# zhu-xlab/tomosar2height

Measured on AMD Instinct MI355X. Metric: training tiles/sec (Berlin crop, cloud-only), higher is better.
Workload: dtype f32; 1 GPU; BASELINE.json configs[1]: Berlin cloud-only, fp32 per-point GEMMs, train_step(tile) per tile, 4 tiles coalesced per forward/backward (Trainer default), N=131072 points/tile, R=256, ALTO depth 5, 512x512 target, optimize_every=64; points_per_tile=131072, optimize_every=64, train_batch=1, coalesce_tiles=4, optimizer=t2h FlatAdamW (one kernel over the flat bucket), parallelism=dp1, rccl_ranks=0, channels_last=True, point_distribution=70 % in 160 buildings + 30 % uniform, grid_convs=conv_bx3.hip: fp32 products from 3 fp16 MFMAs (2-way split, block scales), library_fallbacks=0, hip_graph=False

## Files before the change

### include/t2h.h

```cpp
#ifndef T2H_H_
#define T2H_H_

#include <stddef.h>
#include <stdint.h>

#ifdef __cplusplus
extern "C" {
#endif

#define T2H_OK 0
#define T2H_ERR_ARG (-1)
#define T2H_ERR_LAUNCH (-2)
#define T2H_ERR_WORKSPACE (-3)

#define T2H_ABI_VERSION 19
#define T2H_MAX_NBITS 10
#define T2H_MAX_RAGGED_TILES 64

typedef void *t2h_stream_t;

int t2h_abi_version(void);
const char *t2h_last_error_string(void);
const char *t2h_last_kernel_name(void);
void t2h_clear_kernel_name(void);
// ... 9 lines not shown
size_t t2h_tile_ragged_workspace_bytes(int B, int64_t total_rows, int max_rows, int nbits);
int t2h_tile_build_ragged(const float *cloud, int dim, int B, const int32_t *starts, int nbits, float *pts_sorted, int out_dim,
                          int32_t *perm, int32_t *cell, int32_t *off0, int32_t *status, void *workspace,
                          size_t workspace_bytes, t2h_stream_t stream);

int t2h_pool_winner_stride(int C);
int t2h_pool_max_fwd(const float *feat, int ldf, const int32_t *off0, int B, int nbits, int C, float *pooled,
                     int ldp, uint8_t *winner, t2h_stream_t stream);
int t2h_pool_max_bwd(const float *gpooled, int ldg, const uint8_t *winner, const int32_t *off0, int B, int nbits,
                     int C, int accumulate, float *gfeat, int ldo, t2h_stream_t stream);
int t2h_scatter_max_fwd(const float *feat, int ld, const int32_t *perm, const int32_t *off0, int B, int N, int nbits, int C,
                        float *val, int64_t *arg, t2h_stream_t stream);
int t2h_scatter_max_bwd(const float *gval, const int64_t *arg, int B, int C, int N, int64_t cells, float *gsrc,
                        t2h_stream_t stream);
int t2h_pool_mean(const float *feat, int ldf, const int32_t *off0, int B, int nbits, int C, int accumulate, float *out,
                  int ldo, t2h_stream_t stream);
int t2h_pool_rows_fwd(const float *feat, int ldf, const int32_t *cell, const int32_t *off0, int64_t n_rows, int C,
                      float *pooled, int ldp, uint8_t *winner, t2h_stream_t stream);
int t2h_pool_rows_bwd(const float *gpooled, int ldg, const uint8_t *winner, const int32_t *cell, const int32_t *off0,
                      int64_t n_rows, int C, int accumulate, float *gfeat, int ldo, t2h_stream_t stream);

size_t t2h_segmean_workspace_bytes(int B, int N, int nbits, int level, int C);
int t2h_segmean_fwd(const float *feat, const int32_t *off0, int B, int N, int nbits, int level, int C,
                    float *plane_nhwc, void *workspace, size_t workspace_bytes, t2h_stream_t stream);
int t2h_segmean_bwd(const float *gplane_nhwc, const int32_t *cell, const int32_t *off0, int B, int N,
                    int nbits, int level, int C, float *gfeat, t2h_stream_t stream);
int t2h_segsum_fwd(const float *feat, const int32_t *off0, int B, int N, int nbits, int level, int C,
                   float *plane_nhwc, int ld_plane, void *workspace, size_t workspace_bytes, t2h_stream_t stream);
int t2h_plane_sumpool2x2(const float *fine_nhwc, int ld_fine, int B, int r_fine, int C, float *coarse_nhwc, int ld_coarse,
                         t2h_stream_t stream);
int t2h_segsum_bwd_multi(const float *const *gplanes_nhwc, const int *levels, const int *lds, int n_planes, const int32_t *cell,
                         int B, int N, int nbits, int C, const float *mask, const float *addend, float *gfeat,
                         t2h_stream_t stream);
int t2h_cell_counts(const int32_t *off0, int B, int nbits, int level, float *cnt, t2h_stream_t stream);
int t2h_mean_bias_fwd(const float *acc, const float *cnt, const float *cvec, int64_t P, int C, float *out, t2h_stream_t stream);
size_t t2h_mean_bias_bwd_workspace_bytes(int64_t P, int C);
int t2h_mean_bias_bwd(const float *g, const float *cnt, int64_t P, int C, float *dacc, float *dcvec, void *workspace,
                      size_t workspace_bytes, t2h_stream_t stream);
int t2h_sample_relu_cellsums(const float *plane_nhwc, const float *pts, int dim, const int32_t *off0, int B, int N, int nbits,
                             int level, int sum_level, int C, float *sums_nhwc, int ld_sums, void *sign_bits, t2h_stream_t stream);
int t2h_sample_relu_cellsums2(const float *plane_nhwc, const float *pts, int dim, const int32_t *off0, int B, int N, int nbits,
                              int level, int sum_level, int C, float *sums_nhwc, int ld_sums, float *pooled_nhwc, int ld_pooled,
                              void *sign_bits, t2h_stream_t stream);
size_t t2h_cell_order_len(int B, int nbits, int level);
int t2h_cell_order_build(const int32_t *off0, int B, int nbits, int level, int32_t *order, t2h_stream_t stream);
int t2h_cell_order_build_range(const int32_t *off0, int B, int nbits, int level_lo, int level_hi, int32_t *order,
                               t2h_stream_t stream);
int t2h_sample_relu_cellsums_ordered(const float *plane_nhwc, const float *pts, int dim, const int32_t *off0, int B, int N,
                                     int nbits, int level, int sum_level, int C, float *sums_nhwc, int ld_sums, float *pooled_nhwc,
                                     int ld_pooled, void *sign_bits, const int32_t *cell_order, t2h_stream_t stream);
int t2h_sample_bwd_from_sums(const float *const *gplanes_nhwc, const int *levels, const int *lds, int n_planes,
                             const int32_t *cell, const void *mask, int mask_is_bits, const float *pts, int dim, const int32_t *off0, int B, int N,
                             int nbits, int level, int C, float *gplane_nhwc, void *workspace, size_t workspace_bytes,
                             t2h_stream_t stream);
int t2h_sample_bwd_from_sums_ordered(const float *const *gplanes_nhwc, const int *levels, const int *lds, int n_planes,
                                     const int32_t *cell, const void *mask, int mask_is_bits, const float *pts, int dim,
                                     const int32_t *off0, int B, int N, int nbits, int level, int C, float *gplane_nhwc,
                                     void *workspace, size_t workspace_bytes, const int32_t *cell_order, t2h_stream_t stream);
int t2h_segmean_bwd_add(const float *gplane_nhwc, const int32_t *cell, const int32_t *off0, int B, int N, int nbits,
                        int level, int C, const float *addend, float *gfeat, t2h_stream_t stream);

int t2h_sample_fwd(const float *plane_nhwc, const float *pts, int dim, int B, int N, int r, int C, float *out,
                   t2h_stream_t stream);
int t2h_sample_fwd_relu(const float *plane_nhwc, const float *pts, int dim, int B, int N, int r, int C, float *out,
                        void *sign_bits, t2h_stream_t stream);
size_t t2h_sample_bwd_workspace_bytes(int B, int N, int nbits, int level, int C);
// ... 216 lines not shown
```

### tomosar2height_amd/_lib.py

```python
import ctypes
import os

import torch

_HERE = os.path.dirname(os.path.abspath(__file__))
LIB_PATH = os.environ.get("T2H_LIBRARY") or os.path.join(_HERE, "libt2h_hip.so")
ABI_VERSION = 19

_vp, _i, _i64, _sz = ctypes.c_void_p, ctypes.c_int, ctypes.c_int64, ctypes.c_size_t

SIGNATURES = {
    "t2h_abi_version": (_i, []),
    "t2h_last_error_string": (ctypes.c_char_p, []),
    "t2h_last_kernel_name": (ctypes.c_char_p, []),
    "t2h_clear_kernel_name": (None, []),
    "t2h_debug_poison_lds": (_i, [_vp]),
    "t2h_coordinate2index": (_i, [_vp, _i, _i64, _i, _vp, _vp]),
    "t2h_tile_workspace_bytes": (_sz, [_i, _i, _i]),
    "t2h_tile_build": (_i, [_vp, _i, _i, _i, _i, _vp, _vp, _vp, _vp, _vp, _vp, _sz, _vp]),
    "t2h_tile_ragged_workspace_bytes": (_sz, [_i, _i64, _i, _i]),
    "t2h_tile_build_ragged": (_i, [_vp, _i, _i, _vp, _i, _vp, _i, _vp, _vp, _vp, _vp, _vp, _sz, _vp]),
    "t2h_pool_winner_stride": (_i, [_i]),
    "t2h_pool_max_fwd": (_i, [_vp, _i, _vp, _i, _i, _i, _vp, _i, _vp, _vp]),
    "t2h_pool_max_bwd": (_i, [_vp, _i, _vp, _vp, _i, _i, _i, _i, _vp, _i, _vp]),
    "t2h_pool_mean": (_i, [_vp, _i, _vp, _i, _i, _i, _i, _vp, _i, _vp]),
    "t2h_scatter_max_fwd": (_i, [_vp, _i, _vp, _vp, _i, _i, _i, _i, _vp, _vp, _vp]),
    "t2h_scatter_max_bwd": (_i, [_vp, _vp, _i, _i, _i, _i64, _vp, _vp]),
    "t2h_pool_rows_fwd": (_i, [_vp, _i, _vp, _vp, _i64, _i, _vp, _i, _vp, _vp]),
    "t2h_pool_rows_bwd": (_i, [_vp, _i, _vp, _vp, _vp, _i64, _i, _i, _vp, _i, _vp]),
    "t2h_segmean_workspace_bytes": (_sz, [_i, _i, _i, _i, _i]),
    "t2h_segmean_fwd": (_i, [_vp, _vp, _i, _i, _i, _i, _i, _vp, _vp, _sz, _vp]),
    "t2h_segmean_bwd": (_i, [_vp, _vp, _vp, _i, _i, _i, _i, _i, _vp, _vp]),
    "t2h_segmean_bwd_add": (_i, [_vp, _vp, _vp, _i, _i, _i, _i, _i, _vp, _vp, _vp]),
    "t2h_segsum_fwd": (_i, [_vp, _vp, _i, _i, _i, _i, _i, _vp, _i, _vp, _sz, _vp]),
    "t2h_plane_sumpool2x2": (_i, [_vp, _i, _i, _i, _i, _vp, _i, _vp]),
    "t2h_segsum_bwd_multi": (_i, [_vp, _vp, _vp, _i, _vp, _i, _i, _i, _i, _vp, _vp, _vp, _vp]),
    "t2h_cell_counts": (_i, [_vp, _i, _i, _i, _vp, _vp]),
    "t2h_mean_bias_fwd": (_i, [_vp, _vp, _vp, _i64, _i, _vp, _vp]),
    "t2h_mean_bias_bwd_workspace_bytes": (_sz, [_i64, _i]),
    "t2h_mean_bias_bwd": (_i, [_vp, _vp, _i64, _i, _vp, _vp, _vp, _sz, _vp]),
    "t2h_sample_relu_cellsums": (_i, [_vp, _vp, _i, _vp, _i, _i, _i, _i, _i, _i, _vp, _i, _vp, _vp]),
    "t2h_sample_relu_cellsums2": (_i, [_vp, _vp, _i, _vp, _i, _i, _i, _i, _i, _i, _vp, _i, _vp, _i, _vp, _vp]),
    "t2h_cell_order_len": (_sz, [_i, _i, _i]),
    "t2h_cell_order_build": (_i, [_vp, _i, _i, _i, _vp, _vp]),
    "t2h_cell_order_build_range": (_i, [_vp, _i, _i, _i, _i, _vp, _vp]),
    "t2h_sample_relu_cellsums_ordered": (_i, [_vp, _vp, _i, _vp, _i, _i, _i, _i, _i, _i, _vp, _i, _vp, _i, _vp, _vp, _vp]),
    "t2h_sample_bwd_from_sums": (_i, [_vp, _vp, _vp, _i, _vp, _vp, _i, _vp, _i, _vp, _i, _i, _i, _i, _i, _vp, _vp, _sz, _vp]),
    "t2h_sample_bwd_from_sums_ordered": (_i, [_vp, _vp, _vp, _i, _vp, _vp, _i, _vp, _i, _vp, _i, _i, _i, _i, _i, _vp, _vp, _sz, _vp, _vp]),
    "t2h_sample_fwd": (_i, [_vp, _vp, _i, _i, _i, _i, _i, _vp, _vp]),
# ... 288 lines not shown
    if name not in _declared:
        raise T2HLibraryError(f"{name} is not declared: the module that binds its header (`_lib.declare`) has not been imported, "
                              "and an untyped call would truncate 64-bit device pointers")
    return getattr(load(), name)


_POISON_LDS = os.environ.get("T2H_POISON_LDS", "0") == "1"


def call(name: str, *args, nbytes: int = 0, flops: int = 0, tag: str = None):
    fn = _fn_cache.get(name)
    if fn is None:
        fn = _fn_cache[name] = _entry(name)
    if _POISON_LDS:
        load().t2h_debug_poison_lds(stream())
    tl = _timeline
    if tl is None:
        rc = fn(*args)
        if rc != 0:
            check(rc, name)
        return
    else:
        s, e = torch.cuda.Event(enable_timing=True), torch.cuda.Event(enable_timing=True)
        lib = load()
        lib.t2h_clear_kernel_name()
        s.record()
        rc = fn(*args)
        e.record()
        symbol = lib.t2h_last_kernel_name().decode() or name
        tl.records.append((tag or name, nbytes, flops, s, e, symbol))
    check(rc, name)


def ptr(t: torch.Tensor) -> int:
    return t.data_ptr()


_ws_cache = {}


def ws_bytes(name: str, *args) -> int:
    key = (name, args)
    hit = _ws_cache.get(key)
    if hit is None:
        hit = _ws_cache[key] = int(_entry(name)(*args))
    return hit


def workspace(nbytes: int, device) -> torch.Tensor:
    return torch.empty(max(int(nbytes), 1), dtype=torch.uint8, device=device)


_on_stream = None
_set_stream = getattr(torch._C, "_cuda_setStream", None)


class on_stream:

    def __init__(self, st, back):
        self.st, self.back = st, back

    def __enter__(self):
        global _on_stream
        st = self.st
        self.prev, _on_stream = _on_stream, st.cuda_stream
        if _set_stream is not None:
# ... 81 lines not shown
```

### tomosar2height_amd/csrc/conv_bx3.hip

```cpp
#include <stdlib.h>
#include "t2h_common.h"
#include "gemm_args.h"
#include "gemm_tile.h"

namespace t2h {
namespace {

using bf16x8 = __attribute__((ext_vector_type(8))) __bf16;
using f16x8 = __attribute__((ext_vector_type(8))) _Float16;
using f16x2 = __attribute__((ext_vector_type(2))) _Float16;
using bf16x2 = __attribute__((ext_vector_type(2))) __bf16;
using f32x2 = __attribute__((ext_vector_type(2))) float;
using s16x4 = __attribute__((ext_vector_type(4))) short;
using s16x8 = __attribute__((ext_vector_type(8))) short;
typedef __attribute__((address_space(3))) void lds_void;
typedef const __attribute__((address_space(1))) void glb_void;
typedef __attribute__((address_space(3))) s16x4 lds_s16x4;

#ifndef T2H_BX3_BDIRECT
#define T2H_BX3_BDIRECT 1
#endif
constexpr int NT = 256;
constexpr int TW = 32;
constexpr int CC = 32;
// ... 150 lines not shown
__global__ __launch_bounds__(256) void prep_split_batch_kernel(PrepBatch b) {
    const int i = prep_find(b, blockIdx.x);
    const t2h_prep_desc &d = b.d[i];
    const long long t = (long long)(blockIdx.x - b.first[i]) * 256 + threadIdx.x;
    unsigned *wf = static_cast<unsigned *>(d.wf), *trailer = wf + d.trailer_word;
    if (d.h2) {
        if (t == 0) trailer[d.maxslot ^ 3] = 0u;
        if (d.kind == 0) prepare_conv_body<false, true>(d.w, d.a, d.b, wf, trailer, d.maxslot, t);
        else if (d.kind == 1) prepare_conv_body<true, true>(d.w, d.a, d.b, wf, trailer, d.maxslot, t);
        else if (d.kind == 2) prepare_gemm_body<true, true>(d.w, d.a, d.b, d.ldw, wf, trailer, d.maxslot, t);
        else prepare_gemm_body<false, true>(d.w, d.a, d.b, d.ldw, wf, trailer, d.maxslot, t);
    } else {
        if (d.kind == 0) prepare_conv_body<false, false>(d.w, d.a, d.b, wf, nullptr, 0, t);
        else if (d.kind == 1) prepare_conv_body<true, false>(d.w, d.a, d.b, wf, nullptr, 0, t);
        else if (d.kind == 2) prepare_gemm_body<true, false>(d.w, d.a, d.b, d.ldw, wf, nullptr, 0, t);
        else prepare_gemm_body<false, false>(d.w, d.a, d.b, d.ldw, wf, nullptr, 0, t);
    }
}

struct RowsArgs {
    const float *x;
    const unsigned *wf;
    const float *wscale;
    const float *bias;
    const float *mask;
    float *y;
    int B, H, W, Kc, Nc, flags;
    int splits, chunks_per_split;
    int ntn_per_wg;
    int ldx, ldy, ldm;
    const float *addend;
    int up_logW, up_logH, up_cout;
    const float *r1_g, *r1_w;
};

__device__ inline size_t up_pixel(long long m, int tap, int logW, int logH) {
    const long long x = m & ((1LL << logW) - 1), y = (m >> logW) & ((1LL << logH) - 1), b = m >> (logW + logH);
    return (size_t)(((b << (logH + 1)) + 2 * y + (tap >> 1)) << (logW + 1)) + 2 * x + (tap & 1);
}

template <int TH, int BN, int WAVES_M, int WAVES_N, int CCH, int NPL, int NTAP, int UPM = 0, bool PERSIST = false>
__global__ __launch_bounds__(NT, 2) void bx3_rows_kernel(RowsArgs p) {
    static_assert(UPM == 0 || NTAP == 1, "the transposed convolution runs on the 1-tap form");
    static_assert(!PERSIST || (NTAP == 1 && UPM == 0 && T2H_BX3_BDIRECT != 0), "PERSIST: plain 1-tap form with register-fetched weights");
    constexpr int PXB = CCH * 2 + 16;
    constexpr int NQ = CCH / 16, F4 = CCH / 4, NSTEP = NTAP * NQ;
    constexpr int QUNROLL = (NPL == 3 && NTAP == 9) ? 1 : NQ;
    constexpr int TM = TH / WAVES_M, TN = BN / (32 * WAVES_N);
    constexpr int HB = NTAP == 9 ? 1 : 0;
    constexpr int HW = TW + 2 * HB;
    constexpr int HP = (TH + 2 * HB) * HW;
    constexpr int PLANE = HP * PXB;
    constexpr int BSLAB = (BN / 32) * NPL * 1024;
    constexpr int HALO_BYTES = NPL * PLANE;
    constexpr bool BDIRECT = T2H_BX3_BDIRECT != 0;
    constexpr int LDS_WORK = HALO_BYTES + (BDIRECT ? 0 : 2 * BSLAB);
    constexpr int PATCH_BYTES = 4 * 32 * 36 * 4;
    constexpr int LDS_BYTES = PERSIST ? LDS_WORK + PATCH_BYTES : (LDS_WORK >= PATCH_BYTES ? LDS_WORK : PATCH_BYTES);
    constexpr bool H2 = NPL == 2;
    constexpr int WPL = H2 ? 2 : 3;
    static_assert(WAVES_M * WAVES_N == 4 && TM * WAVES_M == TH && TN * WAVES_N * 32 == BN, "wave layout");
    __shared__ __attribute__((aligned(1024))) unsigned char lds[LDS_BYTES + (H2 ? 64 : 0)];
    unsigned char *halo = lds, *bbuf = lds + HALO_BYTES;
    float *slots = reinterpret_cast<float *>(lds + LDS_BYTES);

    const int tid = threadIdx.x, lane = tid & 63, wave = tid >> 6;
    const int wm = wave / WAVES_N, wn = wave % WAVES_N;
    const unsigned nb = gridDim.x, bid = blockIdx.x;
    const unsigned qq = nb / 8, rr = nb % 8, xx = bid % 8, i8 = bid / 8;
    unsigned t = (xx < rr ? xx * (qq + 1) : rr * (qq + 1) + (xx - rr) * qq) + i8;
    const int split = t % p.splits; t /= p.splits;
    const int ntn = p.Nc / BN;
    const int tn_groups = PERSIST ? (ntn + p.ntn_per_wg - 1) / p.ntn_per_wg : ntn;
    const int tng = t % tn_groups; t /= tn_groups;
    const int tn_lo = PERSIST ? tng * p.ntn_per_wg : tng, tn_hi = PERSIST ? min(ntn, tn_lo + p.ntn_per_wg) : tng + 1;
    const int tiles_x = p.W / TW;
    const int tx = t % tiles_x; t /= tiles_x;
    const int tiles_y = p.H / TH;
    const int ty = t % tiles_y, b = t / tiles_y;
    const int x0 = tx * TW, y0 = ty * TH;
    int n0 = tn_lo * BN;
    const int c_beg = split * p.chunks_per_split, c_end = min(p.Kc / CCH, c_beg + p.chunks_per_split);

    constexpr int NF4 = HP * F4, PER = (NF4 + NT - 1) / NT;
    float4 hreg[PER];
    auto halo_load = [&](int c) {
#pragma unroll
        for (int f = 0; f < PER; ++f) {
            const int idx = tid + f * NT;
            const int px = idx / F4, c4 = idx % F4;
            const int hy = px / HW, hx = px - hy * HW;
            const int gy = y0 + hy - HB, gx = x0 + hx - HB;
            float4 v = make_float4(0.f, 0.f, 0.f, 0.f);
            if (UPM == 2) {
                const int k0 = c * CCH, tap = k0 / p.up_cout, co0 = k0 - tap * p.up_cout;
                if (idx < NF4)
                    v = *reinterpret_cast<const float4 *>(p.x + up_pixel(((long long)b * p.H + gy) * p.W + gx, tap, p.up_logW, p.up_logH) *
                                                                    p.ldx + co0 + c4 * 4);
            } else if (idx < NF4 && (unsigned)gy < (unsigned)p.H && (unsigned)gx < (unsigned)p.W)
                v = *reinterpret_cast<const float4 *>(p.x + (((size_t)b * p.H + gy) * p.W + gx) * p.ldx + c * CCH + c4 * 4);
            hreg[f] = v;
        }
    };
    int e_run = E_UNSET, e_cur = 0;
    auto halo_store = [&]() {
#pragma unroll
        for (int f = 0; f < PER; ++f) {
            const int idx = tid + f * NT;
            if (idx < NF4) {
                const int px = idx / F4, c4 = idx % F4;
                unsigned a1, a2, a3, b1, b2, b3;
                unsigned char *d = halo + px * PXB + c4 * 8;
                if (H2) {
                    split2h(hreg[f].x, hreg[f].y, e_cur, a1, a2);
                    split2h(hreg[f].z, hreg[f].w, e_cur, b1, b2);
                    *reinterpret_cast<uint2 *>(d) = make_uint2(a1, b1);
                    *reinterpret_cast<uint2 *>(d + PLANE) = make_uint2(a2, b2);
                    continue;
                }
                split3(hreg[f].x, hreg[f].y, a1, a2, a3);
                split3(hreg[f].z, hreg[f].w, b1, b2, b3);
                *reinterpret_cast<uint2 *>(d) = make_uint2(a1, b1);
                if (NPL == 3) {
                    *reinterpret_cast<uint2 *>(d + PLANE) = make_uint2(a2, b2);
                    *reinterpret_cast<uint2 *>(d + 2 * PLANE) = make_uint2(a3, b3);
                }
            }
        }
    };
    auto publish_block_max = [&](int parity) {
        float m = 0.f;
#pragma unroll
// ... 770 lines not shown
    if (int rc = check_launch("conv3x3_bx3_wgrad")) return rc;
    return launch_reduce_slabs(slab, p.splits, (long long)Cout * Ncols, Cout, Ncols, Ncols, (flags & T2H_ACCUM) ? 1 : 0, dw, colslab, db, s,
                               0, 0, (flags & T2H_DEFER_REDUCE) != 0);
}

T2H_API int t2h_gemm_bx3_supported(int64_t M, int K, int N) {
    return M >= 128 && M % 128 == 0 && M <= (1LL << 30) && K >= 64 && K % 64 == 0 && N >= 32 && N % 32 == 0;
}

T2H_API size_t t2h_gemm_bx3_weights_bytes(int K, int N) {
    if (K < 16 || N < 32 || K % 16 || N % 32) return 0;
    return (size_t)K * N * 6;
}

T2H_API int t2h_gemm_bx3_prepare(const float *w, int ldw, int K, int N, int w_is_kn, void *wf, t2h_stream_t stream) {
    if (!w || !wf) return fail(T2H_ERR_ARG, "gemm_bx3_prepare: null pointer");
    if (K < 16 || N < 32 || K % 16 || N % 32 || !al16(wf) || ldw < (w_is_kn ? N : K))
        return fail(T2H_ERR_ARG, "gemm_bx3_prepare: K=%d must be a multiple of 16, N=%d of 32, ldw=%d at least the row length", K, N, ldw);
    const long long total = (long long)(K / 16) * (N / 32) * 64;
    const unsigned blocks = (unsigned)((total + 255) / 256);
    if (w_is_kn) hipLaunchKernelGGL(bx3_prepare_gemm_kernel<true>, dim3(blocks), dim3(256), 0, as_stream(stream), w, K, N, ldw, static_cast<unsigned *>(wf));
    else hipLaunchKernelGGL(bx3_prepare_gemm_kernel<false>, dim3(blocks), dim3(256), 0, as_stream(stream), w, K, N, ldw, static_cast<unsigned *>(wf));
    return check_launch("gemm_bx3_prepare");
}

T2H_API size_t t2h_gemm_bx3_workspace_bytes(int64_t M, int K, int N) {
    if (!t2h_gemm_bx3_supported(M, K, N)) return 0;
    const RowsPlan r = bx3_rows_plan(1, (int)(M / 32), 32, K, N, 1);
    return r.splits > 1 ? (size_t)r.splits * M * N * sizeof(float) : 0;
}

T2H_API int t2h_gemm_bx3(const float *x, int ldx, const void *wf, const float *bias, const float *mask, int ldm, float *y, int ldy,
                         int64_t M, int K, int N, int flags, void *workspace, size_t workspace_bytes, t2h_stream_t stream) {
    if (!x || !wf || !y) return fail(T2H_ERR_ARG, "gemm_bx3: null pointer");
    if (!t2h_gemm_bx3_supported(M, K, N))
        return fail(T2H_ERR_ARG, "gemm_bx3: needs M %% 128 == 0, K %% 64 == 0, N %% 32 == 0 (M=%lld K=%d N=%d)", (long long)M, K, N);
    if (ldx < K || ldy < N || ldx % 4 || ldy % 4 || (mask && (ldm < N || ldm % 4)) || !al16(x) || !al16(wf) || !al16(y) || (bias && !al16(bias)) ||
        (mask && !al16(mask)))
        return fail(T2H_ERR_ARG, "gemm_bx3: rows must be 16-byte aligned and at least K / N floats long");
    RowsArgs a{};
    a.x = x; a.wf = static_cast<const unsigned *>(wf); a.bias = bias; a.mask = mask; a.y = y;
    a.B = 1; a.H = (int)(M / 32); a.W = 32; a.Kc = K; a.Nc = N; a.ldx = ldx; a.ldy = ldy; a.ldm = ldm;
    a.flags = ((flags & T2H_RELU_OUT) ? F_RELU_OUT : 0) | ((flags & T2H_ACCUM) ? F_ACCUM : 0);
    a.wscale = f16_trailer(wf, (size_t)K * N * 4);
    return launch_rows(a, npl_of(flags), workspace, workspace_bytes, as_stream(stream), "gemm_bx3", 1);
}

static int gemm_wgrad_splits(int64_t M, int N) {
    static const long long target = getenv("T2H_GEMM_BX3_WGRAD_WGS") ? atoll(getenv("T2H_GEMM_BX3_WGRAD_WGS")) : 4096;
    const long long groups = N / 64, units = M / TW;
    long long splits = (target + groups - 1) / groups;
    if (splits > units) splits = units;
    if (splits < 1) splits = 1;
    const long long per = (units + splits - 1) / splits;
    return (int)((units + per - 1) / per);
}

T2H_API int t2h_gemm_bx3_wgrad_supported(int64_t M, int K, int N) {
    return M >= TW && M % TW == 0 && M <= (1LL << 30) && (K == 64 || K == 128 || K == 256) && N >= 64 && N % 64 == 0;
}

T2H_API size_t t2h_gemm_bx3_wgrad_workspace_bytes(int64_t M, int K, int N) {
    if (!t2h_gemm_bx3_wgrad_supported(M, K, N)) return 0;
    return (size_t)gemm_wgrad_splits(M, N) * ((size_t)N * K + N) * sizeof(float);
}

T2H_API int t2h_gemm_bx3_wgrad(const float *dy, int lddy, const float *x, int ldx, int64_t M, int K, int N, float *dw, float *db, int flags,
                               void *workspace, size_t workspace_bytes, t2h_stream_t stream) {
    if (!dy || !x || !dw) return fail(T2H_ERR_ARG, "gemm_bx3_wgrad: null pointer");
    if (!t2h_gemm_bx3_wgrad_supported(M, K, N))
        return fail(T2H_ERR_ARG, "gemm_bx3_wgrad: needs M %% 32 == 0, K in {64, 128, 256}, N %% 64 == 0 (M=%lld K=%d N=%d)", (long long)M, K, N);
    if (lddy < N || ldx < K || lddy % 4 || ldx % 4 || !al16(dy) || !al16(x))
        return fail(T2H_ERR_ARG, "gemm_bx3_wgrad: rows must be 16-byte aligned and at least N / K floats long");
    if (!(flags & T2H_F16X2)) return fail(T2H_ERR_ARG, "gemm_bx3_wgrad: only the fp16 two-way split (T2H_F16X2) is built");
    const size_t need = t2h_gemm_bx3_wgrad_workspace_bytes(M, K, N);
    if (!workspace || workspace_bytes < need || !al16(workspace))
        return fail(T2H_ERR_WORKSPACE, "gemm_bx3_wgrad: workspace %zu < %zu bytes", workspace_bytes, need);
// ... 195 lines not shown
```

### tomosar2height_amd/csrc/deferred.hip

```cpp
#include "t2h_common.h"
#include "gemm_tile.h"

namespace t2h {
namespace {

__global__ __launch_bounds__(256) void cell_counts_kernel(const int32_t *__restrict__ off0, int B, int nbits, int level,
                                                         float *__restrict__ cnt) {
    const int rbits = nbits - level, r = 1 << rbits;
    const int64_t total = (int64_t)B << (2 * rbits);
    const int64_t i = (int64_t)blockIdx.x * 256 + threadIdx.x;
    if (i >= total) return;
    const int x = (int)(i & (r - 1)), y = (int)((i >> rbits) & (r - 1));
    const int64_t b = i >> (2 * rbits);
    const size_t obase = ((size_t)b << (2 * nbits)) + ((size_t)morton2((uint32_t)x, (uint32_t)y) << (2 * level));
    cnt[i] = (float)(off0[obase + ((size_t)1 << (2 * level))] - off0[obase]);
}

__global__ __launch_bounds__(256) void mean_bias_fwd_kernel(const float *__restrict__ acc, const float *__restrict__ cnt,
                                                           const float *__restrict__ cvec, int64_t total4, int C4,
                                                           float *__restrict__ out) {
    const int64_t t = (int64_t)blockIdx.x * 256 + threadIdx.x;
    if (t >= total4) return;
    const int64_t p = t / C4;
    const int c4 = (int)(t % C4);
    const float n = cnt[p];
    const float den = n > 0.f ? n : 1.f, ne = n > 0.f ? 1.f : 0.f;
    const float4 a = reinterpret_cast<const float4 *>(acc)[t];
    const float4 cv = reinterpret_cast<const float4 *>(cvec)[c4];
    float4 o;
    o.x = __fadd_rn(__fdiv_rn(a.x, den), __fmul_rn(ne, cv.x)); o.y = __fadd_rn(__fdiv_rn(a.y, den), __fmul_rn(ne, cv.y));
    o.z = __fadd_rn(__fdiv_rn(a.z, den), __fmul_rn(ne, cv.z)); o.w = __fadd_rn(__fdiv_rn(a.w, den), __fmul_rn(ne, cv.w));
    reinterpret_cast<float4 *>(out)[t] = o;
}

static int mb_rows(int64_t P) {
    int64_t r = (P + 255) / 256;
    r = (r + 63) / 64 * 64;
    return (int)(r < 64 ? 64 : (r > 4096 ? 4096 : r));
}
__global__ __launch_bounds__(256) void mean_bias_bwd_kernel(const float *__restrict__ g, const float *__restrict__ cnt,
                                                           int64_t P, int C, float *__restrict__ dacc,
                                                           float *__restrict__ slab, int kMbRows) {
    __shared__ float4 red[256];
    const int C4 = C / 4;
    const int cols = min(C4, 256), slots = 256 / cols;
    const int col = threadIdx.x % cols, slot = threadIdx.x / cols;
    const int64_t p0 = (int64_t)blockIdx.x * kMbRows;
    const int rows = (int)min((int64_t)kMbRows, P - p0);
    for (int c4base = 0; c4base < C4; c4base += cols) {
        const int c4 = c4base + col;
        float4 s = make_float4(0.f, 0.f, 0.f, 0.f);
        if (slot < slots && c4 < C4) {
            for (int i = slot; i < rows; i += slots) {
                const float n = cnt[p0 + i];
                const float4 v = reinterpret_cast<const float4 *>(g + (size_t)(p0 + i) * C)[c4];
                if (dacc) {
                    const float den = n > 0.f ? n : 1.f;
                    reinterpret_cast<float4 *>(dacc + (size_t)(p0 + i) * C)[c4] =
                        make_float4(__fdiv_rn(v.x, den), __fdiv_rn(v.y, den), __fdiv_rn(v.z, den), __fdiv_rn(v.w, den));
                }
                if (n > 0.f) { s.x += v.x; s.y += v.y; s.z += v.z; s.w += v.w; }
            }
        }
        __syncthreads();
        red[threadIdx.x] = s;
        __syncthreads();
        if (slab && slot == 0 && c4 < C4) {
            float4 t = red[col];
            for (int q = 1; q < slots; ++q) {
                const float4 u = red[q * cols + col];
                t.x += u.x; t.y += u.y; t.z += u.z; t.w += u.w;
            }
            reinterpret_cast<float4 *>(slab + (size_t)blockIdx.x * C)[c4] = t;
        }
    }
}

}
}

using namespace t2h;

T2H_API int t2h_cell_counts(const int32_t *off0, int B, int nbits, int level, float *cnt, t2h_stream_t stream) {
    if (!off0 || !cnt) return fail(T2H_ERR_ARG, "cell_counts: null pointer");
    if (B < 1 || nbits < 1 || nbits > T2H_MAX_NBITS || level < 0 || level > nbits) return fail(T2H_ERR_ARG, "cell_counts: bad level");
    const int64_t total = (int64_t)B << (2 * (nbits - level));
    hipLaunchKernelGGL(cell_counts_kernel, dim3((unsigned)((total + 255) / 256)), dim3(256), 0, as_stream(stream), off0, B, nbits,
                       level, cnt);
    return check_launch("cell_counts");
}

static bool al16(const void *p) { return ((uintptr_t)p & 15) == 0; }

T2H_API int t2h_mean_bias_fwd(const float *acc, const float *cnt, const float *cvec, int64_t P, int C, float *out,
                              t2h_stream_t stream) {
    if (!acc || !cnt || !cvec || !out) return fail(T2H_ERR_ARG, "mean_bias_fwd: null pointer");
    if (P < 0 || C < 4 || C % 4 != 0 || !al16(acc) || !al16(cvec) || !al16(out))
        return fail(T2H_ERR_ARG, "mean_bias_fwd: needs C %% 4 == 0 and 16-byte aligned rows");
    if (P == 0) return T2H_OK;
    const int64_t total4 = P * (C / 4);
    hipLaunchKernelGGL(mean_bias_fwd_kernel, dim3((unsigned)((total4 + 255) / 256)), dim3(256), 0, as_stream(stream), acc, cnt,
                       cvec, total4, C / 4, out);
    return check_launch("mean_bias_fwd");
}

T2H_API size_t t2h_mean_bias_bwd_workspace_bytes(int64_t P, int C) {
    if (P < 1 || C < 1) return 0;
    const int kMbRows = mb_rows(P);
    return (size_t)((P + kMbRows - 1) / kMbRows) * C * sizeof(float);
}

T2H_API int t2h_mean_bias_bwd(const float *g, const float *cnt, int64_t P, int C, float *dacc, float *dcvec, void *workspace,
                              size_t workspace_bytes, t2h_stream_t stream) {
    if (!g || !cnt) return fail(T2H_ERR_ARG, "mean_bias_bwd: null pointer");
    if (P < 1 || C < 4 || C % 4 != 0 || !al16(g) || (dacc && !al16(dacc)) || (dcvec && !al16(dcvec)))
        return fail(T2H_ERR_ARG, "mean_bias_bwd: needs P >= 1, C %% 4 == 0 and 16-byte aligned rows");
    const size_t need = t2h_mean_bias_bwd_workspace_bytes(P, C);
    if (dcvec && (!workspace || workspace_bytes < need || !al16(workspace)))
        return fail(T2H_ERR_WORKSPACE, "mean_bias_bwd: workspace %zu < %zu bytes", workspace_bytes, need);
    if (!dacc && !dcvec) return T2H_OK;
    const int kMbRows = mb_rows(P);
    const int blocks = (int)((P + kMbRows - 1) / kMbRows);
    float *slab = dcvec ? static_cast<float *>(workspace) : nullptr;
    hipLaunchKernelGGL(mean_bias_bwd_kernel, dim3(blocks), dim3(256), 0, as_stream(stream), g, cnt, P, C, dacc, slab, kMbRows);
    if (int rc = check_launch("mean_bias_bwd")) return rc;
    if (!dcvec) return T2H_OK;
    return launch_reduce_slabs(slab, blocks, C, 1, C, C, 0, dcvec, nullptr, nullptr, as_stream(stream));
}
```

### tomosar2height_amd/csrc/gemm.hip

```cpp
#include <stdlib.h>
#include <mutex>
#include <string>
#include <vector>
#include "t2h_common.h"
#include "gemm_args.h"
#include "gemm_tile.h"

namespace t2h {

using bf16x8 = __attribute__((ext_vector_type(8))) __bf16;

template <int BM, int BN, int WAVES_M, int WAVES_N, bool A_KC, bool B_KC, int BK = 16, bool XCD = true, int MINW = 1,
          int MODE = 0>
__global__ __launch_bounds__(64 * WAVES_M * WAVES_N, MINW) void gemm_kernel(GemmArgs p) {
    constexpr int NT = 64 * WAVES_M * WAVES_N;
    constexpr int TM = BM / (32 * WAVES_M), TN = BN / (32 * WAVES_N);
    constexpr int SA = BM + kPad, SB = BN + kPad;
    static_assert(TM >= 1 && TN >= 1, "tile too small for the wave grid");
    constexpr int LDS_MIN = (NT / 64) * 32 * 36 > 4 * NT ? (NT / 64) * 32 * 36 : 4 * NT;
    constexpr int LDS_FLOATS = 2 * BK * (SA + SB) > LDS_MIN ? 2 * BK * (SA + SB) : LDS_MIN;
    __shared__ __attribute__((aligned(16))) float lds[LDS_FLOATS];
    constexpr int BUF = BK * (SA + SB);

    const int tid = threadIdx.x, lane = tid & 63, wave = tid >> 6;
    const int wm = wave / WAVES_N, wn = wave % WAVES_N;
    int tile_m = blockIdx.y, tile_n = blockIdx.x, split = blockIdx.z;
    if (XCD) {
        const unsigned nb = gridDim.x * gridDim.y * gridDim.z;
        const unsigned b = (blockIdx.z * gridDim.y + blockIdx.y) * gridDim.x + blockIdx.x;
        const unsigned q = nb / 8, r = nb % 8, x = b % 8, i = b / 8;
        const unsigned t = (x < r ? x * (q + 1) : r * (q + 1) + (x - r) * q) + i;
        tile_n = t % gridDim.x;
        tile_m = (t / gridDim.x) % gridDim.y;
        split = t / (gridDim.x * gridDim.y);
    }
    const int m0 = tile_m * BM, n0 = tile_n * BN;
    const int kbeg = split * p.k_chunk;
    const int kend = min(p.K, kbeg + p.k_chunk);
    const bool relu_a = p.flags & F_RELU_A, relu_b = p.flags & F_RELU_B;

    TileLoader<BM, NT, A_KC, BK> la;
    TileLoader<BN, NT, B_KC, BK> lb;
    f32x16 acc[TM][TN];
#pragma unroll
    for (int i = 0; i < TM; ++i)
#pragma unroll
        for (int j = 0; j < TN; ++j)
#pragma unroll
            for (int q = 0; q < 16; ++q) acc[i][j][q] = 0.0f;

    float4 csum = make_float4(0.f, 0.f, 0.f, 0.f);
    const bool do_colsum = !A_KC && p.colsum != nullptr && tile_n == 0;

    const int nk = (kend - kbeg + BK - 1) / BK;
    if (nk > 0) {
        la.load(p.A, p.lda, m0, p.M, kbeg, kend, tid, relu_a);
        lb.load(p.B, p.ldb, n0, p.N, kbeg, kend, tid, relu_b);
        la.store(lds, tid);
        lb.store(lds + BK * SA, tid);
    }
    __syncthreads();
    for (int kt = 0; kt < nk; ++kt) {
        const int cur = kt & 1;
        if (do_colsum) {
#pragma unroll
            for (int f = 0; f < TileLoader<BM, NT, A_KC, BK>::PER; ++f) {
                csum.x += la.r[f].x; csum.y += la.r[f].y; csum.z += la.r[f].z; csum.w += la.r[f].w;
            }
        }
        if (kt + 1 < nk) {
            la.load(p.A, p.lda, m0, p.M, kbeg + (kt + 1) * BK, kend, tid, relu_a);
// ... 564 lines not shown
}

namespace {
struct WgradPlan { bool smallk; int bm, bn, tiles, splits, k_chunk; };
WgradPlan wgrad_plan(int M, int K, int N) {
    WgradPlan p{};
    p.smallk = (K % 4 != 0);
    if (p.smallk) { p.splits = (M + kSmallKRows - 1) / kSmallKRows; return p; }
    p.bm = N > 64 ? 128 : (N > 32 ? 64 : 32);
    p.bn = K > 64 ? 128 : (K > 32 ? 64 : 32);
    p.tiles = ((N + p.bm - 1) / p.bm) * ((K + p.bn - 1) / p.bn);
    const int target = p.tiles <= 2 ? 512 : 1024;
    int want = target / p.tiles;
    if (want > 512) want = 512;
    int max_splits = (M + 16 * kMinBK - 1) / (16 * kMinBK);
    int splits = want < 1 ? 1 : (want > max_splits ? max_splits : want);
    if (splits < 1) splits = 1;
    int chunk = (M + splits - 1) / splits;
    chunk = (chunk + 31) / 32 * 32;
    p.k_chunk = chunk;
    p.splits = (M + chunk - 1) / chunk;
    return p;
}
}

T2H_API size_t t2h_linear_wgrad_workspace_bytes(int M, int K, int N) {
    if (M < 1 || K < 1 || N < 1) return 0;
    WgradPlan p = wgrad_plan(M, K, N);
    return (size_t)p.splits * ((size_t)N * K + N) * sizeof(float);
}

T2H_API int t2h_linear_wgrad(const float *dy, int lddy, const float *x, int ldx, int M, int K, int N, int flags,
                             float *dw, float *db, void *workspace, size_t workspace_bytes, t2h_stream_t stream) {
    if (!dy || !x || !dw) return fail(T2H_ERR_ARG, "linear_wgrad: null pointer");
    if (M < 1 || K < 1 || N < 1 || lddy < N || ldx < K) return fail(T2H_ERR_ARG, "linear_wgrad: bad shape");
    size_t need = t2h_linear_wgrad_workspace_bytes(M, K, N);
    if (!workspace || workspace_bytes < need)
        return fail(T2H_ERR_WORKSPACE, "linear_wgrad: workspace %zu < %zu bytes", workspace_bytes, need);
    hipStream_t s = as_stream(stream);
    WgradPlan p = wgrad_plan(M, K, N);
    float *slab = static_cast<float *>(workspace);
    float *colslab = slab + (size_t)p.splits * N * K;
    int accumulate = (flags & T2H_ACCUM) ? 1 : 0;
    const bool direct = !p.smallk && p.splits == 1 && !accumulate && !db && aligned4(dw, K);
    if (direct) slab = dw;
    if (p.smallk) {
        if (K > kSmallKMax) return fail(T2H_ERR_ARG, "linear_wgrad: K=%d must be a multiple of 4 (or <= %d)", K, kSmallKMax);
        hipLaunchKernelGGL(wgrad_smallk_kernel, dim3(p.splits), dim3(256), 0, s, dy, lddy, x, ldx, M, K, N,
                           (flags & T2H_RELU_IN) ? 1 : 0, slab, db ? colslab : nullptr);
    } else {
        if (N % 4 != 0 || !aligned4(dy, lddy) || !aligned4(x, ldx))
            return fail(T2H_ERR_ARG, "linear_wgrad: N=%d must be a multiple of 4 (16-byte rows)", N);
        GemmArgs a{};
        a.A = dy; a.lda = lddy; a.B = x; a.ldb = ldx; a.C = slab; a.ldc = K; a.colsum = db ? colslab : nullptr;
        a.M = N; a.N = K; a.K = M; a.flags = (flags & T2H_RELU_IN) ? F_RELU_B : 0;
        a.k_chunk = p.k_chunk; a.slab_stride = (long long)N * K;
        int rc;
        const int mode = mode_of(flags);
        static const int kwaves_wgrad_max_rows = [] { const char *e = getenv("T2H_KWAVES_WGRAD_MAX_ROWS"); return e ? atoi(e) : 1024; }();
        if (mode == 0 && !db && M <= kwaves_wgrad_max_rows && aligned4(dw, K) && kwaves_applicable(N, K, M)) {
            a.C = dw; a.colsum = nullptr; a.k_chunk = M; a.slab_stride = 0;
            if (accumulate) a.flags |= F_ACCUM;
            return launch_gemm_kwaves<false, false>(a, s, "linear_wgrad");
        }
#define T2H_WG(BM_, BN_, WM_, WN_, MW_)                                                                                \
    (mode == 2 ? launch_gemm<BM_, BN_, WM_, WN_, false, false, 16, true, (MW_ > 2 ? 2 : MW_), 2>(a, p.splits, s, "linear_wgrad") \
     : mode == 1 ? launch_gemm<BM_, BN_, WM_, WN_, false, false, 16, true, (MW_ > 3 ? 3 : MW_), 1>(a, p.splits, s, "linear_wgrad") \
                 : launch_gemm<BM_, BN_, WM_, WN_, false, false, 16, true, MW_, 0>(a, p.splits, s, "linear_wgrad"))
        static const bool tn_dma = !(getenv("T2H_GEMM_DMA") && getenv("T2H_GEMM_DMA")[0] == '0');
        if (p.bm == 128 && p.bn == 128 && mode == 0 && tn_dma && gemm_dma_tn_applicable(a))
            rc = launch_gemm_dma_tn(a, p.splits, s, "linear_wgrad");
        else if (p.bm == 128 && p.bn == 128)
            rc = mode != 0 ? launch_gemm_split(mode, false, false, a, p.splits, s, "linear_wgrad") : T2H_WG(128, 128, 2, 2, 4);
        else if (p.bm == 128 && p.bn == 64) rc = T2H_WG(128, 64, 2, 2, 1);
        else if (p.bm == 128 && p.bn == 32) rc = T2H_WG(128, 32, 4, 1, 1);
        else if (p.bm == 64 && p.bn == 128) rc = T2H_WG(64, 128, 2, 2, 1);
        else if (p.bm == 64 && p.bn == 64) rc = T2H_WG(64, 64, 2, 2, 1);
        else if (p.bm == 64 && p.bn == 32) rc = T2H_WG(64, 32, 2, 1, 1);
        else if (p.bm == 32 && p.bn == 128) rc = T2H_WG(32, 128, 1, 4, 1);
        else if (p.bm == 32 && p.bn == 64) rc = T2H_WG(32, 64, 1, 2, 1);
        else rc = T2H_WG(32, 32, 1, 1, 1);
#undef T2H_WG
        if (rc) return rc;
    }
    if (direct) return T2H_OK;
    return launch_reduce_slabs(slab, p.splits, (long long)N * K, N, K, K, accumulate, dw, colslab, db, s, 0, 0,
                               (flags & T2H_DEFER_REDUCE) != 0);
}
```

### tomosar2height_amd/csrc/gemm_args.h

```cpp
#pragma once
#include <hip/hip_runtime.h>

namespace t2h {

enum : int { F_RELU_A = 1, F_RELU_B = 2, F_RELU_OUT = 4, F_ACCUM = 8 };

struct GemmArgs {
    const float *A, *B;
    float *C;
    const float *bias;
    const float *mask;
    const float *addend;
    int ldadd;
    float *colsum;
    int M, N, K;
    int lda, ldb, ldc, ldm;
    int flags;
    int k_chunk;
    long long slab_stride;
};

int launch_gemm_split(int mode, bool a_kc, bool b_kc, const GemmArgs &a, int splits, hipStream_t s, const char *what);

bool gemm_dma_applicable(bool b_kc, const GemmArgs &a);
int launch_gemm_dma(bool b_kc, const GemmArgs &a, hipStream_t s, const char *what);
bool gemm_dma_tn_applicable(const GemmArgs &a);
int launch_gemm_dma_tn(const GemmArgs &a, int splits, hipStream_t s, const char *what);

}
```

### tomosar2height_amd/csrc/point_grid.hip

```cpp
#include <float.h>
#include <stdlib.h>

#include "t2h_common.h"

namespace t2h {

constexpr int kThreads = 256;

struct GroupCfg {
    int lg;
    int span;
};

template <int VEC>
static GroupCfg group_cfg(int C) {
    GroupCfg g;
    g.lg = group_log2(C, VEC);
    g.span = (1 << g.lg) * VEC;
    return g;
}

static inline unsigned grid_for(int64_t groups, int lg) {
    int64_t threads = groups << lg;
    return (unsigned)((threads + kThreads - 1) / kThreads);
// ... 292 lines not shown
            for (int g = 1; g < NG; ++g) { const float4 v = pval[g * G + lane]; t.x += v.x; t.y += v.y; t.z += v.z; t.w += v.w; }
            oval[side * G + lane] = t;
        }
        __syncthreads();
    }
#pragma unroll
    for (int p = 0; p < PASSES; ++p) {
        const int row = r0 + p * NG + grp;
        if (row >= r1 || row != max(segs[p], r0)) continue;
        float4 acc = segs[p] < r0 ? oval[lane] : make_float4(0.f, 0.f, 0.f, 0.f);
        const int end = min(sege[p], r1);
        for (int n = row; n < end; ++n) { const float4 v = val[(n - r0) * G + lane]; acc.x += v.x; acc.y += v.y; acc.z += v.z; acc.w += v.w; }
        if (sege[p] > r1) { const float4 v = oval[G + lane]; acc.x += v.x; acc.y += v.y; acc.z += v.z; acc.w += v.w; }
        val[(row - r0) * G + lane] = acc;
    }
    __syncthreads();
#pragma unroll
    for (int p = 0; p < PASSES; ++p) {
        const int row = r0 + p * NG + grp;
        if (row >= r1 || !cv) continue;
        const float4 sum = val[(max(segs[p], r0) - r0) * G + lane];
        const uint8_t bits = winner[(size_t)row * wstride + lane];
        float4 o = make_float4((bits & 1) ? sum.x : 0.f, (bits & 2) ? sum.y : 0.f, (bits & 4) ? sum.z : 0.f, (bits & 8) ? sum.w : 0.f);
        float4 *dst = reinterpret_cast<float4 *>(gfeat + (size_t)row * ldo + lane * 4);
        if (accumulate) { const float4 old = *dst; o.x += old.x; o.y += old.y; o.z += old.z; o.w += old.w; }
        *dst = o;
    }
}

template <int VEC, bool MEAN = true>
__global__ __launch_bounds__(kThreads) void segmean_fwd_kernel(const float *__restrict__ feat,
                                                               const int32_t *__restrict__ off0, int B, int nbits,
                                                               int level, int C, int lg, float *__restrict__ plane,
                                                               int ld_out) {
    int64_t t = (int64_t)blockIdx.x * kThreads + threadIdx.x;
    int64_t gid = t >> lg;
    const int rbits = nbits - level;
    const int64_t cells_per_tile = (int64_t)1 << (2 * rbits);
    if (gid >= (int64_t)B * cells_per_tile) return;
    int b = (int)(gid >> (2 * rbits));
    uint32_t mk = (uint32_t)(gid & (cells_per_tile - 1));
    size_t obase = ((size_t)b << (2 * nbits)) + ((size_t)mk << (2 * level));
    int s = off0[obase], e = off0[obase + ((size_t)1 << (2 * level))];
    int cx = (int)compact1by1(mk), cy = (int)compact1by1(mk >> 1);
    int r = 1 << rbits;
    float *orow = plane + (((size_t)b * r + cy) * r + cx) * ld_out;
    float inv_den = (float)(e - s > 0 ? e - s : 1);
    int span = VEC << lg;
    for (int c = ((int)t & ((1 << lg) - 1)) * VEC; c < C; c += span) {
        float sum[VEC];
#pragma unroll
        for (int j = 0; j < VEC; ++j) sum[j] = 0.0f;
        int n = s;
        for (; n + 4 <= e; n += 4) {
            Vec<VEC> a0 = Vec<VEC>::load(feat + (size_t)(n + 0) * C + c);
            Vec<VEC> a1 = Vec<VEC>::load(feat + (size_t)(n + 1) * C + c);
            Vec<VEC> a2 = Vec<VEC>::load(feat + (size_t)(n + 2) * C + c);
            Vec<VEC> a3 = Vec<VEC>::load(feat + (size_t)(n + 3) * C + c);
#pragma unroll
            for (int j = 0; j < VEC; ++j) sum[j] = (((sum[j] + a0.v[j]) + a1.v[j]) + a2.v[j]) + a3.v[j];
        }
        for (; n < e; ++n) {
            Vec<VEC> a = Vec<VEC>::load(feat + (size_t)n * C + c);
#pragma unroll
            for (int j = 0; j < VEC; ++j) sum[j] += a.v[j];
        }
        Vec<VEC> o;
#pragma unroll
        for (int j = 0; j < VEC; ++j) o.v[j] = MEAN ? __fdiv_rn(sum[j], inv_den) : sum[j];
        o.store(orow + c);
    }
}

constexpr int kMaxMultiPlanes = 8;
struct MultiPlanes { const float *g[kMaxMultiPlanes]; int level[kMaxMultiPlanes]; int ld[kMaxMultiPlanes]; int n; };
template <int VEC>
__global__ __launch_bounds__(kThreads) void segsum_bwd_multi_kernel(MultiPlanes mp, const int32_t *__restrict__ cell,
                                                                    int64_t npts, int nbits, int C, int lg,
                                                                    const float *__restrict__ mask,
                                                                    const float *__restrict__ addend,
                                                                    float *__restrict__ gfeat) {
    int64_t t = (int64_t)blockIdx.x * kThreads + threadIdx.x;
    int64_t n = t >> lg;
    if (n >= npts) return;
    const uint32_t code = (uint32_t)cell[n];
    const uint32_t b = code >> (2 * nbits), m = code & ((1u << (2 * nbits)) - 1u);
    const uint32_t x0 = compact1by1(m), y0 = compact1by1(m >> 1);
    const float *rows[kMaxMultiPlanes];
#pragma unroll
    for (int q = 0; q < kMaxMultiPlanes; ++q) {
        rows[q] = nullptr;
        if (q < mp.n) {
            const int l = mp.level[q], r = 1 << (nbits - l);
            rows[q] = mp.g[q] + (((size_t)b * r + (y0 >> l)) * r + (x0 >> l)) * mp.ld[q];
        }
    }
    const int span = VEC << lg;
    for (int c = ((int)t & ((1 << lg) - 1)) * VEC; c < C; c += span) {
        Vec<VEC> acc = Vec<VEC>::load(rows[0] + c);
#pragma unroll
        for (int q = 1; q < kMaxMultiPlanes; ++q)
            if (q < mp.n) {
                Vec<VEC> g = Vec<VEC>::load(rows[q] + c);
#pragma unroll
                for (int j = 0; j < VEC; ++j) acc.v[j] = __fadd_rn(acc.v[j], g.v[j]);
            }
        if (mask) {
            Vec<VEC> h = Vec<VEC>::load(mask + (size_t)n * C + c);
#pragma unroll
            for (int j = 0; j < VEC; ++j) acc.v[j] = h.v[j] > 0.0f ? acc.v[j] : 0.0f;
        }
        if (addend) {
            Vec<VEC> o = Vec<VEC>::load(addend + (size_t)n * C + c);
#pragma unroll
            for (int j = 0; j < VEC; ++j) acc.v[j] = __fadd_rn(o.v[j], acc.v[j]);
        }
        acc.store(gfeat + (size_t)n * C + c);
    }
}

__global__ __launch_bounds__(kThreads) void plane_sumpool2x2_kernel(const float *__restrict__ fine, int64_t total4, int rc,
                                                                   int C4, int ld_in, int ld_out, float *__restrict__ coarse) {
    int64_t t = (int64_t)blockIdx.x * kThreads + threadIdx.x;
    if (t >= total4) return;
    const int c4 = (int)(t % C4);
    const int64_t pix = t / C4;
    const int x = (int)(pix % rc), y = (int)((pix / rc) % rc);
    const int64_t b = pix / ((int64_t)rc * rc);
    const int rf = 2 * rc;
    const float *f = fine + ((b * rf + 2 * y) * rf + 2 * x) * (int64_t)ld_in + 4 * c4;
    const float4 a = *reinterpret_cast<const float4 *>(f), bq = *reinterpret_cast<const float4 *>(f + ld_in);
    const float4 cq = *reinterpret_cast<const float4 *>(f + (int64_t)rf * ld_in);
    const float4 d = *reinterpret_cast<const float4 *>(f + (int64_t)rf * ld_in + ld_in);
    float4 o;
    o.x = (a.x + bq.x) + (cq.x + d.x); o.y = (a.y + bq.y) + (cq.y + d.y);
    o.z = (a.z + bq.z) + (cq.z + d.z); o.w = (a.w + bq.w) + (cq.w + d.w);
    *reinterpret_cast<float4 *>(coarse + pix * (int64_t)ld_out + 4 * c4) = o;
}

template <int VEC>
__global__ __launch_bounds__(kThreads) void segmean_bwd_kernel(const float *__restrict__ gplane,
                                                               const int32_t *__restrict__ cell,
                                                               const int32_t *__restrict__ off0, int64_t npts, int nbits,
                                                               int level, int C, int lg, const float *__restrict__ addend,
                                                               float *__restrict__ gfeat) {
    int64_t t = (int64_t)blockIdx.x * kThreads + threadIdx.x;
    int64_t n = t >> lg;
    if (n >= npts) return;
    uint32_t code = (uint32_t)cell[n];
    uint32_t b = code >> (2 * nbits);
    uint32_t m = code & ((1u << (2 * nbits)) - 1u);
    uint32_t mk = m >> (2 * level);
    size_t obase = ((size_t)b << (2 * nbits)) + ((size_t)mk << (2 * level));
    int cnt = off0[obase + ((size_t)1 << (2 * level))] - off0[obase];
    int rbits = nbits - level, r = 1 << rbits;
    int cx = (int)compact1by1(mk), cy = (int)compact1by1(mk >> 1);
    const float *grow = gplane + (((size_t)b * r + cy) * r + cx) * C;
    float den = (float)(cnt > 0 ? cnt : 1);
    int span = VEC << lg;
    for (int c = ((int)t & ((1 << lg) - 1)) * VEC; c < C; c += span) {
        Vec<VEC> g = Vec<VEC>::load(grow + c);
#pragma unroll
        for (int j = 0; j < VEC; ++j) g.v[j] = __fdiv_rn(g.v[j], den);
        if (addend) {
            Vec<VEC> o = Vec<VEC>::load(addend + (size_t)n * C + c);
#pragma unroll
// ... 74 lines not shown
}

__device__ inline float keep_if(unsigned long long lanes, float v) {
    float o;
    asm("v_cndmask_b32_e64 %0, 0, %1, %2" : "=v"(o) : "v"(v), "s"(lanes));
    return o;
}
__device__ inline float readlane_f(float v, int i) { return __int_as_float(__builtin_amdgcn_readlane(__float_as_int(v), i)); }
__device__ inline unsigned long long readlane_u64(unsigned long long v, int i) {
    const unsigned lo = (unsigned)__builtin_amdgcn_readlane((int)(unsigned)v, i);
    const unsigned hi = (unsigned)__builtin_amdgcn_readlane((int)(unsigned)(v >> 32), i);
    return ((unsigned long long)hi << 32) | lo;
}

typedef float f32x2 __attribute__((ext_vector_type(2)));
__device__ inline void park8(unsigned (&acc)[8], unsigned long long w0, unsigned long long w1, unsigned long long w2,
                             unsigned long long w3, int i) {
    asm("s_mov_b32 m0, %8\n\t"
        "v_writelane_b32 %0, %9, m0\n\tv_writelane_b32 %1, %10, m0\n\tv_writelane_b32 %2, %11, m0\n\tv_writelane_b32 %3, %12, m0\n\t"
        "v_writelane_b32 %4, %13, m0\n\tv_writelane_b32 %5, %14, m0\n\tv_writelane_b32 %6, %15, m0\n\tv_writelane_b32 %7, %16, m0"
        : "+v"(acc[0]), "+v"(acc[1]), "+v"(acc[2]), "+v"(acc[3]), "+v"(acc[4]), "+v"(acc[5]), "+v"(acc[6]), "+v"(acc[7])
        : "s"(__builtin_amdgcn_readfirstlane(i)), "s"((unsigned)w0), "s"((unsigned)(w0 >> 32)), "s"((unsigned)w1),
          "s"((unsigned)(w1 >> 32)), "s"((unsigned)w2), "s"((unsigned)(w2 >> 32)), "s"((unsigned)w3), "s"((unsigned)(w3 >> 32))
        : "m0");
}

template <int K, bool POOL>
__global__ __launch_bounds__(256, 2) void sample_relu_cellsums_v2_kernel(const float *__restrict__ plane,
                                                                        const float *__restrict__ pts, int dim,
                                                                        const int32_t *__restrict__ off0, int nbits, int level,
                                                                        int sum_level, int C, float *__restrict__ sums,
                                                                        int ld_sums, unsigned long long *__restrict__ bits,
                                                                        int npts_m1, float *__restrict__ sums2, int ld_sums2,
                                                                        const int32_t *__restrict__ order, int gz) {
    constexpr int SIDE = 3 + K, NS = SIDE * SIDE;
    __shared__ float4 T[NS][64];
    const int tid = threadIdx.x, lane = tid & 63, wave = tid >> 6;
    const int chunks = C >> 8;
    const int chunk = (int)(blockIdx.x % (unsigned)chunks), c0 = chunk * 256 + lane * 4;
    const int zpart = (int)((blockIdx.x / (unsigned)chunks) % (unsigned)gz);
    const unsigned rank = blockIdx.x / (unsigned)(chunks * gz);
    const int rbits = nbits - level, r = 1 << rbits, sbits = rbits - K;
    const int64_t wg = order ? (int64_t)order[rank] : (int64_t)rank;
    const int b = (int)(wg >> (2 * sbits));
    const uint32_t smk = (uint32_t)(wg & (((int64_t)1 << (2 * sbits)) - 1));
    const int d = level - sum_level, nchild = 1 << (2 * d), rs = 1 << (nbits - sum_level);
    const uint32_t mk = K == 0 ? smk : ((smk << 2) | (uint32_t)wave);
    const int cx = (int)compact1by1(mk), cy = (int)compact1by1(mk >> 1);
    const int per_wave = K == 0 ? nchild / (gz * 4) : nchild;
    const int child_lo = K == 0 ? (zpart * 4 + wave) * per_wave : 0, child_hi = child_lo + per_wave;
    const size_t obase = ((size_t)b << (2 * nbits)) + ((size_t)mk << (2 * level));
    int bnd_lo, bnd_hi;
    {
        const int ci = child_lo + lane;
        bnd_lo = ci <= child_hi ? off0[obase + ((size_t)ci << (2 * sum_level))] : 0;
        bnd_hi = ci + 1 <= child_hi ? off0[obase + ((size_t)(ci + 1) << (2 * sum_level))] : 0;
    }
    const int wx0 = K == 0 ? cx - 1 : 2 * (int)compact1by1(smk) - 1, wy0 = K == 0 ? cy - 1 : 2 * (int)compact1by1(smk >> 1) - 1;
    for (int e = tid; e < NS * 64; e += 256) {
        const int sl = e >> 6, py = wy0 + sl / SIDE, px = wx0 + sl % SIDE;
        float4 v = make_float4(0.f, 0.f, 0.f, 0.f);
        if ((unsigned)py < (unsigned)r && (unsigned)px < (unsigned)r)
            v = *reinterpret_cast<const float4 *>(plane + (((size_t)b * r + py) * r + px) * C + chunk * 256 + (e & 63) * 4);
        T[sl][e & 63] = v;
    }
    const int row_first = __builtin_amdgcn_readfirstlane(bnd_lo);
    const int row_end = off0[obase + ((size_t)child_hi << (2 * sum_level))];
// ... 37 lines not shown
                    sw_l = y1ok ? __fmul_rn(tp.wx0, tp.wy1) : 0.f;
                    se_l = (x1ok && y1ok) ? __fmul_rn(tp.wx1, tp.wy1) : 0.f;
#else
                    const float fx1 = (float)min(max(r - 1 - tp.x0, 0), 1), fy1 = (float)min(max(r - 1 - tp.y0, 0), 1);
                    nw_l = __fmul_rn(tp.wx0, tp.wy0);
                    ne_l = __fmul_rn(__fmul_rn(tp.wx1, tp.wy0), fx1);
                    sw_l = __fmul_rn(__fmul_rn(tp.wx0, tp.wy1), fy1);
                    se_l = __fmul_rn(__fmul_rn(tp.wx1, tp.wy1), __fmul_rn(fx1, fy1));
#endif
                    slot_l = (min(max(tp.y0 - cy + 1, 0), 1) + (K ? (wave >> 1) : 0)) * SIDE +
                             min(max(tp.x0 - cx + 1, 0), 1) + (K ? (wave & 1) : 0);
                }
                const int i0 = n - nb0, cnt = min(e - n, 64 - i0);
                auto row = [&](int i) {
                    const float nw = readlane_f(nw_l, i), ne = readlane_f(ne_l, i), sw = readlane_f(sw_l, i), se = readlane_f(se_l, i);
                    const float4 *t00 = Tl + __builtin_amdgcn_readlane(slot_l, i) * 64;
                    const float4 v00 = t00[0], v01 = t00[64], v10 = t00[SIDE * 64], v11 = t00[(SIDE + 1) * 64];
                    f32x2 a01 = f32x2{v00.x, v00.y} * nw, a23 = f32x2{v00.z, v00.w} * nw;
                    a01 = a01 + f32x2{v01.x, v01.y} * ne; a23 = a23 + f32x2{v01.z, v01.w} * ne;
                    a01 = a01 + f32x2{v10.x, v10.y} * sw; a23 = a23 + f32x2{v10.z, v10.w} * sw;
                    a01 = a01 + f32x2{v11.x, v11.y} * se; a23 = a23 + f32x2{v11.z, v11.w} * se;
                    a01.x = fmaxf(a01.x, 0.f); a01.y = fmaxf(a01.y, 0.f); a23.x = fmaxf(a23.x, 0.f); a23.y = fmaxf(a23.y, 0.f);
                    const unsigned long long w0 = __ballot(a01.x > 0.f), w1 = __ballot(a01.y > 0.f);
                    const unsigned long long w2 = __ballot(a23.x > 0.f), w3 = __ballot(a23.y > 0.f);
                    park8(bl, w0, w1, w2, w3, i);
                    sum01 = sum01 + a01; sum23 = sum23 + a23;
                };
                for (int j = 0; j < cnt; ++j) row(i0 + j);
                n += cnt;
            }
            const float4 sum = make_float4(sum01.x, sum01.y, sum23.x, sum23.y);
            const uint32_t cm = (uint32_t)(cb + c);
            const int fx = (cx << d) + (int)compact1by1(cm), fy = (cy << d) + (int)compact1by1(cm >> 1);
            *reinterpret_cast<float4 *>(sums + (((size_t)b * rs + fy) * rs + fx) * ld_sums + c0) = sum;
            if (POOL) {
                const unsigned k4 = cm & 3u;
                if (k4 == 0u) pe = sum;
                else if (k4 == 1u) p01 = make_float4(pe.x + sum.x, pe.y + sum.y, pe.z + sum.z, pe.w + sum.w);
                else if (k4 == 2u) pe = sum;
                else {
                    const float4 o = make_float4(p01.x + (pe.x + sum.x), p01.y + (pe.y + sum.y), p01.z + (pe.z + sum.z),
                                                 p01.w + (pe.w + sum.w));
                    const int rs2 = rs >> 1;
                    *reinterpret_cast<float4 *>(sums2 + (((size_t)b * rs2 + (fy >> 1)) * rs2 + (fx >> 1)) * ld_sums2 + c0) = o;
                }
            }
        }
    }
    flush_bits();
}

template <int VEC>
__global__ __launch_bounds__(kThreads) void sample_bwd_kernel(const float *__restrict__ gout,
                                                              const float *__restrict__ pts, int dim,
                                                              const int32_t *__restrict__ off0, int B, int nbits,
                                                              int level, int C, int lg, const float *__restrict__ addend,
                                                              float *__restrict__ gplane) {
    int64_t t = (int64_t)blockIdx.x * kThreads + threadIdx.x;
    int64_t gid = t >> lg;
    const int rbits = nbits - level, r = 1 << rbits;
    if (gid >= (int64_t)B * r * r) return;
    int b = (int)(gid >> (2 * rbits));
    const uint32_t pm = (uint32_t)(gid & (((int64_t)1 << (2 * rbits)) - 1));
    int py = (int)compact1by1(pm >> 1), px = (int)compact1by1(pm);
    int span = VEC << lg;
    int c0 = ((int)t & ((1 << lg) - 1)) * VEC;
    int segs[9], sege[9];
// ... 224 lines not shown
    int s = off0[obase], e = off0[obase + ((size_t)1 << (2 * level))];
    int lo, hi;
    split_range(s, e, sp, S, lo, hi);
    int c = chunk * cell_chunk_channels(C) + lane_c * 4;
    float4 acc = make_float4(0.f, 0.f, 0.f, 0.f);
    if (c < C) {
        int n = lo + slot;
        for (; n + P < hi; n += 2 * P) {
            float4 a0 = *reinterpret_cast<const float4 *>(feat + (size_t)n * C + c);
            float4 a1 = *reinterpret_cast<const float4 *>(feat + (size_t)(n + P) * C + c);
            acc.x = (acc.x + a0.x) + a1.x; acc.y = (acc.y + a0.y) + a1.y;
            acc.z = (acc.z + a0.z) + a1.z; acc.w = (acc.w + a0.w) + a1.w;
        }
        for (; n < hi; n += P) {
            float4 a0 = *reinterpret_cast<const float4 *>(feat + (size_t)n * C + c);
            acc.x += a0.x; acc.y += a0.y; acc.z += a0.z; acc.w += a0.w;
        }
    }
    red[slot * G + lane_c] = acc;
    __syncthreads();
    if (slot == 0 && c < C) {
        float4 t = red[lane_c];
        for (int q = 1; q < P; ++q) {
            float4 u = red[q * G + lane_c];
            t.x += u.x; t.y += u.y; t.z += u.z; t.w += u.w;
        }
        *reinterpret_cast<float4 *>(partial + ((size_t)cellrow * S + sp) * C + c) = t;
    }
}

__global__ __launch_bounds__(kThreads) void segmean_finalize_kernel(const float *__restrict__ partial,
                                                                   const int32_t *__restrict__ off0, int B, int nbits,
                                                                   int level, int C, int lg, int S,
                                                                   float *__restrict__ plane, int mean = 1, int ld_out = 0) {
    int64_t t = (int64_t)blockIdx.x * kThreads + threadIdx.x;
    int64_t gid = t >> lg;
    const int rbits = nbits - level;
    const int64_t cells_per_tile = (int64_t)1 << (2 * rbits);
    if (gid >= (int64_t)B * cells_per_tile) return;
    int b = (int)(gid >> (2 * rbits));
    uint32_t mk = (uint32_t)(gid & (cells_per_tile - 1));
    size_t obase = ((size_t)b << (2 * nbits)) + ((size_t)mk << (2 * level));
    int cnt = off0[obase + ((size_t)1 << (2 * level))] - off0[obase];
    float den = (float)(cnt > 0 ? cnt : 1);
    int cx = (int)compact1by1(mk), cy = (int)compact1by1(mk >> 1), r = 1 << rbits;
    float *orow = plane + (((size_t)b * r + cy) * r + cx) * (ld_out > 0 ? ld_out : C);
    for (int c = ((int)t & ((1 << lg) - 1)) * 4; c < C; c += 4 << lg) {
        float4 acc = make_float4(0.f, 0.f, 0.f, 0.f);
        for (int sp = 0; sp < S; ++sp) {
            float4 u = *reinterpret_cast<const float4 *>(partial + ((size_t)gid * S + sp) * C + c);
            acc.x += u.x; acc.y += u.y; acc.z += u.z; acc.w += u.w;
        }
        if (mean) {
            acc.x = __fdiv_rn(acc.x, den); acc.y = __fdiv_rn(acc.y, den);
            acc.z = __fdiv_rn(acc.z, den); acc.w = __fdiv_rn(acc.w, den);
        }
        *reinterpret_cast<float4 *>(orow + c) = acc;
    }
}

template <bool FUSED>
__global__ __launch_bounds__(kCellThreads) void sample_bwd_cells_kernel(const float *__restrict__ gout,
                                                                        const float *__restrict__ pts, int dim,
                                                                        const int32_t *__restrict__ off0, int nbits,
                                                                        int level, int C, int lgG, int S,
                                                                        float *__restrict__ partial, MultiPlanes mp,
                                                                        const int32_t *__restrict__ cell,
                                                                        const float *__restrict__ mask) {
    extern __shared__ float4 red[];
    const int G = 1 << lgG, P = kCellThreads >> lgG;
    int lane_c = threadIdx.x & (G - 1), slot = threadIdx.x >> lgG;
    int64_t cellrow = blockIdx.x;
    int sp = blockIdx.y % S, chunk = blockIdx.y / S;
    const int rbits = nbits - level, r = 1 << rbits;
    int b = (int)(cellrow >> (2 * rbits));
    uint32_t mk = (uint32_t)(cellrow & (((int64_t)1 << (2 * rbits)) - 1));
    int cx = (int)compact1by1(mk), cy = (int)compact1by1(mk >> 1);
    size_t obase = ((size_t)b << (2 * nbits)) + ((size_t)mk << (2 * level));
    int s = off0[obase], e = off0[obase + ((size_t)1 << (2 * level))];
    int lo, hi;
    split_range(s, e, sp, S, lo, hi);
    int c = chunk * cell_chunk_channels(C) + lane_c * 4;
    float4 acc[9];
#pragma unroll
    for (int q = 0; q < 9; ++q) acc[q] = make_float4(0.f, 0.f, 0.f, 0.f);
    if (c < C) {
        auto fetch = [&](int n, Taps &tp, float4 &g) {
            tp = make_taps(pts[(size_t)n * dim + 0], pts[(size_t)n * dim + 1], r);
            if (FUSED) {
                const uint32_t code = (uint32_t)cell[n];
                const uint32_t fb = code >> (2 * nbits), fm = code & ((1u << (2 * nbits)) - 1u);
                const uint32_t fx = compact1by1(fm), fy = compact1by1(fm >> 1);
                const float4 hm = *reinterpret_cast<const float4 *>(mask + (size_t)n * C + c);
                g = make_float4(0.f, 0.f, 0.f, 0.f);
#pragma unroll
                for (int q = 0; q < kMaxMultiPlanes; ++q)
                    if (q < mp.n) {
                        const int l = mp.level[q], rq = 1 << (nbits - l);
                        const float4 u = *reinterpret_cast<const float4 *>(mp.g[q] + (((size_t)fb * rq + (fy >> l)) * rq + (fx >> l)) * mp.ld[q] + c);
                        if (q == 0) g = u;
                        else { g.x = __fadd_rn(g.x, u.x); g.y = __fadd_rn(g.y, u.y); g.z = __fadd_rn(g.z, u.z); g.w = __fadd_rn(g.w, u.w); }
                    }
                g.x = hm.x > 0.f ? g.x : 0.f; g.y = hm.y > 0.f ? g.y : 0.f;
                g.z = hm.z > 0.f ? g.z : 0.f; g.w = hm.w > 0.f ? g.w : 0.f;
            } else {
                g = *reinterpret_cast<const float4 *>(gout + (size_t)n * C + c);
            }
        };
        auto accumulate = [&](const Taps &tp, const float4 &g) {
            const int dx = tp.x0 - cx + 1, dy = tp.y0 - cy + 1;
#pragma unroll
            for (int sy = 0; sy < 3; ++sy) {
                float wy = (sy == dy) ? tp.wy0 : ((sy == dy + 1) ? tp.wy1 : 0.0f);
#pragma unroll
                for (int sx = 0; sx < 3; ++sx) {
                    float wx = (sx == dx) ? tp.wx0 : ((sx == dx + 1) ? tp.wx1 : 0.0f);
                    float w = __fmul_rn(wx, wy);
                    float4 &a = acc[sy * 3 + sx];
                    a.x = __fmaf_rn(w, g.x, a.x); a.y = __fmaf_rn(w, g.y, a.y);
                    a.z = __fmaf_rn(w, g.z, a.z); a.w = __fmaf_rn(w, g.w, a.w);
                }
            }
        };
        int n = lo + slot;
        for (; n + P < hi; n += 2 * P) {
            Taps t0, t1;
            float4 g0, g1;
            fetch(n, t0, g0);
            fetch(n + P, t1, g1);
            accumulate(t0, g0);
            accumulate(t1, g1);
        }
// ... 32 lines not shown
                                                                             const int32_t *__restrict__ cell,
                                                                             const float *__restrict__ mask, int tlevel,
                                                                             size_t npts) {
    __shared__ float Wl[kMfmaRows][16];
    __shared__ int Po[kMfmaRows][kMaxMultiPlanes];
    __shared__ float4 Tl[FUSED ? 16 : 1][FUSED ? 65 : 1];
    __shared__ int Ti[kMfmaRows];
    const int tid = threadIdx.x, lane = tid & 63, wave = tid >> 6;
    const int64_t cellrow = blockIdx.x;
    const int sp = blockIdx.y % S, chunk = blockIdx.y / S;
    const int rbits = nbits - level, r = 1 << rbits;
    const int b = (int)(cellrow >> (2 * rbits));
    const uint32_t mk = (uint32_t)(cellrow & (((int64_t)1 << (2 * rbits)) - 1));
    const int cx = (int)compact1by1(mk), cy = (int)compact1by1(mk >> 1);
    const size_t obase = ((size_t)b << (2 * nbits)) + ((size_t)mk << (2 * level));
    const int s = off0[obase], e = off0[obase + ((size_t)1 << (2 * level))];
    int lo, hi;
    split_range(s, e, sp, S, lo, hi);
    const int ch = chunk * cell_chunk_channels(C) + wave * 64 + 4 * (lane & 15);
    const bool active = ch < C;
    const int kq = lane >> 4;
    if (FUSED && tlevel >= 0 && lo < hi) {
        const int tb = 2 * (level - tlevel), nT = 1 << tb;
        for (int e = tid; e < nT * 64; e += kCellThreads) {
            const int t = e >> 6, c4 = e & 63, che = chunk * cell_chunk_channels(C) + c4 * 4;
            if (che < C) {
                const uint32_t mt = (mk << tb) | (uint32_t)t;
                const uint32_t tx = compact1by1(mt), ty = compact1by1(mt >> 1);
                float4 v = make_float4(0.f, 0.f, 0.f, 0.f);
#pragma unroll
                for (int q = 0; q < kMaxMultiPlanes; ++q)
                    if (q < mp.n && mp.level[q] >= tlevel) {
                        const int l = mp.level[q], rq = 1 << (nbits - l), sh = l - tlevel;
                        const float4 w = *reinterpret_cast<const float4 *>(
                            mp.g[q] + (((size_t)b * rq + (ty >> sh)) * rq + (tx >> sh)) * mp.ld[q] + che);
                        v.x = __fadd_rn(v.x, w.x); v.y = __fadd_rn(v.y, w.y); v.z = __fadd_rn(v.z, w.z); v.w = __fadd_rn(v.w, w.w);
                    }
                Tl[t][c4] = v;
            }
        }
    }
    f32x4_t acc[4];
#pragma unroll
    for (int t = 0; t < 4; ++t) acc[t] = f32x4_t{0.f, 0.f, 0.f, 0.f};
    for (int blk = lo; blk < hi; blk += kMfmaRows) {
        __syncthreads();
        if (tid < kMfmaRows) {
            const int n = blk + tid;
            float w[9];
#pragma unroll
            for (int q = 0; q < 9; ++q) w[q] = 0.0f;
            const int nn = min(n, hi - 1);
            if (n < hi) {
                const Taps tp = make_taps(pts[(size_t)n * dim + 0], pts[(size_t)n * dim + 1], r);
                const int dx = tp.x0 - cx + 1, dy = tp.y0 - cy + 1;
#pragma unroll
                for (int sy = 0; sy < 3; ++sy) {
                    const float wy = (sy == dy) ? tp.wy0 : ((sy == dy + 1) ? tp.wy1 : 0.0f);
#pragma unroll
                    for (int sx = 0; sx < 3; ++sx) {
                        const float wx = (sx == dx) ? tp.wx0 : ((sx == dx + 1) ? tp.wx1 : 0.0f);
                        w[sy * 3 + sx] = __fmul_rn(wx, wy);
                    }
                }
            }
            float4 *wr = reinterpret_cast<float4 *>(&Wl[tid][0]);
            wr[0] = make_float4(w[0], w[1], w[2], w[3]);
            wr[1] = make_float4(w[4], w[5], w[6], w[7]);
            wr[2] = make_float4(w[8], 0.f, 0.f, 0.f);
            wr[3] = make_float4(0.f, 0.f, 0.f, 0.f);
            if (FUSED) {
                const uint32_t code = (uint32_t)cell[nn];
                const uint32_t fb = code >> (2 * nbits), fm = code & ((1u << (2 * nbits)) - 1u);
                const uint32_t fx = compact1by1(fm), fy = compact1by1(fm >> 1);
#pragma unroll
                for (int q = 0; q < kMaxMultiPlanes; ++q)
                    if (q < mp.n) {
                        const int l = mp.level[q], rq = 1 << (nbits - l);
                        Po[tid][q] = (int)((fb * rq + (fy >> l)) * rq + (fx >> l));
                    }
                if (tlevel >= 0) Ti[tid] = (int)((fm >> (2 * tlevel)) & ((1u << (2 * (level - tlevel))) - 1u));
            }
        }
        __syncthreads();
        if (active) {
            const int steps = (min(kMfmaRows, hi - blk) + 3) >> 2;
            for (int st0 = 0; st0 < steps; st0 += 2) {
                float a[2];
                float4 g[2];
#pragma unroll
                for (int u = 0; u < 2; ++u) {
                    const int rr = 4 * (st0 + u) + kq;
                    const int n = min(blk + rr, hi - 1);
                    a[u] = Wl[rr][lane & 15];
                    if (FUSED) {
                        float4 hm;
                        if (BITS) {
                            const uint4 *bw = reinterpret_cast<const uint4 *>(
                                reinterpret_cast<const unsigned long long *>(mask) + ((size_t)(ch >> 8) * npts + n) * 4);
                            const uint4 b01 = bw[0], b23 = bw[1];
                            const int li = (ch & 255) >> 2;
                            const unsigned int s0 = li < 32 ? b01.x : b01.y, s1 = li < 32 ? b01.z : b01.w;
                            const unsigned int s2 = li < 32 ? b23.x : b23.y, s3 = li < 32 ? b23.z : b23.w;
                            const int sh = li & 31;
                            hm = make_float4((float)((s0 >> sh) & 1u), (float)((s1 >> sh) & 1u), (float)((s2 >> sh) & 1u),
                                             (float)((s3 >> sh) & 1u));
                        } else {
                            hm = *reinterpret_cast<const float4 *>(mask + (size_t)n * C + ch);
                        }
                        float4 v;
                        if (tlevel >= 0) {
                            v = Tl[Ti[rr]][wave * 16 + (lane & 15)];
// ... 51 lines not shown
                                                            const unsigned long long *__restrict__ bits, int npts_m1,
                                                            const int32_t *__restrict__ order) {
    constexpr int SIDE = 3 + K, NS = SIDE * SIDE;
    __shared__ float4 NB[4 * 9][64];
    const int tid = threadIdx.x, lane = tid & 63, wave = tid >> 6;
    const int cpc = C >> 8;
    const int chunk = (int)(blockIdx.x % (unsigned)cpc), c0 = chunk * 256 + lane * 4;
    const unsigned rank = blockIdx.x / (unsigned)cpc;
    const int rbits = nbits - level, r = 1 << rbits, sbits = rbits - K;
    const int64_t wg = order ? (int64_t)order[rank] : (int64_t)rank;
    const int b = (int)(wg >> (2 * sbits));
    const uint32_t smk = (uint32_t)(wg & (((int64_t)1 << (2 * sbits)) - 1));
    const int d = level - wl, nchild = 1 << (2 * d);
    const uint32_t mk = K == 0 ? smk : ((smk << 2) | (uint32_t)wave);
    const int child_lo = K == 0 ? wave * (nchild >> 2) : 0, child_hi = K == 0 ? child_lo + (nchild >> 2) : nchild;
    const int cx = (int)compact1by1(mk), cy = (int)compact1by1(mk >> 1);
    const size_t obase = ((size_t)b << (2 * nbits)) + ((size_t)mk << (2 * level));
    f32x2 acc[9][2];
#pragma unroll
    for (int q = 0; q < 9; ++q) { acc[q][0] = f32x2{0.f, 0.f}; acc[q][1] = f32x2{0.f, 0.f}; }
    float4 raw[kWalkPlanes];
    int held[kWalkPlanes];
    int prow_l[kWalkPlanes];
#pragma unroll
    for (int q = 0; q < kWalkPlanes; ++q) { held[q] = -1; prow_l[q] = 0; raw[q] = make_float4(0.f, 0.f, 0.f, 0.f); }
    auto plane_rows = [&](int child) {
        const uint32_t cm = (uint32_t)child;
        const int fx = (cx << d) + (int)compact1by1(cm), fy = (cy << d) + (int)compact1by1(cm >> 1);
#pragma unroll
        for (int q = 0; q < kWalkPlanes; ++q)
            if (q < mp.n) {
                const int sh = mp.level[q] - wl, rq = 1 << (nbits - mp.level[q]);
                prow_l[q] = (b * rq + (fy >> sh)) * rq + (fx >> sh);
            }
    };
    auto request = [&](int c) {
#pragma unroll
        for (int q = 0; q < kWalkPlanes; ++q)
            if (q < mp.n) {
                const int row = __builtin_amdgcn_readlane(prow_l[q], c);
                if (row != held[q]) {
                    held[q] = row;
                    raw[q] = *reinterpret_cast<const float4 *>(mp.g[q] + (size_t)row * mp.ld[q] + c0);
                }
            }
    };
    int nb0 = 0;
    float nw_l = 0.f, ne_l = 0.f, sw_l = 0.f, se_l = 0.f;
    unsigned long long cm0 = 0, cm1 = 0, cm2 = 0, cm3 = 0;
    unsigned long long w0_l = 0, w1_l = 0, w2_l = 0, w3_l = 0;
    bool have = false;
    for (int cb = child_lo; cb < child_hi; cb += 64) {
        const int ci = cb + lane;
        const int bnd_lo = ci < child_hi ? off0[obase + ((size_t)ci << (2 * wl))] : 0;
        const int bnd_hi = ci < child_hi ? off0[obase + ((size_t)(ci + 1) << (2 * wl))] : 0;
        unsigned long long todo = __ballot(bnd_hi > bnd_lo);
        plane_rows(ci);
        if (todo) request((int)__builtin_ctzll(todo));
        while (todo) {
            const int c = (int)__builtin_ctzll(todo);
            todo &= todo - 1;
            const int s = __builtin_amdgcn_readlane(bnd_lo, c), e = __builtin_amdgcn_readlane(bnd_hi, c);
            float4 G = raw[0];
#pragma unroll
            for (int q = 1; q < kWalkPlanes; ++q)
                if (q < mp.n) { G.x = __fadd_rn(G.x, raw[q].x); G.y = __fadd_rn(G.y, raw[q].y); G.z = __fadd_rn(G.z, raw[q].z); G.w = __fadd_rn(G.w, raw[q].w); }
// ... 312 lines not shown
    if (n_rows == 0) return T2H_OK;
    const int ws = t2h_pool_winner_stride(C);
    const int lg = group_log2(C, 4);
    const int rows_per_wg = (256 >> lg) > kPoolRows ? (256 >> lg) : kPoolRows;
    const unsigned blocks = (unsigned)((n_rows + rows_per_wg - 1) / rows_per_wg);
#define T2H_POOL_FWD(LG) hipLaunchKernelGGL(pool_rows_fwd_kernel<LG>, dim3(blocks), dim3(256), 0, as_stream(stream), feat, ldf, \
                                            cell, off0, (int)n_rows, C, pooled, ldp, winner, ws)
    if (lg <= 0) T2H_POOL_FWD(0); else if (lg == 1) T2H_POOL_FWD(1); else if (lg == 2) T2H_POOL_FWD(2);
    else if (lg == 3) T2H_POOL_FWD(3); else T2H_POOL_FWD(4);
#undef T2H_POOL_FWD
    return check_launch("pool_rows_fwd");
}

T2H_API int t2h_pool_rows_bwd(const float *gpooled, int ldg, const uint8_t *winner, const int32_t *cell, const int32_t *off0,
                              int64_t n_rows, int C, int accumulate, float *gfeat, int ldo, t2h_stream_t stream) {
    if (!gpooled || !winner || !cell || !off0 || !gfeat) return fail(T2H_ERR_ARG, "pool_rows_bwd: null pointer");
    if (n_rows < 0 || n_rows > (1LL << 30) || C < 4 || C % 4 || C > 64 || ldg < C || ldo < C || ldg % 4 || ldo % 4 ||
        (uintptr_t)gpooled % 16 || (uintptr_t)gfeat % 16)
        return fail(T2H_ERR_ARG, "pool_rows_bwd: needs C in {4, 8, .., 64} and 16-byte aligned rows");
    if (n_rows == 0) return T2H_OK;
    const int ws = t2h_pool_winner_stride(C);
    const int lg = group_log2(C, 4);
    const int rows_per_wg = (256 >> lg) > kPoolRows ? (256 >> lg) : kPoolRows;
    const unsigned blocks = (unsigned)((n_rows + rows_per_wg - 1) / rows_per_wg);
#define T2H_POOL_BWD(LG) hipLaunchKernelGGL(pool_rows_bwd_kernel<LG>, dim3(blocks), dim3(256), 0, as_stream(stream), gpooled, \
                                            ldg, winner, ws, cell, off0, (int)n_rows, C, accumulate, gfeat, ldo)
    if (lg <= 0) T2H_POOL_BWD(0); else if (lg == 1) T2H_POOL_BWD(1); else if (lg == 2) T2H_POOL_BWD(2);
    else if (lg == 3) T2H_POOL_BWD(3); else T2H_POOL_BWD(4);
#undef T2H_POOL_BWD
    return check_launch("pool_rows_bwd");
}

static int segreduce_fwd(bool mean, const float *feat, const int32_t *off0, int B, int N, int nbits, int level, int C,
                         float *plane_nhwc, int ld_out, void *workspace, size_t workspace_bytes, t2h_stream_t stream) {
    if (!feat || !off0 || !plane_nhwc) return fail(T2H_ERR_ARG, "segmean_fwd: null pointer");
    if (ld_out < C || (C % 4 == 0 && ld_out % 4 != 0)) return fail(T2H_ERR_ARG, "segmean_fwd: plane row stride %d < C = %d", ld_out, C);
    int rc = check_level("segmean_fwd", B, nbits, level, C);
    if (rc) return rc;
    int64_t groups = (int64_t)B << (2 * (nbits - level));
    CoarsePlan cp = coarse_plan(B, N, nbits, level, C);
    if (cp.use) {
        size_t need = t2h_segmean_workspace_bytes(B, N, nbits, level, C);
        if (!workspace || workspace_bytes < need)
            return fail(T2H_ERR_WORKSPACE, "segmean_fwd: workspace %zu < %zu bytes", workspace_bytes, need);
        float *partial = static_cast<float *>(workspace);
        int G = 1 << cp.lgG, P = kCellThreads >> cp.lgG;
        hipLaunchKernelGGL(segmean_cells_kernel, dim3((unsigned)groups, cp.S * cp.chunks), dim3(kCellThreads),
                           (size_t)P * G * sizeof(float4), as_stream(stream), feat, off0, nbits, level, C, cp.lgG, cp.S,
                           partial);
        GroupCfg g = group_cfg<4>(C);
        hipLaunchKernelGGL(segmean_finalize_kernel, dim3(grid_for(groups, g.lg)), dim3(kThreads), 0, as_stream(stream),
                           partial, off0, B, nbits, level, C, g.lg, cp.S, plane_nhwc, mean ? 1 : 0, ld_out);
        return check_launch("segmean_fwd(coarse)");
    }
    if (mean) {
        T2H_DISPATCH_VEC(C,
            { GroupCfg g = group_cfg<4>(C);
              hipLaunchKernelGGL(segmean_fwd_kernel<4>, dim3(grid_for(groups, g.lg)), dim3(kThreads), 0, as_stream(stream),
                                 feat, off0, B, nbits, level, C, g.lg, plane_nhwc, ld_out); },
            { GroupCfg g = group_cfg<1>(C);
              hipLaunchKernelGGL(segmean_fwd_kernel<1>, dim3(grid_for(groups, g.lg)), dim3(kThreads), 0, as_stream(stream),
                                 feat, off0, B, nbits, level, C, g.lg, plane_nhwc, ld_out); });
    } else {
        T2H_DISPATCH_VEC(C,
            { GroupCfg g = group_cfg<4>(C);
              hipLaunchKernelGGL((segmean_fwd_kernel<4, false>), dim3(grid_for(groups, g.lg)), dim3(kThreads), 0, as_stream(stream),
                                 feat, off0, B, nbits, level, C, g.lg, plane_nhwc, ld_out); },
            { GroupCfg g = group_cfg<1>(C);
              hipLaunchKernelGGL((segmean_fwd_kernel<1, false>), dim3(grid_for(groups, g.lg)), dim3(kThreads), 0, as_stream(stream),
                                 feat, off0, B, nbits, level, C, g.lg, plane_nhwc, ld_out); });
    }
    return check_launch("segmean_fwd");
}

T2H_API int t2h_segmean_fwd(const float *feat, const int32_t *off0, int B, int N, int nbits, int level, int C,
                            float *plane_nhwc, void *workspace, size_t workspace_bytes, t2h_stream_t stream) {
    return segreduce_fwd(true, feat, off0, B, N, nbits, level, C, plane_nhwc, C, workspace, workspace_bytes, stream);
}

T2H_API int t2h_segsum_fwd(const float *feat, const int32_t *off0, int B, int N, int nbits, int level, int C,
                           float *plane_nhwc, int ld_plane, void *workspace, size_t workspace_bytes, t2h_stream_t stream) {
    return segreduce_fwd(false, feat, off0, B, N, nbits, level, C, plane_nhwc, ld_plane, workspace, workspace_bytes, stream);
}

T2H_API int t2h_plane_sumpool2x2(const float *fine_nhwc, int ld_fine, int B, int r_fine, int C, float *coarse_nhwc, int ld_coarse,
                                 t2h_stream_t stream) {
    if (!fine_nhwc || !coarse_nhwc) return fail(T2H_ERR_ARG, "plane_sumpool2x2: null pointer");
    if (B < 1 || r_fine < 2 || (r_fine & 1) || C < 4 || C % 4 != 0 || ((uintptr_t)fine_nhwc & 15) || ((uintptr_t)coarse_nhwc & 15) ||
        ld_fine < C || ld_coarse < C || ld_fine % 4 != 0 || ld_coarse % 4 != 0)
        return fail(T2H_ERR_ARG, "plane_sumpool2x2: needs an even resolution, C %% 4 == 0, row strides >= C and 16-byte aligned rows");
    const int rc = r_fine / 2;
    const int64_t total4 = (int64_t)B * rc * rc * (C / 4);
    hipLaunchKernelGGL(plane_sumpool2x2_kernel, dim3((unsigned)((total4 + kThreads - 1) / kThreads)), dim3(kThreads), 0,
                       as_stream(stream), fine_nhwc, total4, rc, C / 4, ld_fine, ld_coarse, coarse_nhwc);
    return check_launch("plane_sumpool2x2");
}

T2H_API int t2h_segsum_bwd_multi(const float *const *gplanes_nhwc, const int *levels, const int *lds, int n_planes,
                                 const int32_t *cell, int B, int N, int nbits, int C, const float *mask, const float *addend,
                                 float *gfeat, t2h_stream_t stream) {
    if (!gplanes_nhwc || !levels || !lds || !cell || !gfeat) return fail(T2H_ERR_ARG, "segsum_bwd_multi: null pointer");
    if (n_planes < 1 || n_planes > kMaxMultiPlanes)
        return fail(T2H_ERR_ARG, "segsum_bwd_multi: 1..%d planes, got %d", kMaxMultiPlanes, n_planes);
    if (B < 1 || nbits < 1 || nbits > T2H_MAX_NBITS || C < 1) return fail(T2H_ERR_ARG, "segsum_bwd_multi: unsupported shape");
    MultiPlanes mp{};
    mp.n = n_planes;
    for (int q = 0; q < n_planes; ++q) {
        if (!gplanes_nhwc[q] || levels[q] < 0 || levels[q] > nbits) return fail(T2H_ERR_ARG, "segsum_bwd_multi: bad plane %d", q);
        if (C % 4 == 0 && (((uintptr_t)gplanes_nhwc[q] & 15) || lds[q] % 4 != 0)) return fail(T2H_ERR_ARG, "segsum_bwd_multi: planes must be 16-byte aligned");
        if (lds[q] < C) return fail(T2H_ERR_ARG, "segsum_bwd_multi: plane %d row stride %d < C", q, lds[q]);
        mp.g[q] = gplanes_nhwc[q]; mp.level[q] = levels[q]; mp.ld[q] = lds[q];
    }
    if (C % 4 == 0 && ((mask && ((uintptr_t)mask & 15)) || (addend && ((uintptr_t)addend & 15)) || ((uintptr_t)gfeat & 15)))
        return fail(T2H_ERR_ARG, "segsum_bwd_multi: rows must be 16-byte aligned");
    const int64_t npts = rows_of(B, N);
    if (npts == 0) return T2H_OK;
    T2H_DISPATCH_VEC(C,
        { GroupCfg g = group_cfg<4>(C);
          hipLaunchKernelGGL(segsum_bwd_multi_kernel<4>, dim3(grid_for(npts, g.lg)), dim3(kThreads), 0, as_stream(stream),
                             mp, cell, npts, nbits, C, g.lg, mask, addend, gfeat); },
        { GroupCfg g = group_cfg<1>(C);
          hipLaunchKernelGGL(segsum_bwd_multi_kernel<1>, dim3(grid_for(npts, g.lg)), dim3(kThreads), 0, as_stream(stream),
                             mp, cell, npts, nbits, C, g.lg, mask, addend, gfeat); });
    return check_launch("segsum_bwd_multi");
}

T2H_API int t2h_segmean_bwd(const float *gplane_nhwc, const int32_t *cell, const int32_t *off0, int B, int N, int nbits,
                            int level, int C, float *gfeat, t2h_stream_t stream) {
    return t2h_segmean_bwd_add(gplane_nhwc, cell, off0, B, N, nbits, level, C, nullptr, gfeat, stream);
}

T2H_API int t2h_segmean_bwd_add(const float *gplane_nhwc, const int32_t *cell, const int32_t *off0, int B, int N, int nbits,
                                int level, int C, const float *addend, float *gfeat, t2h_stream_t stream) {
    if (!gplane_nhwc || !cell || !off0 || !gfeat) return fail(T2H_ERR_ARG, "segmean_bwd: null pointer");
    if (addend && C % 4 == 0 && ((uintptr_t)addend & 15)) return fail(T2H_ERR_ARG, "segmean_bwd: addend must be 16-byte aligned");
    int rc = check_level("segmean_bwd", B, nbits, level, C);
    if (rc) return rc;
    int64_t npts = rows_of(B, N);
    if (npts == 0) return T2H_OK;
    T2H_DISPATCH_VEC(C,
        { GroupCfg g = group_cfg<4>(C);
          hipLaunchKernelGGL(segmean_bwd_kernel<4>, dim3(grid_for(npts, g.lg)), dim3(kThreads), 0, as_stream(stream),
                             gplane_nhwc, cell, off0, npts, nbits, level, C, g.lg, addend, gfeat); },
        { GroupCfg g = group_cfg<1>(C);
          hipLaunchKernelGGL(segmean_bwd_kernel<1>, dim3(grid_for(npts, g.lg)), dim3(kThreads), 0, as_stream(stream),
                             gplane_nhwc, cell, off0, npts, nbits, level, C, g.lg, addend, gfeat); });
    return check_launch("segmean_bwd");
// ... 24 lines not shown
T2H_API int t2h_cell_order_build(const int32_t *off0, int B, int nbits, int level, int32_t *order, t2h_stream_t stream) {
    return t2h_cell_order_build_range(off0, B, nbits, level, level, order, stream);
}

T2H_API int t2h_cell_order_build_range(const int32_t *off0, int B, int nbits, int level_lo, int level_hi, int32_t *order,
                                       t2h_stream_t stream) {
    if (!off0 || !order) return fail(T2H_ERR_ARG, "cell_order_build: null pointer");
    if (level_lo > level_hi || t2h_cell_order_len(B, nbits, level_lo) == 0 || t2h_cell_order_len(B, nbits, level_hi) == 0)
        return fail(T2H_ERR_ARG, "cell_order_build: needs 0 <= level_lo <= level_hi < nbits");
    note_kernel("t2h::cell_order_kernel");
    hipLaunchKernelGGL(cell_order_kernel, dim3(2 * (level_hi - level_lo + 1)), dim3(1024), 0, as_stream(stream), off0, B, nbits,
                       level_lo, order);
    return check_launch("cell_order_build");
}

T2H_API int t2h_sample_relu_cellsums(const float *plane_nhwc, const float *pts, int dim, const int32_t *off0, int B, int N,
                                     int nbits, int level, int sum_level, int C, float *sums_nhwc, int ld_sums, void *sign_bits,
                                     t2h_stream_t stream) {
    return t2h_sample_relu_cellsums2(plane_nhwc, pts, dim, off0, B, N, nbits, level, sum_level, C, sums_nhwc, ld_sums, nullptr, 0,
                                     sign_bits, stream);
}

T2H_API int t2h_sample_relu_cellsums2(const float *plane_nhwc, const float *pts, int dim, const int32_t *off0, int B, int N,
                                      int nbits, int level, int sum_level, int C, float *sums_nhwc, int ld_sums,
                                      float *pooled_nhwc, int ld_pooled, void *sign_bits, t2h_stream_t stream) {
    return t2h_sample_relu_cellsums_ordered(plane_nhwc, pts, dim, off0, B, N, nbits, level, sum_level, C, sums_nhwc, ld_sums,
                                            pooled_nhwc, ld_pooled, sign_bits, nullptr, stream);
}

T2H_API int t2h_sample_relu_cellsums_ordered(const float *plane_nhwc, const float *pts, int dim, const int32_t *off0, int B, int N,
                                             int nbits, int level, int sum_level, int C, float *sums_nhwc, int ld_sums,
                                             float *pooled_nhwc, int ld_pooled, void *sign_bits, const int32_t *cell_order,
                                             t2h_stream_t stream) {
    if (!plane_nhwc || !pts || !off0 || !sums_nhwc) return fail(T2H_ERR_ARG, "sample_relu_cellsums: null pointer");
    if (pooled_nhwc && (sum_level >= level || ld_pooled < C || ld_pooled % 4 != 0 || ((uintptr_t)pooled_nhwc & 15)))
        return fail(T2H_ERR_ARG, "sample_relu_cellsums: the pooled sums need sum_level < level and 16-byte aligned rows of >= C floats");
    int rc = check_level("sample_relu_cellsums", B, nbits, level, C);
    if (rc) return rc;
    if (dim < 2 || sum_level < 0 || sum_level > level || C % 256 != 0 || ld_sums < C || ld_sums % 4 != 0 ||
        ((uintptr_t)plane_nhwc & 15) || ((uintptr_t)sums_nhwc & 15) || ((uintptr_t)sign_bits & 15))
        return fail(T2H_ERR_ARG, "sample_relu_cellsums: needs C %% 256 == 0, sum_level <= level, 16-byte aligned rows");
    if (rows_of(B, N) == 0) return fail(T2H_ERR_ARG, "sample_relu_cellsums: empty tile");
    if (level == nbits)
        return fail(T2H_ERR_ARG, "sample_relu_cellsums: needs level < nbits (a 1 x 1 plane: use t2h_sample_fwd_relu + t2h_segsum_fwd)");
    const int64_t cells = (int64_t)B << (2 * (nbits - level));
    const int chunks = C / 256;
    const int nchild = 1 << (2 * (level - sum_level));
    constexpr int64_t kMinWgs = 8192;
    const int npts_m1 = (int)(rows_of(B, N) - 1);
    unsigned long long *bw = static_cast<unsigned long long *>(sign_bits);
    const int quad = pooled_nhwc ? 4 : 1;
    note_kernel("t2h::sample_relu_cellsums_v2_kernel");
    const bool k0 = nchild >= 4 * quad;
    const int32_t *order_k0 = cell_order, *order_k1 = cell_order ? cell_order + cells : nullptr;
    int gz = 1;
    if (k0) while (nchild / (4 * gz * 2) >= quad && cells * chunks * gz < kMinWgs) gz *= 2;
    const dim3 grid((unsigned)((k0 ? cells : (cells >> 2)) * chunks * gz));
#define T2H_V2_LAUNCH(KK, PP) hipLaunchKernelGGL((sample_relu_cellsums_v2_kernel<KK, PP>), grid, dim3(256), 0, as_stream(stream), \
        plane_nhwc, pts, dim, off0, nbits, level, sum_level, C, sums_nhwc, ld_sums, bw, npts_m1, pooled_nhwc, ld_pooled, k0 ? order_k0 : order_k1, gz)
    if (k0) { if (pooled_nhwc) T2H_V2_LAUNCH(0, true); else T2H_V2_LAUNCH(0, false); }
    else { if (pooled_nhwc) T2H_V2_LAUNCH(1, true); else T2H_V2_LAUNCH(1, false); }
#undef T2H_V2_LAUNCH
    return check_launch("sample_relu_cellsums(v2)");
}

T2H_API int t2h_sample_bwd_from_sums(const float *const *gplanes_nhwc, const int *levels, const int *lds, int n_planes,
                                     const int32_t *cell, const void *mask, int mask_is_bits, const float *pts, int dim, const int32_t *off0, int B, int N, int nbits,
                                     int level, int C, float *gplane_nhwc, void *workspace, size_t workspace_bytes,
                                     t2h_stream_t stream) {
    return t2h_sample_bwd_from_sums_ordered(gplanes_nhwc, levels, lds, n_planes, cell, mask, mask_is_bits, pts, dim, off0, B, N, nbits,
                                            level, C, gplane_nhwc, workspace, workspace_bytes, nullptr, stream);
}

T2H_API int t2h_sample_bwd_from_sums_ordered(const float *const *gplanes_nhwc, const int *levels, const int *lds, int n_planes,
                                             const int32_t *cell, const void *mask, int mask_is_bits, const float *pts, int dim,
                                             const int32_t *off0, int B, int N, int nbits, int level, int C, float *gplane_nhwc,
                                             void *workspace, size_t workspace_bytes, const int32_t *cell_order,
                                             t2h_stream_t stream) {
    if (!gplanes_nhwc || !levels || !lds || !cell || !mask || !pts || !off0 || !gplane_nhwc)
        return fail(T2H_ERR_ARG, "sample_bwd_from_sums: null pointer");
    if (n_planes < 1 || n_planes > kMaxMultiPlanes)
        return fail(T2H_ERR_ARG, "sample_bwd_from_sums: 1..%d planes, got %d", kMaxMultiPlanes, n_planes);
    int rc = check_level("sample_bwd_from_sums", B, nbits, level, C);
    if (rc) return rc;
    if (dim < 2 || C % 4 != 0 || ((uintptr_t)mask & 15)) return fail(T2H_ERR_ARG, "sample_bwd_from_sums: unsupported shape");
    if (mask_is_bits && (C % 256 != 0 || !cells_mfma(C)))
        return fail(T2H_ERR_ARG, "sample_bwd_from_sums: packed sign bits need C %% 256 == 0 (and the matrix-core partials)");
    const float *maskf = static_cast<const float *>(mask);
    CoarsePlan cp = coarse_plan(B, N, nbits, level, C, kSampleBwdMinPts);
    if (!cp.use)
        return fail(T2H_ERR_ARG, "sample_bwd_from_sums: level %d holds too few points per cell for the per-cell partials "
                                 "(t2h_sample_bwd_workspace_bytes == 0): use t2h_segsum_bwd_multi + t2h_sample_bwd", level);
    size_t need = t2h_sample_bwd_workspace_bytes(B, N, nbits, level, C);
    if (!workspace || workspace_bytes < need)
        return fail(T2H_ERR_WORKSPACE, "sample_bwd_from_sums: workspace %zu < %zu bytes", workspace_bytes, need);
    MultiPlanes mp{};
    mp.n = n_planes;
    for (int q = 0; q < n_planes; ++q) {
        if (!gplanes_nhwc[q] || levels[q] < 0 || levels[q] > nbits || ((uintptr_t)gplanes_nhwc[q] & 15) || lds[q] < C || lds[q] % 4)
            return fail(T2H_ERR_ARG, "sample_bwd_from_sums: bad plane %d", q);
        mp.g[q] = gplanes_nhwc[q]; mp.level[q] = levels[q]; mp.ld[q] = lds[q];
    }
    int64_t groups = (int64_t)B << (2 * (nbits - level));
    float *partial = static_cast<float *>(workspace);
    int G = 1 << cp.lgG, P = kCellThreads >> cp.lgG;
    static const int table_on = getenv("T2H_CELLS_TABLE") ? atoi(getenv("T2H_CELLS_TABLE")) : 1;
    int tlevel = -1;
    if (table_on && C % 256 == 0) {
        int finest = nbits;
        for (int q = 0; q < n_planes; ++q) finest = levels[q] < finest ? levels[q] : finest;
        int tl = level - 2 > finest ? level - 2 : finest;
        if (tl < 0) tl = 0;
        if (tl > level) tl = level;
        const int64_t entries = (int64_t)1 << (2 * (level - tl));
        int folded = 0;
        for (int q = 0; q < n_planes; ++q) folded += levels[q] >= tl;
        const int64_t rows_per_wg = rows_of(B, N) / (groups * cp.S > 0 ? groups * cp.S : 1);
        if (folded > 0 && rows_per_wg * table_on >= entries) tlevel = tl;
    }
    if (mask_is_bits && level >= 1 && nbits - level >= 1 && n_planes <= kWalkPlanes) {
        int wl = level - 1;
        for (int q = 0; q < n_planes; ++q) wl = levels[q] < wl ? levels[q] : wl;
        const bool blocks = rows_of(B, N) < 64 * groups;
        const unsigned long long *bw = static_cast<const unsigned long long *>(mask);
        const int npts_m1 = (int)(rows_of(B, N) - 1);
        GroupCfg g = group_cfg<4>(C);
        const int32_t *order_k0 = cell_order, *order_k1 = cell_order ? cell_order + groups : nullptr;
        if (blocks) {
            hipLaunchKernelGGL(sample_bwd_walk_kernel<1>, dim3((unsigned)((groups >> 2) * (C / 256))), dim3(256), 0, as_stream(stream), pts,
                               dim, off0, nbits, level, wl, C, partial, mp, bw, npts_m1, order_k1);
            hipLaunchKernelGGL(sample_bwd_gather4_kernel, dim3(grid_for(groups, g.lg)), dim3(kThreads), 0, as_stream(stream), partial,
                               B, nbits - level, C, g.lg, gplane_nhwc);
        } else {
            hipLaunchKernelGGL(sample_bwd_walk_kernel<0>, dim3((unsigned)(groups * (C / 256))), dim3(256), 0, as_stream(stream), pts, dim,
                               off0, nbits, level, wl, C, partial, mp, bw, npts_m1, order_k0);
// ... 139 lines not shown
```

### tomosar2height_amd/csrc/t2h_common.h

```cpp
#pragma once
#include <hip/hip_runtime.h>
#include <stdint.h>
#include <stdio.h>
#include <stdarg.h>

#include "../../include/t2h.h"

#define T2H_API extern "C" __attribute__((visibility("default")))

namespace t2h {

constexpr int kWave = 64;

char *err_buf();
int fail(int code, const char *fmt, ...);
int check_launch(const char *what);
void note_kernel(const char *name);
const char *noted_kernel();

inline hipStream_t as_stream(t2h_stream_t s) { return reinterpret_cast<hipStream_t>(s); }

inline int64_t rows_of(int B, int N) { return N >= 0 ? (int64_t)B * N : -(int64_t)N; }
inline int rows_per_tile(int B, int N) { return N >= 0 ? N : (int)(-(int64_t)N / (B > 0 ? B : 1)); }

__host__ __device__ inline uint32_t part1by1(uint32_t v) {
    v &= 0x0000ffffu;
    v = (v | (v << 8)) & 0x00ff00ffu;
    v = (v | (v << 4)) & 0x0f0f0f0fu;
    v = (v | (v << 2)) & 0x33333333u;
    v = (v | (v << 1)) & 0x55555555u;
    return v;
}
__host__ __device__ inline uint32_t compact1by1(uint32_t v) {
    v &= 0x55555555u;
    v = (v | (v >> 1)) & 0x33333333u;
    v = (v | (v >> 2)) & 0x0f0f0f0fu;
    v = (v | (v >> 4)) & 0x00ff00ffu;
    v = (v | (v >> 8)) & 0x0000ffffu;
    return v;
}
__host__ __device__ inline uint32_t morton2(uint32_t x, uint32_t y) { return part1by1(x) | (part1by1(y) << 1); }

template <int VEC> struct Vec;
template <> struct Vec<4> {
    float v[4];
    __device__ static Vec load(const float *p) {
        float4 t = *reinterpret_cast<const float4 *>(p);
        Vec r; r.v[0] = t.x; r.v[1] = t.y; r.v[2] = t.z; r.v[3] = t.w; return r;
    }
    __device__ void store(float *p) const { *reinterpret_cast<float4 *>(p) = make_float4(v[0], v[1], v[2], v[3]); }
};
// ... 22 lines not shown
```

### tomosar2height_amd/csrc/tile_index.hip

```cpp
#include "t2h_common.h"

namespace t2h {

char *err_buf() {
    static thread_local char buf[256] = "no error";
    return buf;
}
int fail(int code, const char *fmt, ...) {
    va_list ap;
    va_start(ap, fmt);
    vsnprintf(err_buf(), 256, fmt, ap);
    va_end(ap);
    return code;
}
static thread_local const char *g_noted_kernel = "";
void note_kernel(const char *name) { g_noted_kernel = name; }
const char *noted_kernel() { return g_noted_kernel; }
int check_launch(const char *what) {
    hipError_t e = hipGetLastError();
    if (e != hipSuccess) return fail(T2H_ERR_LAUNCH, "%s: %s", what, hipGetErrorString(e));
    return T2H_OK;
}

constexpr int kMaxRagged = T2H_MAX_RAGGED_TILES;
struct Spans { int start[kMaxRagged + 1]; };
__device__ inline void tile_span(const Spans &sp, int N, int b, size_t &base, int &n) {
    if (N > 0) { base = (size_t)b * N; n = N; }
    else { base = (size_t)sp.start[b]; n = sp.start[b + 1] - sp.start[b]; }
}

constexpr int kSortThreads = 256;
constexpr int kSortItems = 8;
constexpr int kSortTile = kSortThreads * kSortItems;
constexpr int kSortWaves = kSortThreads / kWave;

__global__ void coordinate2index_kernel(const float *__restrict__ pts, int stride, int64_t total, int reso,
                                        int64_t *__restrict__ index) {
    int64_t i = (int64_t)blockIdx.x * blockDim.x + threadIdx.x;
    if (i >= total) return;
    float fx = __fmul_rn(pts[i * stride + 0], (float)reso);
    float fy = __fmul_rn(pts[i * stride + 1], (float)reso);
    int64_t ix = (int64_t)fx, iy = (int64_t)fy;
    index[i] = ix + (int64_t)reso * iy;
}

__global__ void tile_keys_kernel(const float *__restrict__ cloud, int dim, int N, Spans sp, int nbits,
                                 uint32_t *__restrict__ keys, int32_t *__restrict__ status) {
    int b = blockIdx.y;
    int i = blockIdx.x * blockDim.x + threadIdx.x;
    size_t base; int n;
// ... 119 lines not shown
    uint32_t key = keys[g], src = vals[g];
    const float *p = cloud + (tbase + src) * dim;
    float *q = pts_sorted + g * out_dim;
    for (int d = 0; d < dim; ++d) q[d] = p[d];
    if (out_dim > dim) q[out_dim - 1] = __int_as_float(b);
    perm[g] = (int32_t)src;
    cell[g] = b * M0 + (int32_t)key;
    int prev = (i == 0) ? -1 : (int)keys[g - 1];
    for (int m = prev + 1; m <= (int)key; ++m) off0[(size_t)b * M0 + m] = (int32_t)g;
    if (i == N - 1) {
        for (int m = (int)key + 1; m < M0; ++m) off0[(size_t)b * M0 + m] = (int32_t)(g + 1);
        if (b == B - 1) off0[(size_t)B * M0] = (int32_t)(g + 1);
    }
}

static size_t align256(size_t v) { return (v + 255) & ~(size_t)255; }

__global__ __launch_bounds__(256) void poison_lds_kernel(int words, unsigned *sink) {
    extern __shared__ unsigned lds_words[];
    for (int i = threadIdx.x; i < words; i += 256) lds_words[i] = 0x7fc00000u | (unsigned)(i & 0xffff);
    __syncthreads();
    for (int k = 0; k < 40; ++k) __builtin_amdgcn_s_sleep(127);
    if (lds_words[(threadIdx.x * 97) % words] == 1u) sink[0] = 1u;
}

}

using namespace t2h;

T2H_API int t2h_abi_version(void) { return T2H_ABI_VERSION; }
T2H_API const char *t2h_last_error_string(void) { return err_buf(); }
T2H_API const char *t2h_last_kernel_name(void) { return noted_kernel(); }
T2H_API void t2h_clear_kernel_name(void) { note_kernel(""); }

T2H_API int t2h_debug_poison_lds(t2h_stream_t stream) {
    static unsigned *sink = nullptr;
    static int bytes = 0;
    if (!sink) {
        if (hipMalloc(&sink, 256) != hipSuccess) return fail(T2H_ERR_LAUNCH, "debug_poison_lds: hipMalloc failed");
        bytes = 160 * 1024;
        if (hipFuncSetAttribute(reinterpret_cast<const void *>(poison_lds_kernel), hipFuncAttributeMaxDynamicSharedMemorySize, bytes) != hipSuccess) {
            (void)hipGetLastError();
            bytes = 64 * 1024;
        }
    }
    hipLaunchKernelGGL(poison_lds_kernel, dim3(512), dim3(256), (size_t)bytes, as_stream(stream), bytes / 4, sink);
    return check_launch("debug_poison_lds");
}

T2H_API int t2h_coordinate2index(const float *pts, int stride, int64_t total, int reso, int64_t *index,
                                 t2h_stream_t stream) {
    if (!pts || !index || stride < 2 || reso < 1 || total < 0) return fail(T2H_ERR_ARG, "coordinate2index: bad argument");
    if (total == 0) return T2H_OK;
    int64_t blocks = (total + 255) / 256;
    hipLaunchKernelGGL(coordinate2index_kernel, dim3((unsigned)blocks), dim3(256), 0, as_stream(stream), pts, stride,
                       total, reso, index);
    return check_launch("coordinate2index");
}

static size_t tile_ws_bytes(int B, size_t rows, int max_n, int nbits) {
    int nblk = (max_n + kSortTile - 1) / kSortTile;
    if (nblk < 1) nblk = 1;
    return 4 * align256((rows > 0 ? rows : 1) * sizeof(uint32_t)) + align256((size_t)B * 256 * nblk * sizeof(uint32_t));
}

T2H_API size_t t2h_tile_workspace_bytes(int B, int N, int nbits) {
// ... 95 lines not shown
```

### tomosar2height_amd/deferred.py

```python
import ctypes
import os

import torch

from . import _lib, mlp, ops

DEFER_MIN_CHANNELS = int(os.environ.get("T2H_DEFER_MIN_CHANNELS", "128"))
FUSED_SAMPLE_BWD = os.environ.get("T2H_FUSED_SAMPLE_BWD", "1") != "0"
CELLS_MFMA = os.environ.get("T2H_CELLS_MFMA", "1") != "0"
SIGN_BITS = os.environ.get("T2H_SIGN_BITS", "1") != "0"
ON_CHIP_HIDDEN = os.environ.get("T2H_ON_CHIP_HIDDEN", "1") != "0"
ON_CHIP_MIN_PTS_PER_CELL = float(os.environ.get("T2H_ON_CHIP_MIN_PTS", "8"))


def _segsum_into(tile, rows, level, dst):
    n, c = rows.shape
    r = tile.R >> level
    ws_bytes = _lib.ws_bytes("t2h_segmean_workspace_bytes", tile.B, tile.N, tile.nbits, level, c)
    ws = _lib.workspace(ws_bytes, rows.device)
    _lib.call("t2h_segsum_fwd", _lib.ptr(rows), _lib.ptr(tile.off0), tile.B, tile.N, tile.nbits, level, c, dst.data_ptr(),
              dst.stride(0), _lib.ptr(ws), ws_bytes, _lib.stream(), nbytes=4 * c * n + 4 * n + 4 * c * tile.B * r * r,
              tag=_lib.timing() and f"t2h_segsum_fwd[C={c},r={r}]")


def _sumpool_into(tile, fine, level_fine, coarse):
    c = fine.shape[1]
    r = tile.R >> level_fine
    _lib.call("t2h_plane_sumpool2x2", fine.data_ptr(), fine.stride(0), tile.B, r, c, coarse.data_ptr(), coarse.stride(0),
              _lib.stream(), nbytes=5 * c * tile.B * r * r, tag=_lib.timing() and f"t2h_plane_sumpool2x2[C={c}]")


def _plane_args(planes):
    arr = (ctypes.c_void_p * len(planes))(*[p.data_ptr() for p, _ in planes])
    lvs = (ctypes.c_int * len(planes))(*[lv for _, lv in planes])
    lds = (ctypes.c_int * len(planes))(*[p.stride(0) for p, _ in planes])
    return ctypes.cast(arr, ctypes.c_void_p), ctypes.cast(lvs, ctypes.c_void_p), ctypes.cast(lds, ctypes.c_void_p)


def _gather(tile, planes, c, mask=None):
    out = torch.empty(tile.n_points, c, dtype=torch.float32, device=tile.device)
    arr, lvs, lds = _plane_args(planes)
    _lib.call("t2h_segsum_bwd_multi", arr, lvs, lds, len(planes), _lib.ptr(tile.cell), tile.B, tile.N, tile.nbits, c,
              None if mask is None else _lib.ptr(mask), None, _lib.ptr(out), _lib.stream(),
              nbytes=4 * c * tile.n_points * (2 if mask is not None else 1) + 4 * tile.n_points
              + sum(4 * c * p.shape[0] for p, _ in planes), tag=_lib.timing() and f"t2h_segsum_bwd_multi[C={c},n={len(planes)}]")
    return out


def counts(tile, level):
    cache = tile.__dict__.setdefault("_cell_counts", {})
    if level not in cache:
        r = tile.R >> level
        cnt = torch.empty(tile.B * r * r, dtype=torch.float32, device=tile.device)
        _lib.call("t2h_cell_counts", _lib.ptr(tile.off0), tile.B, tile.nbits, level, _lib.ptr(cnt), _lib.stream(),
                  nbytes=12 * cnt.numel())
        cache[level] = cnt
    return cache[level]


class _ComposeStack(torch.autograd.Function):

    @staticmethod
    def forward(ctx, a_prev, wc, w1):
        ck, cprev = wc.shape
        k2 = w1.shape[1]
        rows_prev = cprev if a_prev is None else a_prev.shape[0]
        out = torch.empty(rows_prev + k2, ck, dtype=torch.float32, device=wc.device)
        wc_c, w1_c = wc.contiguous(), w1.contiguous()
        if a_prev is None:
            _transpose(wc_c, out[:rows_prev])
        else:
            a_prev = a_prev.contiguous()
            mlp.linear_fwd_(a_prev, wc_c, None, out[:rows_prev])
        _transpose(w1_c, out[rows_prev:])
        ctx.has_prev = a_prev is not None
        ctx.rows_prev = rows_prev
        ctx.wc_param = wc
        ctx.save_for_backward(a_prev if a_prev is not None else wc_c, wc_c)
        return out
# ... 20 lines not shown
def _transpose(src, dst):
    ops.nchw_to_nhwc_(src, 1, src.shape[0], src.shape[1], dst)


def _compose_step(a_prev, const_prev, params):
    wc, bc, w1, b1 = params
    a_all = _ComposeStack.apply(a_prev, wc, w1)
    return a_all, ((bc + b1).reshape(1, -1) if const_prev is None else mlp.linear(const_prev, wc, bc) + b1.reshape(1, -1))


class _DeferredLevel(torch.autograd.Function):

    @staticmethod
    def forward(ctx, q_rows, a_all, const, base_rows, state, idx, r):
        tile = state.tile
        q_rows, a_all, const = q_rows.contiguous(), a_all.contiguous(), const.contiguous()
        c2 = q_rows.shape[1]
        if idx == 0:
            state.write_sums(0, base_rows.contiguous())
        need_bwd = any(ctx.needs_input_grad[:4])
        bits_ok = (SIGN_BITS and c2 % 256 == 0 and FUSED_SAMPLE_BWD and CELLS_MFMA and tile.n_points > 0 and
                   _lib.ws_bytes("t2h_sample_bwd_workspace_bytes", tile.B, tile.N, tile.nbits, tile.level(r), c2) > 0)
        on_chip = (bits_ok if need_bwd else (c2 % 256 == 0 and tile.n_points > 0)) and ON_CHIP_HIDDEN and tile.level(r) < tile.nbits
        on_chip = on_chip and tile.n_points >= ON_CHIP_MIN_PTS_PER_CELL * tile.B * r * r
        want_bits = need_bwd and (on_chip or bits_ok)
        bits = torch.empty(tile.n_points * (c2 // 256) * 4, dtype=torch.int64, device=q_rows.device) if want_bits else None
        if on_chip:
            levels = state.needed(idx + 1)
            finest = state.sums(idx + 1, levels[0])
            second = None
            if len(levels) > 1 and levels[1] == levels[0] + 1 and levels[0] < tile.level(r):
                second = state.sums(idx + 1, levels[1])
            order = tile.cell_order(tile.level(r))
            _lib.call("t2h_sample_relu_cellsums_ordered", _lib.ptr(q_rows), _lib.ptr(tile.pts), tile.dim, _lib.ptr(tile.off0), tile.B,
                      tile.N, tile.nbits, tile.level(r), levels[0], c2, finest.data_ptr(), finest.stride(0),
                      None if second is None else second.data_ptr(), 0 if second is None else second.stride(0),
                      None if bits is None else _lib.ptr(bits), None if order is None else _lib.ptr(order), _lib.stream(),
                      nbytes=4 * q_rows.numel() + 12 * tile.n_points + 4 * c2 * finest.shape[0]
                      + (0 if bits is None else (c2 // 8) * tile.n_points) + (0 if second is None else 4 * c2 * second.shape[0]),
                      tag=_lib.timing() and f"t2h_sample_relu_cellsums[C={c2},r={r}]")
            state.pool_down(idx + 1, start=1 if second is not None else 0)
            return _DeferredLevel._finish(ctx, state, idx, r, a_all, const, bits, True)
        h = torch.empty(tile.n_points, c2, dtype=torch.float32, device=q_rows.device)
        ops.sample_fwd_relu_(tile, q_rows, r, h, bits)
        state.write_sums(idx + 1, h)
        return _DeferredLevel._finish(ctx, state, idx, r, a_all, const, h if bits is None else bits, bits is not None)

    @staticmethod
    def _finish(ctx, state, idx, r, a_all, const, saved_mask, mask_is_bits):
        tile = state.tile
        lv = state.levels_seq[idx]
        k = state.off[idx + 2]
        if a_all.shape[0] != k:
            raise RuntimeError(f"deferred level {idx}: {a_all.shape[0]} composed rows for {k} source columns")
        x = state.S[lv][:, :k]
        acc = torch.empty(x.shape[0], a_all.shape[1], dtype=torch.float32, device=x.device)
        mlp.linear_dgrad_(x, a_all, acc, bx3=True)
        cnt = counts(tile, lv)
        out = torch.empty_like(acc)
        _lib.call("t2h_mean_bias_fwd", _lib.ptr(acc), _lib.ptr(cnt), _lib.ptr(const), acc.shape[0], acc.shape[1], _lib.ptr(out),
                  _lib.stream(), nbytes=8 * acc.numel() + 4 * acc.shape[0])
        ctx.state, ctx.idx, ctx.r, ctx.has_base = state, idx, r, idx == 0
        ctx.const_shape = const.shape
        ctx.mask_is_bits = mask_is_bits
        ctx.save_for_backward(saved_mask, a_all)
        return out, a_all.as_strided(a_all.size(), a_all.stride(), a_all.storage_offset())

    @staticmethod
    def backward(ctx, g, ga_thru):
        h, a_all = ctx.saved_tensors
        state, idx, r = ctx.state, ctx.idx, ctx.r
        tile = state.tile
        lv = state.levels_seq[idx]
        k = state.off[idx + 2]
        g = g.contiguous()
        p, c = g.shape
        cnt = counts(tile, lv)
        dacc = torch.empty_like(g)
        cached = state.cache is not None and not ctx.needs_input_grad[1]
        dconst = torch.empty(ctx.const_shape, dtype=torch.float32, device=g.device) if (ctx.needs_input_grad[2] or cached) else None
        ws_bytes = _lib.ws_bytes("t2h_mean_bias_bwd_workspace_bytes", p, c)
        ws = _lib.workspace(ws_bytes, g.device)
        _lib.call("t2h_mean_bias_bwd", _lib.ptr(g), _lib.ptr(cnt), p, c, _lib.ptr(dacc), None if dconst is None else _lib.ptr(dconst),
                  _lib.ptr(ws), ws_bytes, _lib.stream(), nbytes=8 * p * c + 4 * p)
        x = state.S[lv][:, :k]
        da = ga_thru
        if cached:
            e = state.cache.levels[idx]
            e.ready.wait()
            mlp.linear_wgrad_(x, dacc, e.ga, None, accumulate=True, defer=True)
            e.gconst.add_(dconst)
            dconst = None
            state.cache.pending = True
        elif ctx.needs_input_grad[1]:
            if ga_thru is not None and ga_thru.is_contiguous() and ga_thru.dtype == torch.float32 and mlp.sole_owner(ga_thru):
                mlp.linear_wgrad_(x, dacc, ga_thru, None, accumulate=True)
            else:
                da = torch.empty_like(a_all)
                mlp.linear_wgrad_(x, dacc, da, None)
                if ga_thru is not None:
                    da = da + ga_thru
        dS, seen = state.grad_matrix(lv)
        if seen and seen < k:
            raise RuntimeError("deferred backward out of order")
        mlp.linear_fwd_(dacc, a_all, None, dS[:, :k], accumulate=bool(seen), bx3=True)
        state.dS_cols[lv] = max(seen, k)
        lo, hi = state.off[idx + 1], state.off[idx + 2]
        planes = [(state.dS[l][:, lo:hi], l) for l in state.needed(idx + 1)]
        dq = None
        if ctx.needs_input_grad[0]:
            dq = state.hidden_grad(planes, h, r, hi - lo, ctx.mask_is_bits)
        dbase = None
        if ctx.has_base and ctx.needs_input_grad[3]:
            lo0, hi0 = state.off[0], state.off[1]
            dbase = _gather(tile, [(state.dS[l][:, lo0:hi0], l) for l in state.needed(0)], hi0 - lo0)
        return dq, da, dconst, dbase, None, None, None


class _CachedLevel:
    __slots__ = ("params", "versions", "a_all", "const", "ga", "gconst", "ready")

    def __init__(self, params, versions, a_all, const):
        self.params, self.versions, self.a_all, self.const = params, versions, a_all, const
        self.ga, self.gconst, self.ready = torch.zeros_like(a_all), torch.zeros_like(const), _lib.Ready()


class ComposeCache:

    def __init__(self):
        self.levels = []
        self.pending = False

    def _compute(self, idx, params):
        prev = self.levels[idx - 1] if idx > 0 else None
        with torch.no_grad():
            return _compose_step(None if prev is None else prev.a_all, None if prev is None else prev.const, params)

    def get(self, idx, params):
        params = tuple(params)
        if idx > len(self.levels):
            raise RuntimeError("ComposeCache: levels must be requested in order")
        ver = tuple(p._version for p in params)
        if idx == len(self.levels):
            self.levels.append(_CachedLevel(params, ver, *self._compute(idx, params)))
            self.levels[idx].ready.mark()
            return self.levels[idx].a_all, self.levels[idx].const
        e = self.levels[idx]
        if any(p is not q for p, q in zip(e.params, params)):
# ... 28 lines not shown
            e.versions = None
            self.get(idx, e.params)

    def drop_accumulated(self):
        for e in self.levels:
            e.ga.zero_()
            e.gconst.zero_()
        self.pending = False

    def flush(self):
        if not self.levels:
            return
        outs, a_all, const = [], None, None
        with torch.enable_grad():
            for e in self.levels:
                a_all, const = _compose_step(a_all, const, e.params)
                outs += [a_all, const]
            torch.autograd.backward(outs, [g.clone() for e in self.levels for g in (e.ga, e.gconst)])
        self.drop_accumulated()


class Deferred:

    def __init__(self, tile, levels_seq, channels_seq, base_rows, cache=None):
        self.tile = tile
        self.cache = cache
        self.levels_seq = list(levels_seq)
        ks = [base_rows.shape[1]] + [2 * c for c in channels_seq]
        self.off = [0]
        for kk in ks:
            self.off.append(self.off[-1] + kk)
        self.base = base_rows
        self.S, self.dS, self.dS_cols = {}, {}, {}
        self.a_all, self.const = None, None
        self.n_done = 0

    def needed(self, src):
        first = 0 if src == 0 else src - 1
        return sorted(set(self.levels_seq[first:]))

    def _matrix(self, store, lv):
        if lv not in store:
            r = self.tile.R >> lv
            store[lv] = torch.empty(self.tile.B * r * r, self.off[-1], dtype=torch.float32, device=self.tile.device)
        return store[lv]

    def sums(self, src, lv):
        return self._matrix(self.S, lv)[:, self.off[src]:self.off[src + 1]]

    def grad_matrix(self, lv):
        return self._matrix(self.dS, lv), self.dS_cols.get(lv, 0)

    def write_sums(self, src, rows):
        finest = self.needed(src)[0]
        _segsum_into(self.tile, rows, finest, self.sums(src, finest))
        self.pool_down(src)

    def pool_down(self, src, start=0):
        levels = self.needed(src)
        cur_level = levels[start]
        cur = self.sums(src, cur_level)
        for lv in levels[start + 1:]:
            while cur_level < lv:
                nxt_level = cur_level + 1
                if nxt_level in levels:
                    nxt = self.sums(src, nxt_level)
                else:
                    rn = self.tile.R >> nxt_level
                    nxt = torch.empty(self.tile.B * rn * rn, cur.shape[1], dtype=torch.float32, device=cur.device)
                _sumpool_into(self.tile, cur, cur_level, nxt)
                cur, cur_level = nxt, nxt_level

    def hidden_grad(self, planes, h, r, c2, mask_is_bits=False):
        tile = self.tile
        level = tile.level(r)
        ws_bytes = _lib.ws_bytes("t2h_sample_bwd_workspace_bytes", tile.B, tile.N, tile.nbits, level, c2)
        if mask_is_bits or (FUSED_SAMPLE_BWD and ws_bytes > 0 and c2 % 4 == 0):
            arr, lvs, lds = _plane_args(planes)
            ws = _lib.workspace(ws_bytes, h.device)
            dq = torch.empty(tile.B * r * r, c2, dtype=torch.float32, device=h.device)
            order = tile.cell_order(level) if mask_is_bits else None
            _lib.call("t2h_sample_bwd_from_sums_ordered", arr, lvs, lds, len(planes), _lib.ptr(tile.cell), _lib.ptr(h),
                      1 if mask_is_bits else 0, _lib.ptr(tile.pts), tile.dim, _lib.ptr(tile.off0), tile.B, tile.N, tile.nbits,
                      level, c2, _lib.ptr(dq), _lib.ptr(ws), ws_bytes, None if order is None else _lib.ptr(order), _lib.stream(),
                      nbytes=(c2 // 8 if mask_is_bits else 4 * c2) * tile.n_points + 12 * tile.n_points + 4 * dq.numel()
                      + sum(4 * c2 * p.shape[0] for p, _ in planes), tag=_lib.timing() and f"t2h_sample_bwd_from_sums[C={c2},r={r}]")
            return dq
        dh = _gather(tile, planes, c2, mask=h)
        return ops._sample_bwd(tile, dh, r, c2, None).reshape(tile.B * r * r, c2)

    def advance(self, q_rows, r, fc_b, fc_c):
        idx = self.n_done
        if self.tile.level(r) != self.levels_seq[idx]:
            raise RuntimeError("deferred levels out of order")
        params = (fc_c.weight, fc_c.bias, fc_b.weight, fc_b.bias)
        if self.cache is not None:
            a_all, const = self.cache.get(idx, params)
        else:
            a_all, const = self.a_all, self.const = _compose_step(self.a_all, self.const, params)
        raster, a_thru = _DeferredLevel.apply(q_rows, a_all, const, self.base if idx == 0 else None, self, idx, r)
        self.n_done += 1
        if self.cache is None:
            last = self.n_done == len(self.levels_seq)
            self.a_all, self.const = (None, None) if last else (a_thru, const)
        return raster


def applicable(tile, r: int, c: int) -> bool:
    return DEFER_MIN_CHANNELS > 0 and c >= DEFER_MIN_CHANNELS and mlp.grid_first_applicable(tile, r, c)
```

### tomosar2height_amd/mlp.py

```python
import contextlib
import ctypes
import os
from typing import Optional

import torch

from . import _lib, ops
from .ops import _rows, pool_max_fwd_ as _pool_fwd_


_MODE = "fp32"


def set_precision(name: str):
    global _MODE
    if name not in ("fp32", "bf16", "bf16x3"):
        raise ValueError("precision must be 'fp32', 'bf16' or 'bf16x3'")
    _MODE = name


def get_precision() -> str:
    return _MODE


def trunk_precision() -> str:
    return "fp32 (fused trunk block kernel)" if (FUSED_TRUNK or _MODE == "fp32") else _MODE


def _pflag() -> int:
    return {"fp32": 0, "bf16": _lib.BF16, "bf16x3": _lib.BF16X3}[_MODE]


GEMM_BX3 = os.environ.get("T2H_GEMM_BX3", "1") != "0"


_BX3_MIN_N = int(os.environ.get("T2H_GEMM_BX3_MIN_N", "64"))
_BX3_MIN_K = int(os.environ.get("T2H_GEMM_BX3_MIN_K", "128"))
_GEMM_BX3_WGRAD = os.environ.get("T2H_GEMM_BX3_WGRAD", "0") == "1"
_BX3_WGRAD_MIN_N = int(os.environ.get("T2H_GEMM_BX3_WGRAD_MIN_N", "1024"))
_BX3_WGRAD_MIN_M = int(os.environ.get("T2H_GEMM_BX3_WGRAD_MIN_M", "4096"))
_PERSIST_N = os.environ.get("T2H_BX3_PERSIST_N", "1") != "0"


def _bx3_gemm_ok(m, k, n, *rows, force=False) -> bool:
    if not (GEMM_BX3 and _MODE == "fp32" and bool(_lib.ws_bytes("t2h_gemm_bx3_supported", m, k, n))
            and all(t is None or (t.stride(0) % 4 == 0 and t.data_ptr() % 16 == 0) for t in rows)):
        return False
    min_n, min_k = _BX3_MIN_N, _BX3_MIN_K
    wide_short = _PERSIST_N and k == 64 and n >= 512 and m >= 4096
    return force or wide_short or (n >= min_n and k >= min_k and m >= 4096)


def _gemm_bx3(x, w, w_is_kn, bias, mask, y, relu_out, accumulate, tag):
    from . import grid
    (xp, ldx), (yp, ldy) = _rows(x, "gemm_bx3 x"), _rows(y, "gemm_bx3 y")
    m, k = x.shape
    n = y.shape[1]
    mp, ldm = (None, 0) if mask is None else _rows(mask, "gemm_bx3 mask")
    nws = _lib.ws_bytes("t2h_gemm_bx3_workspace_bytes", m, k, n)
    ws = _lib.workspace(nws, x.device)
    flags = (_lib.RELU_OUT if relu_out else 0) | (_lib.ACCUM if accumulate else 0) | (_lib.F16X2 if grid._h2() else 0)
    _lib.call("t2h_gemm_bx3", xp, ldx, _lib.ptr(grid.split_weights.get_gemm(w, w_is_kn)), bias.data_ptr() if bias is not None else None,
              mp, ldm, yp, ldy, m, k, n, flags, _lib.ptr(ws), nws, _lib.stream(),
              nbytes=4 * (m * k + m * n + n * k + (m * n if mask is not None else 0)), flops=2 * m * k * n, tag=_lib.timing() and tag)
    return y


def linear_fwd_(x, w, bias, y, relu_in=False, relu_out=False, accumulate=False, bx3=False):
    (xp, ldx), (yp, ldy) = _rows(x, "linear_fwd x"), _rows(y, "linear_fwd y")
    m, k = x.shape
    n = w.shape[0]
    if bx3 and not relu_in and w.is_contiguous() and _bx3_gemm_ok(m, k, n, x, y):
        return _gemm_bx3(x, w, False, bias, None, y, relu_out, accumulate, f"t2h_linear_fwd[K={k},N={n}]")
    w = w.contiguous()
    flags = (_lib.RELU_IN if relu_in else 0) | (_lib.RELU_OUT if relu_out else 0) | (_lib.ACCUM if accumulate else 0) | _pflag()
    _lib.call("t2h_linear_fwd", xp, ldx, w.data_ptr(), bias.data_ptr() if bias is not None else None, yp, ldy, m, k, n,
              flags, _lib.stream(), nbytes=4 * (m * k + m * n + n * k), flops=2 * m * k * n,
              tag=_lib.timing() and f"t2h_linear_fwd[K={k},N={n}]")
    return y


def linear_dgrad_(dy, w, dx, mask=None, accumulate=False, bx3=False):
    (gp, ldg), (dp, ldd) = _rows(dy, "linear_dgrad dy"), _rows(dx, "linear_dgrad dx")
    m, n = dy.shape
    k = w.shape[1]
    if bx3 and w.is_contiguous() and _bx3_gemm_ok(m, n, k, dy, dx, mask):
        return _gemm_bx3(dy, w, True, None, mask, dx, False, accumulate, f"t2h_linear_dgrad[N={n},K={k}]")
    w = w.contiguous()
    mp, ldm = (None, 0) if mask is None else _rows(mask, "linear_dgrad mask")
    _lib.call("t2h_linear_dgrad", gp, ldg, w.data_ptr(), dp, ldd, m, k, n, mp, ldm,
              (_lib.ACCUM if accumulate else 0) | _pflag(),
              _lib.stream(), nbytes=4 * (m * k + m * n + n * k + (m * k if mask is not None else 0)),
              flops=2 * m * k * n, tag=_lib.timing() and f"t2h_linear_dgrad[N={n},K={k}]")
    return dx


def _grid_h2() -> bool:
    from . import grid
    return grid._h2()


def linear_wgrad_(dy, x, dw, db, relu_in=False, accumulate=False, defer=False):
    (gp, ldg), (xp, ldx) = _rows(dy, "linear_wgrad dy"), _rows(x, "linear_wgrad x")
    m, n = dy.shape
    k = x.shape[1]
    if not dw.is_contiguous() or (db is not None and not db.is_contiguous()):
        raise ValueError("linear_wgrad: dw / db must be contiguous")
    if m == 0:
        if not accumulate:
            dw.zero_()
            if db is not None:
                db.zero_()
        return
    bx3 = (_GEMM_BX3_WGRAD and GEMM_BX3 and _MODE == "fp32" and not relu_in and n >= _BX3_WGRAD_MIN_N and m >= _BX3_WGRAD_MIN_M
           and _grid_h2() and bool(_lib.ws_bytes("t2h_gemm_bx3_wgrad_supported", m, k, n)))
    query, pflags = (("t2h_gemm_bx3_wgrad_workspace_bytes", _lib.F16X2) if bx3 else
                     ("t2h_linear_wgrad_workspace_bytes", (_lib.RELU_IN if relu_in else 0) | _pflag()))
    ws_bytes = _lib.ws_bytes(query, m, k, n)
    ws = _lib.workspace(ws_bytes, dy.device)
    flags = pflags | (_lib.ACCUM if accumulate else 0) | (_lib.defer_reduce(ws, dw) if defer else 0)
    outs = (dw.data_ptr(), db.data_ptr() if db is not None else None)
    cost = dict(nbytes=4 * (m * k + m * n + n * k), flops=2 * m * k * n, tag=_lib.timing() and f"t2h_linear_wgrad[N={n},K={k}]")
    if bx3:
        _lib.call("t2h_gemm_bx3_wgrad", gp, ldg, xp, ldx, m, k, n, *outs, flags, ws.data_ptr(), ws_bytes, _lib.stream(), **cost)
    else:
        _lib.call("t2h_linear_wgrad", gp, ldg, xp, ldx, m, k, n, flags, *outs, ws.data_ptr(), ws_bytes, _lib.stream(), **cost)


class direct_grad_accumulation:
    __slots__ = ("enabled", "side_stream", "conv_side_stream", "main_stream", "held", "prev")

    def __init__(self, enabled: bool = True, side_stream=None, conv_side_stream=None):
        self.enabled = enabled
        self.side_stream = side_stream if enabled else None
        self.conv_side_stream = conv_side_stream if enabled else None
        self.main_stream, self.held = None, []

    def __enter__(self):
        global _PASS
        self.prev, _PASS = _PASS, self
        self.main_stream, self.held = self.prev.main_stream, self.prev.held
        if self.side_stream is not None or self.conv_side_stream is not None:
            self.main_stream = torch.cuda.current_stream()
        return self

    def __exit__(self, *exc):
        global _PASS
        if self.main_stream is not None and self.prev.main_stream is None:
            for st in {id(s): s for s in (self.side_stream, self.conv_side_stream) if s is not None}.values():
                self.main_stream.wait_stream(st)
            self.held.clear()
        _PASS = self.prev


_PASS = direct_grad_accumulation(False)


def direct_accum() -> bool:
# ... 498 lines not shown
```

### tomosar2height_amd/tile.py

```python
import torch

from . import _lib


def _log2_exact(v: int) -> int:
    if v < 1 or v & (v - 1):
        raise ValueError(f"plane resolution must be a power of two, got {v}")
    return v.bit_length() - 1


class TileIndex:

    def __init__(self, cloud, plane_resolution: int, status: torch.Tensor = None):
        if isinstance(cloud, (list, tuple)):
            self._init_ragged(cloud, plane_resolution, status)
            return
        if cloud.dim() != 3 or cloud.shape[-1] < 2:
            raise ValueError(f"expected a [B, N, dim>=2] point tensor, got {tuple(cloud.shape)}")
        if cloud.dtype != torch.float32:
            raise TypeError("points must be float32")
        self.R = int(plane_resolution)
        self.nbits = _log2_exact(self.R)
        if not 1 <= self.nbits <= 10:
            raise ValueError("plane resolution must be in [2, 1024]")
# ... 105 lines not shown
            lo, hi = 1, min(3, self.nbits - 1)
            if not (lo <= level <= hi):
                lo = hi = level
            lens = [int(lib.t2h_cell_order_len(self.B, self.nbits, lv)) for lv in range(lo, hi + 1)]
            if min(lens) > 0 and self.n_points > 0:
                buf = torch.empty(sum(lens), dtype=torch.int32, device=self.device)
                _lib.call("t2h_cell_order_build_range", _lib.ptr(self.off0), self.B, self.nbits, lo, hi, _lib.ptr(buf),
                          _lib.stream(), nbytes=16 * sum(lens))
                at = 0
                for lv, n in zip(range(lo, hi + 1), lens):
                    self._adjoint[("order", lv)] = buf[at:at + n]
                    at += n
            else:
                for lv in range(lo, hi + 1):
                    self._adjoint[("order", lv)] = None
            hit = self._adjoint[("order", level)]
        return hit

    @property
    def n_points(self) -> int:
        return -self.N if self.N < 0 else self.B * self.N

    @classmethod
    def prebuild(cls, cloud: torch.Tensor, plane_resolution: int, status: torch.Tensor = None, stream=None):
        if stream is None:
            return cls(cloud, plane_resolution, status=status)
        main = torch.cuda.current_stream(cloud.device)
        stream.wait_stream(main)
        with torch.cuda.stream(stream):
            tile = cls(cloud, plane_resolution, status=status)
            from . import ops, deferred
            if ops.SAMPLE_ADJOINT and 0 < tile.n_points <= ops.SAMPLE_ADJOINT_MAX_ROWS * tile.B * tile.R * tile.R:
                tile.sample_adjoint(0)
            for lv in range(min(4, tile.nbits)):
                deferred.counts(tile, lv)
                if lv >= 1:
                    tile.cell_order(lv)
            tile.ready = torch.cuda.Event()
            tile.ready.record(stream)
        cloud.record_stream(stream)
        for t in tile._tensors():
            t.record_stream(main)
        return tile

    def _tensors(self):
        out = [self.pts, self.perm, self.cell, self.off0]
        for key, val in self._adjoint.items():
            if isinstance(key, tuple):
                out += [val] if val is not None else []
            else:
                out += list(val)
        out += list(self.__dict__.get("_cell_counts", {}).values())
        return out

    def wait_ready(self):
        ev = self.__dict__.pop("ready", None)
        if ev is not None:
            torch.cuda.current_stream(self.device).wait_event(ev)
        return self

    def to(self, device=None, *args, **kwargs):
        if device is not None and torch.device(device).type != self.device.type:
            raise ValueError("a TileIndex cannot be moved between devices")
        return self

    def level(self, reso: int) -> int:
        k = self.nbits - _log2_exact(int(reso))
        if k < 0:
            raise ValueError(f"plane resolution {reso} is finer than the tile's {self.R}")
        return k

    def out_of_domain(self) -> int:
        return int(self.status[0].item())

    def check_domain(self):
        bad = self.out_of_domain()
        if bad:
            raise ValueError(f"{bad} point(s) have x or y outside [0, 1): normalise the tile first")

    def sort_rows(self, feat: torch.Tensor) -> torch.Tensor:
        if self.N < 0:
            raise NotImplementedError("sort_rows / unsort_rows: equal-N batches only (test / interop helpers)")
        b, n, c = feat.shape
        idx = (self.perm.long() + torch.arange(b, device=feat.device).repeat_interleave(n) * n)
        return feat.reshape(b * n, c)[idx].contiguous()
# ... 8 lines not shown
```

Baseline: 189.5 tiles/s.

## Compact deferred cell sums to occupied cells and bound GEMM rows by a device count

Builds a compacted row list of occupied plane cells (a count, scan and fill kernel chain) and stores the deferred segment sums only for occupied cells. The GEMMs on those sums read a device-side row count: forward bx3 tiles past the limit exit early and wgrad clamps its K range. The mean/bias kernels remap rows through the cell-to-row map. This avoids GEMM work on the many empty cells of a sparse point cloud. It adds prefix-scan kernels, a global side channel for passing compaction state, and disables the kwaves and bx3 wgrad paths when a limit is set.

```diff
diff --git a/include/t2h.h b/include/t2h.h
--- a/include/t2h.h
+++ b/include/t2h.h
@@ -65,6 +65,7 @@
 int t2h_segsum_bwd_multi(const float *const *gplanes_nhwc, const int *levels, const int *lds, int n_planes, const int32_t *cell,
                          int B, int N, int nbits, int C, const float *mask, const float *addend, float *gfeat,
                          t2h_stream_t stream);
+void t2h_compact_next(const int32_t *row_of_cell, int level, const int32_t *n_rows);
 int t2h_cell_counts(const int32_t *off0, int B, int nbits, int level, float *cnt, t2h_stream_t stream);
 int t2h_mean_bias_fwd(const float *acc, const float *cnt, const float *cvec, int64_t P, int C, float *out, t2h_stream_t stream);
 size_t t2h_mean_bias_bwd_workspace_bytes(int64_t P, int C);
diff --git a/tomosar2height_amd/_lib.py b/tomosar2height_amd/_lib.py
--- a/tomosar2height_amd/_lib.py
+++ b/tomosar2height_amd/_lib.py
@@ -15,6 +15,7 @@
     "t2h_last_kernel_name": (ctypes.c_char_p, []),
     "t2h_clear_kernel_name": (None, []),
     "t2h_debug_poison_lds": (_i, [_vp]),
+    "t2h_compact_next": (None, [_vp, _i, _vp]),
     "t2h_coordinate2index": (_i, [_vp, _i, _i64, _i, _vp, _vp]),
     "t2h_tile_workspace_bytes": (_sz, [_i, _i, _i]),
     "t2h_tile_build": (_i, [_vp, _i, _i, _i, _i, _vp, _vp, _vp, _vp, _vp, _vp, _sz, _vp]),
@@ -369,6 +370,10 @@
     check(rc, name)
 
 
+def compact_next(row_of_cell, level: int, n_rows):
+    load().t2h_compact_next(row_of_cell, level, n_rows)
+
+
 def ptr(t: torch.Tensor) -> int:
     return t.data_ptr()
 
diff --git a/tomosar2height_amd/csrc/conv_bx3.hip b/tomosar2height_amd/csrc/conv_bx3.hip
--- a/tomosar2height_amd/csrc/conv_bx3.hip
+++ b/tomosar2height_amd/csrc/conv_bx3.hip
@@ -206,6 +206,7 @@
     const float *addend;
     int up_logW, up_logH, up_cout;
     const float *r1_g, *r1_w;
+    const int *row_limit;
 };
 
 __device__ inline size_t up_pixel(long long m, int tap, int logW, int logH) {
@@ -255,6 +256,11 @@
     const int x0 = tx * TW, y0 = ty * TH;
     int n0 = tn_lo * BN;
     const int c_beg = split * p.chunks_per_split, c_end = min(p.Kc / CCH, c_beg + p.chunks_per_split);
+    int row_lim = 0x7fffffff;
+    if (NTAP == 1 && UPM == 0 && p.row_limit) {
+        row_lim = __builtin_amdgcn_readfirstlane(*p.row_limit);
+        if ((b * p.H + y0) * p.W + x0 >= row_lim) return;
+    }
 
     constexpr int NF4 = HP * F4, PER = (NF4 + NT - 1) / NT;
     float4 hreg[PER];
@@ -271,7 +277,8 @@
                 if (idx < NF4)
                     v = *reinterpret_cast<const float4 *>(p.x + up_pixel(((long long)b * p.H + gy) * p.W + gx, tap, p.up_logW, p.up_logH) *
                                                                     p.ldx + co0 + c4 * 4);
-            } else if (idx < NF4 && (unsigned)gy < (unsigned)p.H && (unsigned)gx < (unsigned)p.W)
+            } else if (idx < NF4 && (unsigned)gy < (unsigned)p.H && (unsigned)gx < (unsigned)p.W &&
+                       (NTAP != 1 || (b * p.H + gy) * p.W + gx < row_lim))
                 v = *reinterpret_cast<const float4 *>(p.x + (((size_t)b * p.H + gy) * p.W + gx) * p.ldx + c * CCH + c4 * 4);
             hreg[f] = v;
         }
@@ -1108,6 +1115,7 @@
 
 T2H_API int t2h_gemm_bx3(const float *x, int ldx, const void *wf, const float *bias, const float *mask, int ldm, float *y, int ldy,
                          int64_t M, int K, int N, int flags, void *workspace, size_t workspace_bytes, t2h_stream_t stream) {
+    const CompactRows cr = take_compact();
     if (!x || !wf || !y) return fail(T2H_ERR_ARG, "gemm_bx3: null pointer");
     if (!t2h_gemm_bx3_supported(M, K, N))
         return fail(T2H_ERR_ARG, "gemm_bx3: needs M %% 128 == 0, K %% 64 == 0, N %% 32 == 0 (M=%lld K=%d N=%d)", (long long)M, K, N);
@@ -1119,6 +1127,7 @@
     a.B = 1; a.H = (int)(M / 32); a.W = 32; a.Kc = K; a.Nc = N; a.ldx = ldx; a.ldy = ldy; a.ldm = ldm;
     a.flags = ((flags & T2H_RELU_OUT) ? F_RELU_OUT : 0) | ((flags & T2H_ACCUM) ? F_ACCUM : 0);
     a.wscale = f16_trailer(wf, (size_t)K * N * 4);
+    a.row_limit = cr.n_rows;
     return launch_rows(a, npl_of(flags), workspace, workspace_bytes, as_stream(stream), "gemm_bx3", 1);
 }
 
diff --git a/tomosar2height_amd/csrc/deferred.hip b/tomosar2height_amd/csrc/deferred.hip
--- a/tomosar2height_amd/csrc/deferred.hip
+++ b/tomosar2height_amd/csrc/deferred.hip
@@ -16,16 +16,86 @@
     cnt[i] = (float)(off0[obase + ((size_t)1 << (2 * level))] - off0[obase]);
 }
 
+constexpr int kRowBlock = 2048;
+__device__ inline int cell_occupied(const int32_t *__restrict__ off0, int nbits, int level, int rbits, int64_t i) {
+    const int r = 1 << rbits;
+    const int x = (int)(i & (r - 1)), y = (int)((i >> rbits) & (r - 1));
+    const int64_t b = i >> (2 * rbits);
+    const size_t obase = ((size_t)b << (2 * nbits)) + ((size_t)morton2((uint32_t)x, (uint32_t)y) << (2 * level));
+    return off0[obase + ((size_t)1 << (2 * level))] > off0[obase] ? 1 : 0;
+}
+__device__ inline int scan256(int v, int *sh, int &total) {
+    const int tid = threadIdx.x;
+    sh[tid] = v;
+    __syncthreads();
+    for (int off = 1; off < 256; off <<= 1) {
+        const int add = tid >= off ? sh[tid - off] : 0;
+        __syncthreads();
+        sh[tid] += add;
+        __syncthreads();
+    }
+    const int incl = sh[tid];
+    total = sh[255];
+    __syncthreads();
+    return incl - v;
+}
+__global__ __launch_bounds__(256) void cell_rows_count_kernel(const int32_t *__restrict__ off0, int nbits, int level, int64_t total,
+                                                             int32_t *__restrict__ blockcnt) {
+    __shared__ int sh[256];
+    const int rbits = nbits - level;
+    const int64_t i0 = (int64_t)blockIdx.x * kRowBlock + threadIdx.x * 8;
+    int n = 0;
+    for (int j = 0; j < 8; ++j)
+        if (i0 + j < total) n += cell_occupied(off0, nbits, level, rbits, i0 + j);
+    int sum;
+    scan256(n, sh, sum);
+    if (threadIdx.x == 0) blockcnt[blockIdx.x] = sum;
+}
+__global__ __launch_bounds__(256) void cell_rows_scan_kernel(int32_t *__restrict__ blockcnt, int nblk, int32_t *__restrict__ n_rows) {
+    __shared__ int sh[256];
+    int carry = 0;
+    for (int base = 0; base < nblk; base += 256) {
+        const int j = base + threadIdx.x;
+        const int v = j < nblk ? blockcnt[j] : 0;
+        int sum;
+        const int ex = scan256(v, sh, sum);
+        if (j < nblk) blockcnt[j] = carry + ex;
+        carry += sum;
+    }
+    if (threadIdx.x == 0) n_rows[0] = carry;
+}
+__global__ __launch_bounds__(256) void cell_rows_fill_kernel(const int32_t *__restrict__ off0, int nbits, int level, int64_t total,
+                                                            const int32_t *__restrict__ blockcnt, int32_t *__restrict__ row_of_cell,
+                                                            int32_t *__restrict__ cell_of_row) {
+    __shared__ int sh[256];
+    const int rbits = nbits - level;
+    const int64_t i0 = (int64_t)blockIdx.x * kRowBlock + threadIdx.x * 8;
+    int occ[8], n = 0;
+    for (int j = 0; j < 8; ++j) {
+        occ[j] = i0 + j < total ? cell_occupied(off0, nbits, level, rbits, i0 + j) : 0;
+        n += occ[j];
+    }
+    int sum;
+    int row = blockcnt[blockIdx.x] + scan256(n, sh, sum);
+    for (int j = 0; j < 8; ++j)
+        if (i0 + j < total) {
+            row_of_cell[i0 + j] = occ[j] ? row : -1;
+            if (occ[j]) { cell_of_row[row] = (int32_t)(i0 + j); ++row; }
+        }
+}
+
 __global__ __launch_bounds__(256) void mean_bias_fwd_kernel(const float *__restrict__ acc, const float *__restrict__ cnt,
                                                            const float *__restrict__ cvec, int64_t total4, int C4,
-                                                           float *__restrict__ out) {
+                                                           float *__restrict__ out, const int32_t *__restrict__ rows) {
     const int64_t t = (int64_t)blockIdx.x * 256 + threadIdx.x;
     if (t >= total4) return;
     const int64_t p = t / C4;
     const int c4 = (int)(t % C4);
     const float n = cnt[p];
     const float den = n > 0.f ? n : 1.f, ne = n > 0.f ? 1.f : 0.f;
-    const float4 a = reinterpret_cast<const float4 *>(acc)[t];
+    float4 a = make_float4(0.f, 0.f, 0.f, 0.f);
+    if (!rows) a = reinterpret_cast<const float4 *>(acc)[t];
+    else if (n > 0.f) a = reinterpret_cast<const float4 *>(acc)[(int64_t)rows[p] * C4 + c4];
     const float4 cv = reinterpret_cast<const float4 *>(cvec)[c4];
     float4 o;
     o.x = __fadd_rn(__fdiv_rn(a.x, den), __fmul_rn(ne, cv.x)); o.y = __fadd_rn(__fdiv_rn(a.y, den), __fmul_rn(ne, cv.y));
@@ -40,7 +110,8 @@
 }
 __global__ __launch_bounds__(256) void mean_bias_bwd_kernel(const float *__restrict__ g, const float *__restrict__ cnt,
                                                            int64_t P, int C, float *__restrict__ dacc,
-                                                           float *__restrict__ slab, int kMbRows) {
+                                                           float *__restrict__ slab, int kMbRows,
+                                                           const int32_t *__restrict__ rowmap) {
     __shared__ float4 red[256];
     const int C4 = C / 4;
     const int cols = min(C4, 256), slots = 256 / cols;
@@ -54,9 +125,10 @@
             for (int i = slot; i < rows; i += slots) {
                 const float n = cnt[p0 + i];
                 const float4 v = reinterpret_cast<const float4 *>(g + (size_t)(p0 + i) * C)[c4];
-                if (dacc) {
+                const int64_t drow = rowmap ? (n > 0.f ? (int64_t)rowmap[p0 + i] : -1) : p0 + i;
+                if (dacc && drow >= 0) {
                     const float den = n > 0.f ? n : 1.f;
-                    reinterpret_cast<float4 *>(dacc + (size_t)(p0 + i) * C)[c4] =
+                    reinterpret_cast<float4 *>(dacc + (size_t)drow * C)[c4] =
                         make_float4(__fdiv_rn(v.x, den), __fdiv_rn(v.y, den), __fdiv_rn(v.z, den), __fdiv_rn(v.w, den));
                 }
                 if (n > 0.f) { s.x += v.x; s.y += v.y; s.z += v.z; s.w += v.w; }
@@ -82,25 +154,38 @@
 using namespace t2h;
 
 T2H_API int t2h_cell_counts(const int32_t *off0, int B, int nbits, int level, float *cnt, t2h_stream_t stream) {
+    const CompactRows rows = take_compact();
     if (!off0 || !cnt) return fail(T2H_ERR_ARG, "cell_counts: null pointer");
     if (B < 1 || nbits < 1 || nbits > T2H_MAX_NBITS || level < 0 || level > nbits) return fail(T2H_ERR_ARG, "cell_counts: bad level");
     const int64_t total = (int64_t)B << (2 * (nbits - level));
     hipLaunchKernelGGL(cell_counts_kernel, dim3((unsigned)((total + 255) / 256)), dim3(256), 0, as_stream(stream), off0, B, nbits,
                        level, cnt);
-    return check_launch("cell_counts");
+    if (int rc = check_launch("cell_counts")) return rc;
+    if (!rows.row_of_cell) return T2H_OK;
+    if (rows.level != level || !rows.n_rows || rows.n_rows != rows.row_of_cell + 2 * total)
+        return fail(T2H_ERR_ARG, "cell_counts: the row list asked for is not this level's (level %d, asked %d)", level, rows.level);
+    int32_t *row_of_cell = const_cast<int32_t *>(rows.row_of_cell), *n_rows = const_cast<int32_t *>(rows.n_rows);
+    int32_t *blockcnt = n_rows + 4;
+    const int nblk = (int)((total + kRowBlock - 1) / kRowBlock);
+    hipLaunchKernelGGL(cell_rows_count_kernel, dim3(nblk), dim3(256), 0, as_stream(stream), off0, nbits, level, total, blockcnt);
+    hipLaunchKernelGGL(cell_rows_scan_kernel, dim3(1), dim3(256), 0, as_stream(stream), blockcnt, nblk, n_rows);
+    hipLaunchKernelGGL(cell_rows_fill_kernel, dim3(nblk), dim3(256), 0, as_stream(stream), off0, nbits, level, total, blockcnt,
+                       row_of_cell, row_of_cell + total);
+    return check_launch("cell_counts/rows");
 }
 
 static bool al16(const void *p) { return ((uintptr_t)p & 15) == 0; }
 
 T2H_API int t2h_mean_bias_fwd(const float *acc, const float *cnt, const float *cvec, int64_t P, int C, float *out,
                               t2h_stream_t stream) {
+    const CompactRows rows = take_compact();
     if (!acc || !cnt || !cvec || !out) return fail(T2H_ERR_ARG, "mean_bias_fwd: null pointer");
     if (P < 0 || C < 4 || C % 4 != 0 || !al16(acc) || !al16(cvec) || !al16(out))
         return fail(T2H_ERR_ARG, "mean_bias_fwd: needs C %% 4 == 0 and 16-byte aligned rows");
     if (P == 0) return T2H_OK;
     const int64_t total4 = P * (C / 4);
     hipLaunchKernelGGL(mean_bias_fwd_kernel, dim3((unsigned)((total4 + 255) / 256)), dim3(256), 0, as_stream(stream), acc, cnt,
-                       cvec, total4, C / 4, out);
+                       cvec, total4, C / 4, out, rows.row_of_cell);
     return check_launch("mean_bias_fwd");
 }
 
@@ -112,6 +197,7 @@
 
 T2H_API int t2h_mean_bias_bwd(const float *g, const float *cnt, int64_t P, int C, float *dacc, float *dcvec, void *workspace,
                               size_t workspace_bytes, t2h_stream_t stream) {
+    const CompactRows rows = take_compact();
     if (!g || !cnt) return fail(T2H_ERR_ARG, "mean_bias_bwd: null pointer");
     if (P < 1 || C < 4 || C % 4 != 0 || !al16(g) || (dacc && !al16(dacc)) || (dcvec && !al16(dcvec)))
         return fail(T2H_ERR_ARG, "mean_bias_bwd: needs P >= 1, C %% 4 == 0 and 16-byte aligned rows");
@@ -122,7 +208,8 @@
     const int kMbRows = mb_rows(P);
     const int blocks = (int)((P + kMbRows - 1) / kMbRows);
     float *slab = dcvec ? static_cast<float *>(workspace) : nullptr;
-    hipLaunchKernelGGL(mean_bias_bwd_kernel, dim3(blocks), dim3(256), 0, as_stream(stream), g, cnt, P, C, dacc, slab, kMbRows);
+    hipLaunchKernelGGL(mean_bias_bwd_kernel, dim3(blocks), dim3(256), 0, as_stream(stream), g, cnt, P, C, dacc, slab, kMbRows,
+                       rows.row_of_cell);
     if (int rc = check_launch("mean_bias_bwd")) return rc;
     if (!dcvec) return T2H_OK;
     return launch_reduce_slabs(slab, blocks, C, 1, C, C, 0, dcvec, nullptr, nullptr, as_stream(stream));
diff --git a/tomosar2height_amd/csrc/gemm.hip b/tomosar2height_amd/csrc/gemm.hip
--- a/tomosar2height_amd/csrc/gemm.hip
+++ b/tomosar2height_amd/csrc/gemm.hip
@@ -35,8 +35,13 @@
         split = t / (gridDim.x * gridDim.y);
     }
     const int m0 = tile_m * BM, n0 = tile_n * BN;
-    const int kbeg = split * p.k_chunk;
-    const int kend = min(p.K, kbeg + p.k_chunk);
+    int K = p.K, k_chunk = p.k_chunk;
+    if (p.k_limit) {
+        K = min(K, __builtin_amdgcn_readfirstlane(*p.k_limit));
+        k_chunk = min(k_chunk, ((K + (int)gridDim.z - 1) / (int)gridDim.z + 31) / 32 * 32);
+    }
+    const int kbeg = split * k_chunk;
+    const int kend = min(K, kbeg + k_chunk);
     const bool relu_a = p.flags & F_RELU_A, relu_b = p.flags & F_RELU_B;
 
     TileLoader<BM, NT, A_KC, BK> la;
@@ -667,6 +672,7 @@
 
 T2H_API int t2h_linear_wgrad(const float *dy, int lddy, const float *x, int ldx, int M, int K, int N, int flags,
                              float *dw, float *db, void *workspace, size_t workspace_bytes, t2h_stream_t stream) {
+    const CompactRows cr = take_compact();
     if (!dy || !x || !dw) return fail(T2H_ERR_ARG, "linear_wgrad: null pointer");
     if (M < 1 || K < 1 || N < 1 || lddy < N || ldx < K) return fail(T2H_ERR_ARG, "linear_wgrad: bad shape");
     size_t need = t2h_linear_wgrad_workspace_bytes(M, K, N);
@@ -679,6 +685,7 @@
     int accumulate = (flags & T2H_ACCUM) ? 1 : 0;
     const bool direct = !p.smallk && p.splits == 1 && !accumulate && !db && aligned4(dw, K);
     if (direct) slab = dw;
+    if (p.smallk && cr.n_rows) return fail(T2H_ERR_ARG, "linear_wgrad: a row limit needs K %% 4 == 0");
     if (p.smallk) {
         if (K > kSmallKMax) return fail(T2H_ERR_ARG, "linear_wgrad: K=%d must be a multiple of 4 (or <= %d)", K, kSmallKMax);
         hipLaunchKernelGGL(wgrad_smallk_kernel, dim3(p.splits), dim3(256), 0, s, dy, lddy, x, ldx, M, K, N,
@@ -690,10 +697,11 @@
         a.A = dy; a.lda = lddy; a.B = x; a.ldb = ldx; a.C = slab; a.ldc = K; a.colsum = db ? colslab : nullptr;
         a.M = N; a.N = K; a.K = M; a.flags = (flags & T2H_RELU_IN) ? F_RELU_B : 0;
         a.k_chunk = p.k_chunk; a.slab_stride = (long long)N * K;
+        a.k_limit = cr.n_rows;
         int rc;
         const int mode = mode_of(flags);
         static const int kwaves_wgrad_max_rows = [] { const char *e = getenv("T2H_KWAVES_WGRAD_MAX_ROWS"); return e ? atoi(e) : 1024; }();
-        if (mode == 0 && !db && M <= kwaves_wgrad_max_rows && aligned4(dw, K) && kwaves_applicable(N, K, M)) {
+        if (!a.k_limit && mode == 0 && !db && M <= kwaves_wgrad_max_rows && aligned4(dw, K) && kwaves_applicable(N, K, M)) {
             a.C = dw; a.colsum = nullptr; a.k_chunk = M; a.slab_stride = 0;
             if (accumulate) a.flags |= F_ACCUM;
             return launch_gemm_kwaves<false, false>(a, s, "linear_wgrad");
@@ -703,7 +711,8 @@
      : mode == 1 ? launch_gemm<BM_, BN_, WM_, WN_, false, false, 16, true, (MW_ > 3 ? 3 : MW_), 1>(a, p.splits, s, "linear_wgrad") \
                  : launch_gemm<BM_, BN_, WM_, WN_, false, false, 16, true, MW_, 0>(a, p.splits, s, "linear_wgrad"))
         static const bool tn_dma = !(getenv("T2H_GEMM_DMA") && getenv("T2H_GEMM_DMA")[0] == '0');
-        if (p.bm == 128 && p.bn == 128 && mode == 0 && tn_dma && gemm_dma_tn_applicable(a))
+        if (a.k_limit && mode != 0) return fail(T2H_ERR_ARG, "linear_wgrad: a row limit needs the fp32 kernels");
+        if (p.bm == 128 && p.bn == 128 && mode == 0 && tn_dma && !a.k_limit && gemm_dma_tn_applicable(a))
             rc = launch_gemm_dma_tn(a, p.splits, s, "linear_wgrad");
         else if (p.bm == 128 && p.bn == 128)
             rc = mode != 0 ? launch_gemm_split(mode, false, false, a, p.splits, s, "linear_wgrad") : T2H_WG(128, 128, 2, 2, 4);
diff --git a/tomosar2height_amd/csrc/gemm_args.h b/tomosar2height_amd/csrc/gemm_args.h
--- a/tomosar2height_amd/csrc/gemm_args.h
+++ b/tomosar2height_amd/csrc/gemm_args.h
@@ -18,6 +18,7 @@
     int flags;
     int k_chunk;
     long long slab_stride;
+    const int *k_limit;
 };
 
 int launch_gemm_split(int mode, bool a_kc, bool b_kc, const GemmArgs &a, int splits, hipStream_t s, const char *what);
diff --git a/tomosar2height_amd/csrc/point_grid.hip b/tomosar2height_amd/csrc/point_grid.hip
--- a/tomosar2height_amd/csrc/point_grid.hip
+++ b/tomosar2height_amd/csrc/point_grid.hip
@@ -348,7 +348,7 @@
 __global__ __launch_bounds__(kThreads) void segmean_fwd_kernel(const float *__restrict__ feat,
                                                                const int32_t *__restrict__ off0, int B, int nbits,
                                                                int level, int C, int lg, float *__restrict__ plane,
-                                                               int ld_out) {
+                                                               int ld_out, const int32_t *__restrict__ rowmap) {
     int64_t t = (int64_t)blockIdx.x * kThreads + threadIdx.x;
     int64_t gid = t >> lg;
     const int rbits = nbits - level;
@@ -360,7 +360,12 @@
     int s = off0[obase], e = off0[obase + ((size_t)1 << (2 * level))];
     int cx = (int)compact1by1(mk), cy = (int)compact1by1(mk >> 1);
     int r = 1 << rbits;
-    float *orow = plane + (((size_t)b * r + cy) * r + cx) * ld_out;
+    int64_t orow_i = ((int64_t)b * r + cy) * r + cx;
+    if (rowmap) {
+        if (e <= s) return;
+        orow_i = rowmap[orow_i];
+    }
+    float *orow = plane + (size_t)orow_i * ld_out;
     float inv_den = (float)(e - s > 0 ? e - s : 1);
     int span = VEC << lg;
     for (int c = ((int)t & ((1 << lg) - 1)) * VEC; c < C; c += span) {
@@ -389,7 +394,20 @@
 }
 
 constexpr int kMaxMultiPlanes = 8;
-struct MultiPlanes { const float *g[kMaxMultiPlanes]; int level[kMaxMultiPlanes]; int ld[kMaxMultiPlanes]; int n; };
+struct MultiPlanes {
+    const float *g[kMaxMultiPlanes]; int level[kMaxMultiPlanes]; int ld[kMaxMultiPlanes]; int n;
+    int cq = -1; const int32_t *rowmap = nullptr; int cells = 0;
+};
+__device__ inline int plane_row(const MultiPlanes &mp, int q, int ci) {
+    if (q == mp.cq) ci = mp.rowmap[ci];
+    return ci;
+}
+static void set_compact(MultiPlanes &mp, const CompactRows &cr, int B, int nbits) {
+    mp.cq = -1; mp.rowmap = nullptr; mp.cells = 0;
+    if (!cr.row_of_cell) return;
+    for (int q = 0; q < mp.n; ++q)
+        if (mp.level[q] == cr.level) { mp.cq = q; mp.rowmap = cr.row_of_cell; mp.cells = B << (2 * (nbits - cr.level)); }
+}
 template <int VEC>
 __global__ __launch_bounds__(kThreads) void segsum_bwd_multi_kernel(MultiPlanes mp, const int32_t *__restrict__ cell,
                                                                     int64_t npts, int nbits, int C, int lg,
@@ -408,7 +426,7 @@
         rows[q] = nullptr;
         if (q < mp.n) {
             const int l = mp.level[q], r = 1 << (nbits - l);
-            rows[q] = mp.g[q] + (((size_t)b * r + (y0 >> l)) * r + (x0 >> l)) * mp.ld[q];
+            rows[q] = mp.g[q] + (size_t)plane_row(mp, q, (int)((b * r + (y0 >> l)) * r + (x0 >> l))) * mp.ld[q];
         }
     }
     const int span = VEC << lg;
@@ -436,7 +454,8 @@
 }
 
 __global__ __launch_bounds__(kThreads) void plane_sumpool2x2_kernel(const float *__restrict__ fine, int64_t total4, int rc,
-                                                                   int C4, int ld_in, int ld_out, float *__restrict__ coarse) {
+                                                                   int C4, int ld_in, int ld_out, float *__restrict__ coarse,
+                                                                   const int32_t *__restrict__ rowmap) {
     int64_t t = (int64_t)blockIdx.x * kThreads + threadIdx.x;
     if (t >= total4) return;
     const int c4 = (int)(t % C4);
@@ -444,10 +463,22 @@
     const int x = (int)(pix % rc), y = (int)((pix / rc) % rc);
     const int64_t b = pix / ((int64_t)rc * rc);
     const int rf = 2 * rc;
-    const float *f = fine + ((b * rf + 2 * y) * rf + 2 * x) * (int64_t)ld_in + 4 * c4;
-    const float4 a = *reinterpret_cast<const float4 *>(f), bq = *reinterpret_cast<const float4 *>(f + ld_in);
-    const float4 cq = *reinterpret_cast<const float4 *>(f + (int64_t)rf * ld_in);
-    const float4 d = *reinterpret_cast<const float4 *>(f + (int64_t)rf * ld_in + ld_in);
+    const int64_t fc = (b * rf + 2 * y) * rf + 2 * x;
+    float4 a, bq, cq, d;
+    if (rowmap) {
+        const float4 z = make_float4(0.f, 0.f, 0.f, 0.f);
+        const int r0 = rowmap[fc], r1 = rowmap[fc + 1], r2 = rowmap[fc + rf], r3 = rowmap[fc + rf + 1];
+        a = z; bq = z; cq = z; d = z;
+        if (r0 >= 0) a = *reinterpret_cast<const float4 *>(fine + (int64_t)r0 * ld_in + 4 * c4);
+        if (r1 >= 0) bq = *reinterpret_cast<const float4 *>(fine + (int64_t)r1 * ld_in + 4 * c4);
+        if (r2 >= 0) cq = *reinterpret_cast<const float4 *>(fine + (int64_t)r2 * ld_in + 4 * c4);
+        if (r3 >= 0) d = *reinterpret_cast<const float4 *>(fine + (int64_t)r3 * ld_in + 4 * c4);
+    } else {
+        const float *f = fine + fc * (int64_t)ld_in + 4 * c4;
+        a = *reinterpret_cast<const float4 *>(f); bq = *reinterpret_cast<const float4 *>(f + ld_in);
+        cq = *reinterpret_cast<const float4 *>(f + (int64_t)rf * ld_in);
+        d = *reinterpret_cast<const float4 *>(f + (int64_t)rf * ld_in + ld_in);
+    }
     float4 o;
     o.x = (a.x + bq.x) + (cq.x + d.x); o.y = (a.y + bq.y) + (cq.y + d.y);
     o.z = (a.z + bq.z) + (cq.z + d.z); o.w = (a.w + bq.w) + (cq.w + d.w);
@@ -588,7 +619,8 @@
                                                                         int sum_level, int C, float *__restrict__ sums,
                                                                         int ld_sums, unsigned long long *__restrict__ bits,
                                                                         int npts_m1, float *__restrict__ sums2, int ld_sums2,
-                                                                        const int32_t *__restrict__ order, int gz) {
+                                                                        const int32_t *__restrict__ order, int gz,
+                                                                        const int32_t *__restrict__ rowmap) {
     constexpr int SIDE = 3 + K, NS = SIDE * SIDE;
     __shared__ float4 T[NS][64];
     const int tid = threadIdx.x, lane = tid & 63, wave = tid >> 6;
@@ -692,7 +724,9 @@
             const float4 sum = make_float4(sum01.x, sum01.y, sum23.x, sum23.y);
             const uint32_t cm = (uint32_t)(cb + c);
             const int fx = (cx << d) + (int)compact1by1(cm), fy = (cy << d) + (int)compact1by1(cm >> 1);
-            *reinterpret_cast<float4 *>(sums + (((size_t)b * rs + fy) * rs + fx) * ld_sums + c0) = sum;
+            int srow = (b * rs + fy) * rs + fx;
+            if (rowmap) srow = e > s ? __builtin_amdgcn_readfirstlane(rowmap[srow]) : -1;
+            if (srow >= 0) *reinterpret_cast<float4 *>(sums + (size_t)srow * ld_sums + c0) = sum;
             if (POOL) {
                 const unsigned k4 = cm & 3u;
                 if (k4 == 0u) pe = sum;
@@ -983,7 +1017,8 @@
 __global__ __launch_bounds__(kThreads) void segmean_finalize_kernel(const float *__restrict__ partial,
                                                                    const int32_t *__restrict__ off0, int B, int nbits,
                                                                    int level, int C, int lg, int S,
-                                                                   float *__restrict__ plane, int mean = 1, int ld_out = 0) {
+                                                                   float *__restrict__ plane, int mean = 1, int ld_out = 0,
+                                                                   const int32_t *__restrict__ rowmap = nullptr) {
     int64_t t = (int64_t)blockIdx.x * kThreads + threadIdx.x;
     int64_t gid = t >> lg;
     const int rbits = nbits - level;
@@ -995,7 +1030,12 @@
     int cnt = off0[obase + ((size_t)1 << (2 * level))] - off0[obase];
     float den = (float)(cnt > 0 ? cnt : 1);
     int cx = (int)compact1by1(mk), cy = (int)compact1by1(mk >> 1), r = 1 << rbits;
-    float *orow = plane + (((size_t)b * r + cy) * r + cx) * (ld_out > 0 ? ld_out : C);
+    int64_t orow_i = ((int64_t)b * r + cy) * r + cx;
+    if (rowmap) {
+        if (cnt <= 0) return;
+        orow_i = rowmap[orow_i];
+    }
+    float *orow = plane + (size_t)orow_i * (ld_out > 0 ? ld_out : C);
     for (int c = ((int)t & ((1 << lg) - 1)) * 4; c < C; c += 4 << lg) {
         float4 acc = make_float4(0.f, 0.f, 0.f, 0.f);
         for (int sp = 0; sp < S; ++sp) {
@@ -1048,7 +1088,8 @@
                 for (int q = 0; q < kMaxMultiPlanes; ++q)
                     if (q < mp.n) {
                         const int l = mp.level[q], rq = 1 << (nbits - l);
-                        const float4 u = *reinterpret_cast<const float4 *>(mp.g[q] + (((size_t)fb * rq + (fy >> l)) * rq + (fx >> l)) * mp.ld[q] + c);
+                        const float4 u = *reinterpret_cast<const float4 *>(
+                            mp.g[q] + (size_t)plane_row(mp, q, (int)((fb * rq + (fy >> l)) * rq + (fx >> l))) * mp.ld[q] + c);
                         if (q == 0) g = u;
                         else { g.x = __fadd_rn(g.x, u.x); g.y = __fadd_rn(g.y, u.y); g.z = __fadd_rn(g.z, u.z); g.w = __fadd_rn(g.w, u.w); }
                     }
@@ -1147,8 +1188,9 @@
                 for (int q = 0; q < kMaxMultiPlanes; ++q)
                     if (q < mp.n && mp.level[q] >= tlevel) {
                         const int l = mp.level[q], rq = 1 << (nbits - l), sh = l - tlevel;
-                        const float4 w = *reinterpret_cast<const float4 *>(
-                            mp.g[q] + (((size_t)b * rq + (ty >> sh)) * rq + (tx >> sh)) * mp.ld[q] + che);
+                        const int prow = plane_row(mp, q, (int)((b * rq + (ty >> sh)) * rq + (tx >> sh)));
+                        if (prow < 0) continue;
+                        const float4 w = *reinterpret_cast<const float4 *>(mp.g[q] + (size_t)prow * mp.ld[q] + che);
                         v.x = __fadd_rn(v.x, w.x); v.y = __fadd_rn(v.y, w.y); v.z = __fadd_rn(v.z, w.z); v.w = __fadd_rn(v.w, w.w);
                     }
                 Tl[t][c4] = v;
@@ -1192,7 +1234,7 @@
                 for (int q = 0; q < kMaxMultiPlanes; ++q)
                     if (q < mp.n) {
                         const int l = mp.level[q], rq = 1 << (nbits - l);
-                        Po[tid][q] = (int)((fb * rq + (fy >> l)) * rq + (fx >> l));
+                        Po[tid][q] = plane_row(mp, q, (int)((fb * rq + (fy >> l)) * rq + (fx >> l)));
                     }
                 if (tlevel >= 0) Ti[tid] = (int)((fm >> (2 * tlevel)) & ((1u << (2 * (level - tlevel))) - 1u));
             }
@@ -1310,6 +1352,7 @@
             if (q < mp.n) {
                 const int sh = mp.level[q] - wl, rq = 1 << (nbits - mp.level[q]);
                 prow_l[q] = (b * rq + (fy >> sh)) * rq + (fx >> sh);
+                if (q == mp.cq) prow_l[q] = mp.rowmap[min(max(prow_l[q], 0), mp.cells - 1)];
             }
     };
     auto request = [&](int c) {
@@ -1688,8 +1731,11 @@
 }
 
 static int segreduce_fwd(bool mean, const float *feat, const int32_t *off0, int B, int N, int nbits, int level, int C,
-                         float *plane_nhwc, int ld_out, void *workspace, size_t workspace_bytes, t2h_stream_t stream) {
+                         float *plane_nhwc, int ld_out, void *workspace, size_t workspace_bytes, t2h_stream_t stream,
+                         const CompactRows &cr = CompactRows{}) {
     if (!feat || !off0 || !plane_nhwc) return fail(T2H_ERR_ARG, "segmean_fwd: null pointer");
+    if (cr.row_of_cell && cr.level != level) return fail(T2H_ERR_ARG, "segsum_fwd: compact rows of level %d asked for level %d", cr.level, level);
+    const int32_t *rowmap = cr.row_of_cell;
     if (ld_out < C || (C % 4 == 0 && ld_out % 4 != 0)) return fail(T2H_ERR_ARG, "segmean_fwd: plane row stride %d < C = %d", ld_out, C);
     int rc = check_level("segmean_fwd", B, nbits, level, C);
     if (rc) return rc;
@@ -1706,25 +1752,25 @@
                            partial);
         GroupCfg g = group_cfg<4>(C);
         hipLaunchKernelGGL(segmean_finalize_kernel, dim3(grid_for(groups, g.lg)), dim3(kThreads), 0, as_stream(stream),
-                           partial, off0, B, nbits, level, C, g.lg, cp.S, plane_nhwc, mean ? 1 : 0, ld_out);
+                           partial, off0, B, nbits, level, C, g.lg, cp.S, plane_nhwc, mean ? 1 : 0, ld_out, rowmap);
         return check_launch("segmean_fwd(coarse)");
     }
     if (mean) {
         T2H_DISPATCH_VEC(C,
             { GroupCfg g = group_cfg<4>(C);
               hipLaunchKernelGGL(segmean_fwd_kernel<4>, dim3(grid_for(groups, g.lg)), dim3(kThreads), 0, as_stream(stream),
-                                 feat, off0, B, nbits, level, C, g.lg, plane_nhwc, ld_out); },
+                                 feat, off0, B, nbits, level, C, g.lg, plane_nhwc, ld_out, rowmap); },
             { GroupCfg g = group_cfg<1>(C);
               hipLaunchKernelGGL(segmean_fwd_kernel<1>, dim3(grid_for(groups, g.lg)), dim3(kThreads), 0, as_stream(stream),
-                                 feat, off0, B, nbits, level, C, g.lg, plane_nhwc, ld_out); });
+                                 feat, off0, B, nbits, level, C, g.lg, plane_nhwc, ld_out, rowmap); });
     } else {
         T2H_DISPATCH_VEC(C,
             { GroupCfg g = group_cfg<4>(C);
               hipLaunchKernelGGL((segmean_fwd_kernel<4, false>), dim3(grid_for(groups, g.lg)), dim3(kThreads), 0, as_stream(stream),
-                                 feat, off0, B, nbits, level, C, g.lg, plane_nhwc, ld_out); },
+                                 feat, off0, B, nbits, level, C, g.lg, plane_nhwc, ld_out, rowmap); },
             { GroupCfg g = group_cfg<1>(C);
               hipLaunchKernelGGL((segmean_fwd_kernel<1, false>), dim3(grid_for(groups, g.lg)), dim3(kThreads), 0, as_stream(stream),
-                                 feat, off0, B, nbits, level, C, g.lg, plane_nhwc, ld_out); });
+                                 feat, off0, B, nbits, level, C, g.lg, plane_nhwc, ld_out, rowmap); });
     }
     return check_launch("segmean_fwd");
 }
@@ -1736,11 +1782,13 @@
 
 T2H_API int t2h_segsum_fwd(const float *feat, const int32_t *off0, int B, int N, int nbits, int level, int C,
                            float *plane_nhwc, int ld_plane, void *workspace, size_t workspace_bytes, t2h_stream_t stream) {
-    return segreduce_fwd(false, feat, off0, B, N, nbits, level, C, plane_nhwc, ld_plane, workspace, workspace_bytes, stream);
+    const CompactRows cr = take_compact();
+    return segreduce_fwd(false, feat, off0, B, N, nbits, level, C, plane_nhwc, ld_plane, workspace, workspace_bytes, stream, cr);
 }
 
 T2H_API int t2h_plane_sumpool2x2(const float *fine_nhwc, int ld_fine, int B, int r_fine, int C, float *coarse_nhwc, int ld_coarse,
                                  t2h_stream_t stream) {
+    const CompactRows cr = take_compact();
     if (!fine_nhwc || !coarse_nhwc) return fail(T2H_ERR_ARG, "plane_sumpool2x2: null pointer");
     if (B < 1 || r_fine < 2 || (r_fine & 1) || C < 4 || C % 4 != 0 || ((uintptr_t)fine_nhwc & 15) || ((uintptr_t)coarse_nhwc & 15) ||
         ld_fine < C || ld_coarse < C || ld_fine % 4 != 0 || ld_coarse % 4 != 0)
@@ -1748,13 +1796,15 @@
     const int rc = r_fine / 2;
     const int64_t total4 = (int64_t)B * rc * rc * (C / 4);
     hipLaunchKernelGGL(plane_sumpool2x2_kernel, dim3((unsigned)((total4 + kThreads - 1) / kThreads)), dim3(kThreads), 0,
-                       as_stream(stream), fine_nhwc, total4, rc, C / 4, ld_fine, ld_coarse, coarse_nhwc);
+                       as_stream(stream), fine_nhwc, total4, rc, C / 4, ld_fine, ld_coarse, coarse_nhwc,
+                       cr.row_of_cell);
     return check_launch("plane_sumpool2x2");
 }
 
 T2H_API int t2h_segsum_bwd_multi(const float *const *gplanes_nhwc, const int *levels, const int *lds, int n_planes,
                                  const int32_t *cell, int B, int N, int nbits, int C, const float *mask, const float *addend,
                                  float *gfeat, t2h_stream_t stream) {
+    const CompactRows cr = take_compact();
     if (!gplanes_nhwc || !levels || !lds || !cell || !gfeat) return fail(T2H_ERR_ARG, "segsum_bwd_multi: null pointer");
     if (n_planes < 1 || n_planes > kMaxMultiPlanes)
         return fail(T2H_ERR_ARG, "segsum_bwd_multi: 1..%d planes, got %d", kMaxMultiPlanes, n_planes);
@@ -1769,6 +1819,7 @@
     }
     if (C % 4 == 0 && ((mask && ((uintptr_t)mask & 15)) || (addend && ((uintptr_t)addend & 15)) || ((uintptr_t)gfeat & 15)))
         return fail(T2H_ERR_ARG, "segsum_bwd_multi: rows must be 16-byte aligned");
+    set_compact(mp, cr, B, nbits);
     const int64_t npts = rows_of(B, N);
     if (npts == 0) return T2H_OK;
     T2H_DISPATCH_VEC(C,
@@ -1859,7 +1910,11 @@
                                              int nbits, int level, int sum_level, int C, float *sums_nhwc, int ld_sums,
                                              float *pooled_nhwc, int ld_pooled, void *sign_bits, const int32_t *cell_order,
                                              t2h_stream_t stream) {
+    const CompactRows cr = take_compact();
     if (!plane_nhwc || !pts || !off0 || !sums_nhwc) return fail(T2H_ERR_ARG, "sample_relu_cellsums: null pointer");
+    if (cr.row_of_cell && cr.level != sum_level)
+        return fail(T2H_ERR_ARG, "sample_relu_cellsums: compact rows of level %d asked for the sums of level %d", cr.level, sum_level);
+    const int32_t *rowmap = cr.row_of_cell;
     if (pooled_nhwc && (sum_level >= level || ld_pooled < C || ld_pooled % 4 != 0 || ((uintptr_t)pooled_nhwc & 15)))
         return fail(T2H_ERR_ARG, "sample_relu_cellsums: the pooled sums need sum_level < level and 16-byte aligned rows of >= C floats");
     int rc = check_level("sample_relu_cellsums", B, nbits, level, C);
@@ -1884,7 +1939,7 @@
     if (k0) while (nchild / (4 * gz * 2) >= quad && cells * chunks * gz < kMinWgs) gz *= 2;
     const dim3 grid((unsigned)((k0 ? cells : (cells >> 2)) * chunks * gz));
 #define T2H_V2_LAUNCH(KK, PP) hipLaunchKernelGGL((sample_relu_cellsums_v2_kernel<KK, PP>), grid, dim3(256), 0, as_stream(stream), \
-        plane_nhwc, pts, dim, off0, nbits, level, sum_level, C, sums_nhwc, ld_sums, bw, npts_m1, pooled_nhwc, ld_pooled, k0 ? order_k0 : order_k1, gz)
+        plane_nhwc, pts, dim, off0, nbits, level, sum_level, C, sums_nhwc, ld_sums, bw, npts_m1, pooled_nhwc, ld_pooled, k0 ? order_k0 : order_k1, gz, rowmap)
     if (k0) { if (pooled_nhwc) T2H_V2_LAUNCH(0, true); else T2H_V2_LAUNCH(0, false); }
     else { if (pooled_nhwc) T2H_V2_LAUNCH(1, true); else T2H_V2_LAUNCH(1, false); }
 #undef T2H_V2_LAUNCH
@@ -1904,6 +1959,7 @@
                                              const int32_t *off0, int B, int N, int nbits, int level, int C, float *gplane_nhwc,
                                              void *workspace, size_t workspace_bytes, const int32_t *cell_order,
                                              t2h_stream_t stream) {
+    const CompactRows cr = take_compact();
     if (!gplanes_nhwc || !levels || !lds || !cell || !mask || !pts || !off0 || !gplane_nhwc)
         return fail(T2H_ERR_ARG, "sample_bwd_from_sums: null pointer");
     if (n_planes < 1 || n_planes > kMaxMultiPlanes)
@@ -1928,6 +1984,7 @@
             return fail(T2H_ERR_ARG, "sample_bwd_from_sums: bad plane %d", q);
         mp.g[q] = gplanes_nhwc[q]; mp.level[q] = levels[q]; mp.ld[q] = lds[q];
     }
+    set_compact(mp, cr, B, nbits);
     int64_t groups = (int64_t)B << (2 * (nbits - level));
     float *partial = static_cast<float *>(workspace);
     int G = 1 << cp.lgG, P = kCellThreads >> cp.lgG;
diff --git a/tomosar2height_amd/csrc/t2h_common.h b/tomosar2height_amd/csrc/t2h_common.h
--- a/tomosar2height_amd/csrc/t2h_common.h
+++ b/tomosar2height_amd/csrc/t2h_common.h
@@ -17,6 +17,13 @@
 int check_launch(const char *what);
 void note_kernel(const char *name);
 const char *noted_kernel();
+
+struct CompactRows {
+    const int32_t *row_of_cell = nullptr;
+    int level = -1;
+    const int32_t *n_rows = nullptr;
+};
+CompactRows take_compact();
 
 inline hipStream_t as_stream(t2h_stream_t s) { return reinterpret_cast<hipStream_t>(s); }
 
diff --git a/tomosar2height_amd/csrc/tile_index.hip b/tomosar2height_amd/csrc/tile_index.hip
--- a/tomosar2height_amd/csrc/tile_index.hip
+++ b/tomosar2height_amd/csrc/tile_index.hip
@@ -16,6 +16,12 @@
 static thread_local const char *g_noted_kernel = "";
 void note_kernel(const char *name) { g_noted_kernel = name; }
 const char *noted_kernel() { return g_noted_kernel; }
+static thread_local CompactRows g_compact;
+CompactRows take_compact() {
+    const CompactRows c = g_compact;
+    g_compact = CompactRows{};
+    return c;
+}
 int check_launch(const char *what) {
     hipError_t e = hipGetLastError();
     if (e != hipSuccess) return fail(T2H_ERR_LAUNCH, "%s: %s", what, hipGetErrorString(e));
@@ -201,6 +207,9 @@
 T2H_API const char *t2h_last_error_string(void) { return err_buf(); }
 T2H_API const char *t2h_last_kernel_name(void) { return noted_kernel(); }
 T2H_API void t2h_clear_kernel_name(void) { note_kernel(""); }
+T2H_API void t2h_compact_next(const int32_t *row_of_cell, int level, const int32_t *n_rows) {
+    g_compact.row_of_cell = row_of_cell; g_compact.level = level; g_compact.n_rows = n_rows;
+}
 
 T2H_API int t2h_debug_poison_lds(t2h_stream_t stream) {
     static unsigned *sink = nullptr;
diff --git a/tomosar2height_amd/deferred.py b/tomosar2height_amd/deferred.py
--- a/tomosar2height_amd/deferred.py
+++ b/tomosar2height_amd/deferred.py
@@ -10,22 +10,28 @@
 CELLS_MFMA = os.environ.get("T2H_CELLS_MFMA", "1") != "0"
 SIGN_BITS = os.environ.get("T2H_SIGN_BITS", "1") != "0"
 ON_CHIP_HIDDEN = os.environ.get("T2H_ON_CHIP_HIDDEN", "1") != "0"
+COMPACT_SUMS = os.environ.get("T2H_COMPACT_SUMS", "1") != "0"
+_empty = torch.empty
 ON_CHIP_MIN_PTS_PER_CELL = float(os.environ.get("T2H_ON_CHIP_MIN_PTS", "8"))
 
 
-def _segsum_into(tile, rows, level, dst):
+def _segsum_into(tile, rows, level, dst, state=None):
     n, c = rows.shape
     r = tile.R >> level
     ws_bytes = _lib.ws_bytes("t2h_segmean_workspace_bytes", tile.B, tile.N, tile.nbits, level, c)
     ws = _lib.workspace(ws_bytes, rows.device)
+    if state is not None:
+        state.request(level)
     _lib.call("t2h_segsum_fwd", _lib.ptr(rows), _lib.ptr(tile.off0), tile.B, tile.N, tile.nbits, level, c, dst.data_ptr(),
               dst.stride(0), _lib.ptr(ws), ws_bytes, _lib.stream(), nbytes=4 * c * n + 4 * n + 4 * c * tile.B * r * r,
               tag=_lib.timing() and f"t2h_segsum_fwd[C={c},r={r}]")
 
 
-def _sumpool_into(tile, fine, level_fine, coarse):
+def _sumpool_into(tile, fine, level_fine, coarse, state=None):
     c = fine.shape[1]
     r = tile.R >> level_fine
+    if state is not None:
+        state.request(level_fine)
     _lib.call("t2h_plane_sumpool2x2", fine.data_ptr(), fine.stride(0), tile.B, r, c, coarse.data_ptr(), coarse.stride(0),
               _lib.stream(), nbytes=5 * c * tile.B * r * r, tag=_lib.timing() and f"t2h_plane_sumpool2x2[C={c}]")
 
@@ -37,14 +43,34 @@
     return ctypes.cast(arr, ctypes.c_void_p), ctypes.cast(lvs, ctypes.c_void_p), ctypes.cast(lds, ctypes.c_void_p)
 
 
-def _gather(tile, planes, c, mask=None):
+def _gather(tile, planes, c, mask=None, state=None):
     out = torch.empty(tile.n_points, c, dtype=torch.float32, device=tile.device)
     arr, lvs, lds = _plane_args(planes)
+    if state is not None:
+        state.request_any(lv for _, lv in planes)
     _lib.call("t2h_segsum_bwd_multi", arr, lvs, lds, len(planes), _lib.ptr(tile.cell), tile.B, tile.N, tile.nbits, c,
               None if mask is None else _lib.ptr(mask), None, _lib.ptr(out), _lib.stream(),
               nbytes=4 * c * tile.n_points * (2 if mask is not None else 1) + 4 * tile.n_points
               + sum(4 * c * p.shape[0] for p, _ in planes), tag=_lib.timing() and f"t2h_segsum_bwd_multi[C={c},n={len(planes)}]")
     return out
+
+
+def cell_rows(tile, level):
+    cache = tile.__dict__.setdefault("_cell_rows", {})
+    hit = cache.get(level)
+    if hit is None:
+        r = tile.R >> level
+        p = tile.B * r * r
+        buf = torch.empty(2 * p + 4 + (p + 2047) // 2048, dtype=torch.int32, device=tile.device)
+        cnt = torch.empty(p, dtype=torch.float32, device=tile.device)
+        _lib.compact_next(buf.data_ptr(), level, buf.data_ptr() + 8 * p)
+        _lib.call("t2h_cell_counts", _lib.ptr(tile.off0), tile.B, tile.nbits, level, _lib.ptr(cnt), _lib.stream(), nbytes=28 * p)
+        tile.__dict__.setdefault("_cell_counts", {}).setdefault(level, cnt)
+        ready = _lib.Ready()
+        ready.mark()
+        hit = cache[level] = (buf, ready)
+    hit[1].wait()
+    return hit[0]
 
 
 def counts(tile, level):
@@ -131,6 +157,7 @@
             if len(levels) > 1 and levels[1] == levels[0] + 1 and levels[0] < tile.level(r):
                 second = state.sums(idx + 1, levels[1])
             order = tile.cell_order(tile.level(r))
+            state.request(levels[0])
             _lib.call("t2h_sample_relu_cellsums_ordered", _lib.ptr(q_rows), _lib.ptr(tile.pts), tile.dim, _lib.ptr(tile.off0), tile.B,
                       tile.N, tile.nbits, tile.level(r), levels[0], c2, finest.data_ptr(), finest.stride(0),
                       None if second is None else second.data_ptr(), 0 if second is None else second.stride(0),
@@ -153,10 +180,11 @@
         if a_all.shape[0] != k:
             raise RuntimeError(f"deferred level {idx}: {a_all.shape[0]} composed rows for {k} source columns")
         x = state.S[lv][:, :k]
-        acc = torch.empty(x.shape[0], a_all.shape[1], dtype=torch.float32, device=x.device)
-        mlp.linear_dgrad_(x, a_all, acc, bx3=True)
+        acc = _empty(x.shape[0], a_all.shape[1], dtype=torch.float32, device=x.device)
+        mlp.linear_dgrad_(x, a_all, acc, bx3=True, row_limit=state.row_limit(lv))
         cnt = counts(tile, lv)
         out = torch.empty_like(acc)
+        state.request(lv)
         _lib.call("t2h_mean_bias_fwd", _lib.ptr(acc), _lib.ptr(cnt), _lib.ptr(const), acc.shape[0], acc.shape[1], _lib.ptr(out),
                   _lib.stream(), nbytes=8 * acc.numel() + 4 * acc.shape[0])
         ctx.state, ctx.idx, ctx.r, ctx.has_base = state, idx, r, idx == 0
@@ -175,11 +203,13 @@
         g = g.contiguous()
         p, c = g.shape
         cnt = counts(tile, lv)
-        dacc = torch.empty_like(g)
+        dacc = _empty(g.shape, dtype=torch.float32, device=g.device)
+        lim = state.row_limit(lv)
         cached = state.cache is not None and not ctx.needs_input_grad[1]
         dconst = torch.empty(ctx.const_shape, dtype=torch.float32, device=g.device) if (ctx.needs_input_grad[2] or cached) else None
         ws_bytes = _lib.ws_bytes("t2h_mean_bias_bwd_workspace_bytes", p, c)
         ws = _lib.workspace(ws_bytes, g.device)
+        state.request(lv)
         _lib.call("t2h_mean_bias_bwd", _lib.ptr(g), _lib.ptr(cnt), p, c, _lib.ptr(dacc), None if dconst is None else _lib.ptr(dconst),
                   _lib.ptr(ws), ws_bytes, _lib.stream(), nbytes=8 * p * c + 4 * p)
         x = state.S[lv][:, :k]
@@ -187,22 +217,22 @@
         if cached:
             e = state.cache.levels[idx]
             e.ready.wait()
-            mlp.linear_wgrad_(x, dacc, e.ga, None, accumulate=True, defer=True)
+            mlp.linear_wgrad_(x, dacc, e.ga, None, accumulate=True, defer=True, row_limit=lim)
             e.gconst.add_(dconst)
             dconst = None
             state.cache.pending = True
         elif ctx.needs_input_grad[1]:
             if ga_thru is not None and ga_thru.is_contiguous() and ga_thru.dtype == torch.float32 and mlp.sole_owner(ga_thru):
-                mlp.linear_wgrad_(x, dacc, ga_thru, None, accumulate=True)
+                mlp.linear_wgrad_(x, dacc, ga_thru, None, accumulate=True, row_limit=lim)
             else:
                 da = torch.empty_like(a_all)
-                mlp.linear_wgrad_(x, dacc, da, None)
+                mlp.linear_wgrad_(x, dacc, da, None, row_limit=lim)
                 if ga_thru is not None:
                     da = da + ga_thru
         dS, seen = state.grad_matrix(lv)
         if seen and seen < k:
             raise RuntimeError("deferred backward out of order")
-        mlp.linear_fwd_(dacc, a_all, None, dS[:, :k], accumulate=bool(seen), bx3=True)
+        mlp.linear_fwd_(dacc, a_all, None, dS[:, :k], accumulate=bool(seen), bx3=True, row_limit=lim)
         state.dS_cols[lv] = max(seen, k)
         lo, hi = state.off[idx + 1], state.off[idx + 2]
         planes = [(state.dS[l][:, lo:hi], l) for l in state.needed(idx + 1)]
@@ -212,7 +242,7 @@
         dbase = None
         if ctx.has_base and ctx.needs_input_grad[3]:
             lo0, hi0 = state.off[0], state.off[1]
-            dbase = _gather(tile, [(state.dS[l][:, lo0:hi0], l) for l in state.needed(0)], hi0 - lo0)
+            dbase = _gather(tile, [(state.dS[l][:, lo0:hi0], l) for l in state.needed(0)], hi0 - lo0, state=state)
         return dq, da, dconst, dbase, None, None, None
 
 
@@ -307,8 +337,25 @@
             self.off.append(self.off[-1] + kk)
         self.base = base_rows
         self.S, self.dS, self.dS_cols = {}, {}, {}
+        self.compact_lv, self.rows = None, None
+        if COMPACT_SUMS and mlp._MODE == "fp32" and tile.n_points > 0:
+            self.compact_lv = min(self.levels_seq)
+            self.rows = cell_rows(tile, self.compact_lv)
+            r = tile.R >> self.compact_lv
+            self._row_ptr, self._n_rows_ptr = self.rows.data_ptr(), self.rows.data_ptr() + 8 * tile.B * r * r
         self.a_all, self.const = None, None
         self.n_done = 0
+
+    def request(self, lv):
+        if lv == self.compact_lv:
+            _lib.compact_next(self._row_ptr, lv, self._n_rows_ptr)
+
+    def request_any(self, levels):
+        if self.compact_lv is not None and self.compact_lv in levels:
+            self.request(self.compact_lv)
+
+    def row_limit(self, lv):
+        return self._n_rows_ptr if lv == self.compact_lv else None
 
     def needed(self, src):
         first = 0 if src == 0 else src - 1
@@ -317,7 +364,7 @@
     def _matrix(self, store, lv):
         if lv not in store:
             r = self.tile.R >> lv
-            store[lv] = torch.empty(self.tile.B * r * r, self.off[-1], dtype=torch.float32, device=self.tile.device)
+            store[lv] = _empty(self.tile.B * r * r, self.off[-1], dtype=torch.float32, device=self.tile.device)
         return store[lv]
 
     def sums(self, src, lv):
@@ -328,7 +375,7 @@
 
     def write_sums(self, src, rows):
         finest = self.needed(src)[0]
-        _segsum_into(self.tile, rows, finest, self.sums(src, finest))
+        _segsum_into(self.tile, rows, finest, self.sums(src, finest), self)
         self.pool_down(src)
 
     def pool_down(self, src, start=0):
@@ -343,7 +390,7 @@
                 else:
                     rn = self.tile.R >> nxt_level
                     nxt = torch.empty(self.tile.B * rn * rn, cur.shape[1], dtype=torch.float32, device=cur.device)
-                _sumpool_into(self.tile, cur, cur_level, nxt)
+                _sumpool_into(self.tile, cur, cur_level, nxt, self)
                 cur, cur_level = nxt, nxt_level
 
     def hidden_grad(self, planes, h, r, c2, mask_is_bits=False):
@@ -355,13 +402,14 @@
             ws = _lib.workspace(ws_bytes, h.device)
             dq = torch.empty(tile.B * r * r, c2, dtype=torch.float32, device=h.device)
             order = tile.cell_order(level) if mask_is_bits else None
+            self.request_any([lv for _, lv in planes])
             _lib.call("t2h_sample_bwd_from_sums_ordered", arr, lvs, lds, len(planes), _lib.ptr(tile.cell), _lib.ptr(h),
                       1 if mask_is_bits else 0, _lib.ptr(tile.pts), tile.dim, _lib.ptr(tile.off0), tile.B, tile.N, tile.nbits,
                       level, c2, _lib.ptr(dq), _lib.ptr(ws), ws_bytes, None if order is None else _lib.ptr(order), _lib.stream(),
                       nbytes=(c2 // 8 if mask_is_bits else 4 * c2) * tile.n_points + 12 * tile.n_points + 4 * dq.numel()
                       + sum(4 * c2 * p.shape[0] for p, _ in planes), tag=_lib.timing() and f"t2h_sample_bwd_from_sums[C={c2},r={r}]")
             return dq
-        dh = _gather(tile, planes, c2, mask=h)
+        dh = _gather(tile, planes, c2, mask=h, state=self)
         return ops._sample_bwd(tile, dh, r, c2, None).reshape(tile.B * r * r, c2)
 
     def advance(self, q_rows, r, fc_b, fc_c):
diff --git a/tomosar2height_amd/mlp.py b/tomosar2height_amd/mlp.py
--- a/tomosar2height_amd/mlp.py
+++ b/tomosar2height_amd/mlp.py
@@ -51,7 +51,7 @@
     return force or wide_short or (n >= min_n and k >= min_k and m >= 4096)
 
 
-def _gemm_bx3(x, w, w_is_kn, bias, mask, y, relu_out, accumulate, tag):
+def _gemm_bx3(x, w, w_is_kn, bias, mask, y, relu_out, accumulate, tag, row_limit=None):
     from . import grid
     (xp, ldx), (yp, ldy) = _rows(x, "gemm_bx3 x"), _rows(y, "gemm_bx3 y")
     m, k = x.shape
@@ -60,18 +60,21 @@
     nws = _lib.ws_bytes("t2h_gemm_bx3_workspace_bytes", m, k, n)
     ws = _lib.workspace(nws, x.device)
     flags = (_lib.RELU_OUT if relu_out else 0) | (_lib.ACCUM if accumulate else 0) | (_lib.F16X2 if grid._h2() else 0)
-    _lib.call("t2h_gemm_bx3", xp, ldx, _lib.ptr(grid.split_weights.get_gemm(w, w_is_kn)), bias.data_ptr() if bias is not None else None,
+    wf = _lib.ptr(grid.split_weights.get_gemm(w, w_is_kn))
+    if row_limit is not None:
+        _lib.compact_next(None, -1, row_limit)
+    _lib.call("t2h_gemm_bx3", xp, ldx, wf, bias.data_ptr() if bias is not None else None,
               mp, ldm, yp, ldy, m, k, n, flags, _lib.ptr(ws), nws, _lib.stream(),
               nbytes=4 * (m * k + m * n + n * k + (m * n if mask is not None else 0)), flops=2 * m * k * n, tag=_lib.timing() and tag)
     return y
 
 
-def linear_fwd_(x, w, bias, y, relu_in=False, relu_out=False, accumulate=False, bx3=False):
+def linear_fwd_(x, w, bias, y, relu_in=False, relu_out=False, accumulate=False, bx3=False, row_limit=None):
     (xp, ldx), (yp, ldy) = _rows(x, "linear_fwd x"), _rows(y, "linear_fwd y")
     m, k = x.shape
     n = w.shape[0]
     if bx3 and not relu_in and w.is_contiguous() and _bx3_gemm_ok(m, k, n, x, y):
-        return _gemm_bx3(x, w, False, bias, None, y, relu_out, accumulate, f"t2h_linear_fwd[K={k},N={n}]")
+        return _gemm_bx3(x, w, False, bias, None, y, relu_out, accumulate, f"t2h_linear_fwd[K={k},N={n}]", row_limit)
     w = w.contiguous()
     flags = (_lib.RELU_IN if relu_in else 0) | (_lib.RELU_OUT if relu_out else 0) | (_lib.ACCUM if accumulate else 0) | _pflag()
     _lib.call("t2h_linear_fwd", xp, ldx, w.data_ptr(), bias.data_ptr() if bias is not None else None, yp, ldy, m, k, n,
@@ -80,12 +83,12 @@
     return y
 
 
-def linear_dgrad_(dy, w, dx, mask=None, accumulate=False, bx3=False):
+def linear_dgrad_(dy, w, dx, mask=None, accumulate=False, bx3=False, row_limit=None):
     (gp, ldg), (dp, ldd) = _rows(dy, "linear_dgrad dy"), _rows(dx, "linear_dgrad dx")
     m, n = dy.shape
     k = w.shape[1]
     if bx3 and w.is_contiguous() and _bx3_gemm_ok(m, n, k, dy, dx, mask):
-        return _gemm_bx3(dy, w, True, None, mask, dx, False, accumulate, f"t2h_linear_dgrad[N={n},K={k}]")
+        return _gemm_bx3(dy, w, True, None, mask, dx, False, accumulate, f"t2h_linear_dgrad[N={n},K={k}]", row_limit)
     w = w.contiguous()
     mp, ldm = (None, 0) if mask is None else _rows(mask, "linear_dgrad mask")
     _lib.call("t2h_linear_dgrad", gp, ldg, w.data_ptr(), dp, ldd, m, k, n, mp, ldm,
@@ -100,7 +103,7 @@
     return grid._h2()
 
 
-def linear_wgrad_(dy, x, dw, db, relu_in=False, accumulate=False, defer=False):
+def linear_wgrad_(dy, x, dw, db, relu_in=False, accumulate=False, defer=False, row_limit=None):
     (gp, ldg), (xp, ldx) = _rows(dy, "linear_wgrad dy"), _rows(x, "linear_wgrad x")
     m, n = dy.shape
     k = x.shape[1]
@@ -112,7 +115,7 @@
             if db is not None:
                 db.zero_()
         return
-    bx3 = (_GEMM_BX3_WGRAD and GEMM_BX3 and _MODE == "fp32" and not relu_in and n >= _BX3_WGRAD_MIN_N and m >= _BX3_WGRAD_MIN_M
+    bx3 = (row_limit is None and _GEMM_BX3_WGRAD and GEMM_BX3 and _MODE == "fp32" and not relu_in and n >= _BX3_WGRAD_MIN_N and m >= _BX3_WGRAD_MIN_M
            and _grid_h2() and bool(_lib.ws_bytes("t2h_gemm_bx3_wgrad_supported", m, k, n)))
     query, pflags = (("t2h_gemm_bx3_wgrad_workspace_bytes", _lib.F16X2) if bx3 else
                      ("t2h_linear_wgrad_workspace_bytes", (_lib.RELU_IN if relu_in else 0) | _pflag()))
@@ -124,6 +127,8 @@
     if bx3:
         _lib.call("t2h_gemm_bx3_wgrad", gp, ldg, xp, ldx, m, k, n, *outs, flags, ws.data_ptr(), ws_bytes, _lib.stream(), **cost)
     else:
+        if row_limit is not None:
+            _lib.compact_next(None, -1, row_limit)
         _lib.call("t2h_linear_wgrad", gp, ldg, xp, ldx, m, k, n, flags, *outs, ws.data_ptr(), ws_bytes, _lib.stream(), **cost)
 
 
diff --git a/tomosar2height_amd/tile.py b/tomosar2height_amd/tile.py
--- a/tomosar2height_amd/tile.py
+++ b/tomosar2height_amd/tile.py
@@ -161,6 +161,9 @@
             from . import ops, deferred
             if ops.SAMPLE_ADJOINT and 0 < tile.n_points <= ops.SAMPLE_ADJOINT_MAX_ROWS * tile.B * tile.R * tile.R:
                 tile.sample_adjoint(0)
+            from . import mlp
+            if deferred.COMPACT_SUMS and mlp._MODE == "fp32":
+                deferred.cell_rows(tile, 0)
             for lv in range(min(4, tile.nbits)):
                 deferred.counts(tile, lv)
                 if lv >= 1:
@@ -180,6 +183,7 @@
             else:
                 out += list(val)
         out += list(self.__dict__.get("_cell_counts", {}).values())
+        out += [buf for buf, _ in self.__dict__.get("_cell_rows", {}).values()]
         return out
 
     def wait_ready(self):
```

Measured after the change: 193.5 tiles/s, median of 6. 2.1% higher.
